# egpbos/barcode

Measured on AMD Instinct MI355X. Metric: HMC leapfrog steps/sec on 256^3 grid, higher is better.
Workload: dtype f64; 1 GPU; 256^3 grid, L=200 Mpc/h, Gaussian prior, Zel'dovich + plane-parallel RSD (reference behaviour of '2LPT+RSD', SURVEY M3), likelihood=1, mass kernel mk=3 (3 = SPH), calc_h=2, mass_type=1, fp64; one trajectory of 817 leapfrog steps per chain; grid=256, chains=1, parallelism=independent chains, 1 per GPU, rehearsal_single_device=False, steps_done=817, finite=True

## Files before the change

### barcode_amd/csrc/bchmc.hip

```cpp
#include "../../include/bchmc.h"
#include "kernels.hpp"
#include "fft_host.hpp"
#include "owned.hpp"
#include "pass_launch.hpp"
#include "launch_grid.hpp"
#include "eval_plan.hpp"
#include "interp_plan.hpp"

#include <rocfft/rocfft.h>
#include <rocprofiler-sdk-roctx/roctx.h>

#include <algorithm>
#include <chrono>
#include <cmath>
#include <cfloat>
#include <cstdarg>
#include <cstdio>
#include <cstdlib>
#include <climits>
#include <cstring>
#include <mutex>
#include <string>
#include <thread>
#include <type_traits>
#include <vector>

using namespace bchmc;
using namespace owned;

namespace {

struct ProfRec {
  int cls;
  Event a, b;
};

}

struct bchmc_handle {
  bchmc_config c{};
  Geo g{};
  bool f32 = false;
  size_t esz = 8;
  int mass_fs = 0, mass_rs = 0;
  PathSwitches sw;
  bool no_tiles_low = false;
  std::string err;
  RocfftUser fft_user;
  Stream stream;

  DevBytes work;
  FftInfo info;
  FftPlan r2c1, c2r1, r2c3, c2r3;

  DevBytes in_arr[6];
  bool have[6] = {false, false, false, false, false, false};
  DevBuf<double> wS, wM;

  DevBytes qk, pk, gk;
  DevBytes qk2, pk2;
  DevBytes Ck;
  bool ck_pair = false;
  DevBytes tC;
  DevBytes psi;
  DevBytes V;
  DevBytes rho, plike;
  DevBuf<long long> rho_fix;
  DevBuf<int> fix_sat;
  long long fix_sat_limit = 1ll << 62;
  bool fix = false;
  DevBytes ioq, iop;
  DevBytes gprior, glike;
  DevBytes conv;
  DevBuf<double> convF;
  DevBuf<double> dstage;
  DevBytes cq, cp;
  DevBuf<double> part6;
  bool have_cq = false, have_cp = false, have_prop = false;
  DevBytes cg;
  bool cg_valid = false, prop_g_valid = false;
  double c_like = 0., prop_like = 0.;
  DevBuf<double> rho_part, partA;
  DevBuf<double> guard;
  DevBuf<int> stop;
  DevBuf<unsigned long long> steps_done;
  PinnedBuf<double> h_part;
  struct MtDraw {
    long long S = 0, C = 0, G = 0;
    int B = 0;
    DevBuf<uint32_t> poly, win, words, st;
    DevBuf<unsigned long long> nz, nzoff, acc, accoff, lastend;
    DevBuf<unsigned long long> res;
    PinnedBuf<unsigned long long> h_io;
    DevBuf<double> gauss;
    double setup_ms = 0.;
  } mt;
  struct Mock {
    DevBuf<unsigned long long> cnt, off, gsum, goff, res;
  } mock;
  DevBuf<double> spec_bins;
  DevBytes cross_ak;
  struct Ens {
    struct Slot {
      uint64_t count = 0;
      DevBuf<double> mean, m2;
    } slot[BCHMC_ENS_SLOTS];
    int ncu = 0;
  } ens;
  struct Tweb {
    DevBytes t[6];
    DevBytes xk;
    DevBuf<unsigned char> type;
    DevBuf<double> lam;
    DevBuf<unsigned long long> part;
    DevBuf<unsigned int> cnt;
    bool have_t = false;
    uint64_t samples = 0;
    bool have_par = false;
// ... 258 lines not shown
  pp.L = h->g.L;
  pp.rsd = rsd;
  pp.periodic = 1;
  const double a = h->c.ascale, OM = h->c.OM, OL = h->c.OL;
  pp.cpecvel = c_pecvel1(a, OM, OL);
  const double Hub = 100. * std::sqrt(OM / a / a / a + OL + (1. - OM - OL) / a / a);
  pp.v_norm = 1. / Hub / a;
  return pp;
}

SphPar make_sph(const bchmc_handle *h) {
  SphPar sp;
  sp.h = h->c.particle_kernel_h;
  sp.h_inv = 1. / sp.h;
  sp.w_norm = 1. / M_PI / (sp.h * sp.h * sp.h);
  sp.r2_lim = 4. * sp.h * sp.h * (1. + (h->f32 ? 1e-5 : 1e-12));
  sp.min1 = h->c.min1;
  sp.min2 = h->c.min2;
  sp.min3 = h->c.min3;
  sp.reach = h->plan.reach;
  return sp;
}

LikePar make_like(const bchmc_handle *h) {
  LikePar lp;
  lp.rho_c = h->c.rho_c;
  lp.biasP = h->c.biasP;
  lp.biasE = h->c.biasE;
  lp.delta_min = h->c.delta_min;
  lp.likelihood = h->c.likelihood;
  lp.bias_is_identity = (h->c.biasE == 1.0);
  return lp;
}

HullPar make_hull(const bchmc_handle *h) {
  HullPar hp;
  const double hh = h->c.particle_kernel_h;
  hp.cols = h->hull;
  hp.ncol = h->plan.hull_n;
  hp.h_inv = 1. / hh;
  hp.d_h = h->g.d * hp.h_inv;
  hp.norm = 1. / (M_PI * (hh * hh) * (hh * hh));
  hp.normalize = h->c.rho_c * h->g.L * h->g.L * h->g.L / (double)h->g.N;
  hp.f1 = fgrow1(h->c.ascale, h->c.OM, h->c.OL);
  return hp;
}

int need_input(bchmc_handle *h, int f, const char *name) {
  if (!h->have[f]) return h->fail(BCHMC_ERR_STATE, "input array %s was never uploaded", name);
  return BCHMC_OK;
}

struct FieldSource {
  enum Made { kAsHeld, kOverdens, kPositions };
  void *base = nullptr;
  size_t offset = 0;
  Made made = kAsHeld;
};
int field_source(bchmc_handle *h, int field, FieldSource *fs) {
  const size_t N = (size_t)h->g.N;
  *fs = FieldSource{};
  switch (field) {
    case BCHMC_F_SIGNAL_PS: case BCHMC_F_MASS_F: case BCHMC_F_MASS_R:
    case BCHMC_F_NOBS: case BCHMC_F_NOISE: case BCHMC_F_WINDOW:
      fs->base = h->in_arr[field].get();
      break;
    case BCHMC_F_DELTAX: fs->base = h->ioq.get(), fs->made = FieldSource::kOverdens; break;
    case BCHMC_F_POSX: case BCHMC_F_POSY: case BCHMC_F_POSZ: fs->base = h->ioq.get(), fs->made = FieldSource::kPositions; break;
    case BCHMC_F_RHO: fs->base = h->rho.get(); break;
    case BCHMC_F_PART_LIKE: fs->base = h->plike.get(); break;
    case BCHMC_F_VX: case BCHMC_F_VY: case BCHMC_F_VZ: fs->base = h->V.get(), fs->offset = (size_t)(field - BCHMC_F_VX) * N; break;
    case BCHMC_F_PSIX: case BCHMC_F_PSIY: case BCHMC_F_PSIZ:
      fs->base = h->psi.get(), fs->offset = (size_t)(field - BCHMC_F_PSIX) * N;
      break;
    case BCHMC_F_GRAD_PRIOR: fs->base = h->gprior.get(); break;
    case BCHMC_F_GRAD_LIKE: fs->base = h->glike.get(); break;
    default: return h->fail(BCHMC_ERR_ARG, "unknown field %d", field);
  }
  if (!fs->base) return h->fail(BCHMC_ERR_STATE, "field %d has not been computed", field);
  return BCHMC_OK;
}
int fetch_ready(bchmc_handle *h, int field) {
  if (field >= BCHMC_F_DELTAX && field <= BCHMC_F_PSIZ && !h->have_eval)
    return h->fail(BCHMC_ERR_STATE, "no forward evaluation to fetch from");
  FieldSource fs;
  return field_source(h, field, &fs);
}

int check_inputs(bchmc_handle *h) {
  CHK(need_input(h, BCHMC_F_SIGNAL_PS, "signal_PS"));
  if (h->mass_fs) CHK(need_input(h, BCHMC_F_MASS_F, "mass_f"));
  if (h->mass_rs) CHK(need_input(h, BCHMC_F_MASS_R, "mass_r"));
  CHK(need_input(h, BCHMC_F_NOBS, "nobs"));
  CHK(need_input(h, BCHMC_F_WINDOW, "window"));
  if (h->c.likelihood != 0) CHK(need_input(h, BCHMC_F_NOISE, "noise"));
  return BCHMC_OK;
}

RecQuad *recs(const bchmc_handle *h) { return static_cast<RecQuad *>(h->srec.get()); }
int *slot_words(bchmc_handle *h) { return h->t_cnt + (kOct + 1) * (size_t)h->plan.tp.ntiles + 1; }

void repartition(bchmc_handle *h) {
  h->plan.tp.cap = h->plan.slots.cap;
  h->sorted_valid = false;
}

int realloc_slots(bchmc_handle *h, long long want) {
  HIPCHK(hipStreamSynchronize(h->stream));
  SlotPolicy &sl = h->plan.slots;
  const bool verbose = env_on("BCHMC_VERBOSE");
  const long long cap = sl.clamp_to_budget(want);
  if (!cap) {
    if (verbose) fprintf(stderr, "bchmc: record slots stay at %lld per tile (memory budget %lld): overflowing evaluations "
                                 "run the two-pass sort\n", sl.cap_alloc, sl.cap_budget);
    sl.after_realloc(SlotGot::kOldSize, cap);
    return BCHMC_OK;
  }
  (void)h->srec.release();
  h->sorted_valid = false;
  for (SlotGot got : {SlotGot::kWanted, SlotGot::kOldSize, SlotGot::kRecordsOnly}) {
    const size_t nrec = record_count(h->g.N, sl.rung(got, cap), h->plan.tp.ntiles);
    if (h->srec.alloc(nrec * 4 * h->esz) == hipSuccess) {
      if (got == SlotGot::kWanted) {
        if (verbose) fprintf(stderr, "bchmc: record array reallocated for %lld slots per tile\n", cap);
// ... 77 lines not shown
  bool ok2 = rocfft_plan_description_create(&f2) == rocfft_status_success &&
             rocfft_plan_description_create(&i2) == rocfft_status_success;
  ok2 = ok2 && rocfft_plan_description_set_data_layout(f2, rocfft_array_type_real, rocfft_array_type_hermitian_interleaved,
                                                       nullptr, nullptr, 2, rs2, (size_t)g.n * g.n, 2, cs2,
                                                       (size_t)g.n * g.nhp) == rocfft_status_success;
  ok2 = ok2 && rocfft_plan_description_set_data_layout(i2, rocfft_array_type_hermitian_interleaved, rocfft_array_type_real,
                                                       nullptr, nullptr, 2, cs2, (size_t)g.n * g.nhp, 2, rs2,
                                                       (size_t)g.n * g.n) == rocfft_status_success;
  ok2 = ok2 && r2c.create(rocfft_plan_create, rocfft_placement_notinplace, rocfft_transform_type_real_forward, prec, 2,
                          len2, batch, f2) == rocfft_status_success;
  ok2 = ok2 && c2r.create(rocfft_plan_create, rocfft_placement_notinplace, rocfft_transform_type_real_inverse, prec, 2,
                          len2, batch, i2) == rocfft_status_success;
  if (f2) rocfft_plan_description_destroy(f2);
  if (i2) rocfft_plan_description_destroy(i2);
  if (ok2 && h->info) {
    size_t need = 0;
    for (const FftPlan *p : {&r2c, &c2r}) {
      size_t wb = 0;
      if (rocfft_plan_get_work_buffer_size(*p, &wb) != rocfft_status_success) ok2 = false;
      need = std::max(need, wb);
    }
    if (ok2 && need > h->work.capacity()) {
      DevBytes nw;
      (void)hipStreamSynchronize(h->stream);
      if (nw.alloc(need) == hipSuccess &&
          rocfft_execution_info_set_work_buffer(h->info, nw, need) == rocfft_status_success) {
        h->work = std::move(nw);
      } else {
        (void)hipGetLastError();
        ok2 = false;
      }
    }
  }
  if (!ok2) {
    r2c.reset();
    c2r.reset();
    return BCHMC_ERR_ROCFFT;
  }
  return BCHMC_OK;
}

PathSwitches read_path_switches() {
  PathSwitches s;
  s.no_planes = env_on("BCHMC_NO_PLANES");
  s.no_planes_ends = env_on("BCHMC_NO_PLANES_ENDS");
  s.no_fuse = env_on("BCHMC_NO_FUSE");
  s.no_alpt_planes = env_on("BCHMC_NO_ALPT_PLANES");
  s.no_zbin = env_on("BCHMC_NO_ZBIN");
  s.zbin_128 = env_on("BCHMC_ZBIN_128");
  s.yfwd_f64 = env_on("BCHMC_YFWD_F64");
  s.bx_v1 = env_on("BCHMC_BX_V1");
  s.bx_v2 = env_on("BCHMC_BX_V2");
  s.no_pair = env_on("BCHMC_NO_PAIR");
  return s;
}

PathFacts path_facts(bchmc_handle *h, int rsd) {
  PathFacts f;
  f.n = h->g.n, f.esz = (int)h->esz, f.Nhp = h->g.Nhp;
  f.planes_ok = h->planes_ok && h->xtw;
  f.tiled = h->plan.tiled, f.sort_direct = h->plan.slots.sort_direct;
  f.mk = h->c.mk, f.calc_h = h->c.calc_h, f.likelihood = h->c.likelihood, f.sfmodel = h->c.sfmodel;
  f.rsd_model = h->c.rsd_model, f.mass_rs = h->mass_rs != 0;
  if (alpt_planes_wanted(f, h->sw, rsd) && !h->c2r2d_2 && !h->alpt_plans_failed &&
      make_plans_2d(h, 2 * (size_t)h->g.n, h->r2c2d_2, h->c2r2d_2) != BCHMC_OK)
    h->alpt_plans_failed = true;
  f.alpt_plans = h->c2r2d_2 != nullptr;
  return f;
}

int host_sum(bchmc_handle *h, const double *d_part, double *out) {
  HIPCHK(hipMemcpyAsync(h->h_part, d_part, kRedBlocks * sizeof(double), hipMemcpyDeviceToHost, h->stream));
  HIPCHK(hipStreamSynchronize(h->stream));
  double s = 0.;
  for (int i = 0; i < kRedBlocks; i++) s += h->h_part[i];
  *out = s;
  return BCHMC_OK;
}

void par_memcpy(void *dst, const void *src, size_t bytes, int nt) {
  if (nt <= 1 || bytes < ((size_t)4 << 20)) {
    std::memcpy(dst, src, bytes);
    return;
  }
  std::vector<std::thread> th;
  const size_t per = ((bytes / (size_t)nt) + 4095) & ~(size_t)4095;
  for (int t = 1; t < nt; t++) {
    const size_t off = per * (size_t)t;
    if (off >= bytes) break;
    const size_t len = std::min(per, bytes - off);
    th.emplace_back([=] { std::memcpy((char *)dst + off, (const char *)src + off, len); });
  }
  std::memcpy(dst, src, std::min(per, bytes));
  for (auto &t : th) t.join();
}

int stg_init(bchmc_handle *h) {
  if (h->stg[0]) return BCHMC_OK;
  size_t chunk = (size_t)16 << 20;
  if (const char *ev = std::getenv("BCHMC_STAGE_MB")) chunk = (size_t)std::max(1, atoi(ev)) << 20;
  int nt = (int)std::min(8u, std::max(1u, std::thread::hardware_concurrency() / 2));
  if (const char *ev = std::getenv("BCHMC_STAGE_THREADS")) nt = std::max(1, atoi(ev));
  for (int b = 0; b < 2; b++) {
    HIPCHK(h->stg[b].alloc(chunk));
    HIPCHK(h->stg_ev[b].create(hipEventDisableTiming));
  }
  h->stg_chunk = chunk;
  h->stg_threads = nt;
  return BCHMC_OK;
}

int h2d(bchmc_handle *h, void *dst, const void *src, size_t bytes, hipStream_t stream = nullptr) {
  if (!stream) stream = h->stream;
  if (bytes <= ((size_t)1 << 20)) {
// ... 599 lines not shown
      CHK(fft_exec(h, h->r2c2d_2, h->V, Ck, BCHMC_K_FFT_R2C));
      ProfScope ps(h, BCHMC_K_KSPACE_DRIFT_ZA);
      HIPCHK(launch_alpt_mix_x<T>(pass_ctx(h), Ck, h->c.kth, 1. / h->alpt_wtot, 1. / (double)N));
    } else {
      CHK(fft_exec(h, h->r2c1, a_out, Ck, BCHMC_K_FFT_R2C));
      CHK(fft_exec(h, h->r2c1, b_out, Ck + Nhp, BCHMC_K_FFT_R2C));
      ProfScope ps(h, BCHMC_K_KSPACE_DRIFT_ZA);
      k_alpt_mix<T><<<nblk_stride(Nhp), 256, 0, h->stream>>>(h->g, Ck, h->c.kth, 1. / h->alpt_wtot, 1. / (double)N);
      HIPCHK(hipGetLastError());
    }
    return BCHMC_OK;
  }

  static int launch_alpt(bchmc_handle *h, double dq_factor, bool planes) {
    const double scale = dq_factor / (double)h->g.N;
    if (planes) {
      {
        ProfScope ps(h, BCHMC_K_KSPACE_DRIFT_ZA);
        StepCtl nc{h->stop, h->steps_done, nullptr, 0., 0};
        BoundaryX<T> bx;
        bx.qi = C(h->qk), bx.c_za = scale, bx.ctl = nc;
        CHK((launch_boundary_x<BX_FIRST, true>(h, bx)));
      }
      return alpt_middle(h, true);
    }
    {
      ProfScope ps(h, BCHMC_K_KSPACE_DRIFT_ZA);
      k_alpt_poisson<T><<<nblk_stride(h->g.Nhp), 256, 0, h->stream>>>(h->g, C(h->qk), C(h->Ck), C(h->Ck) + h->g.Nhp, scale);
      HIPCHK(hipGetLastError());
    }
    return alpt_middle(h, false);
  }

  static int forward_rest(bchmc_handle *h, int rsd, EvalMode m) {
    if (rsd && !h->c.planepar) return h->fail(BCHMC_ERR_RSD_NOT_PLANEPAR, "non-plane-parallel RSD is not implemented");
    const bool zbin = eval_zbin(path_facts(h, rsd), h->sw, m);
    const bool pair = h->ck_pair;
    h->ck_pair = false;
    if (pair && !zbin) return h->fail(BCHMC_ERR_STATE, "two arrays between the x and y passes, and no y pass of the engine's own");
    if (zbin) {
      ProfScope ps(h, BCHMC_K_FFT_C2R);
      HIPCHK(pair ? launch_ypass_pair<T>(pass_ctx(h), C(h->Ck)) : launch_ypass<T>(pass_ctx(h), C(h->Ck)));
    } else {
      CHK(fft_exec(h, m.planes_c2r ? h->c2r2d : h->c2r3, h->Ck, h->psi, BCHMC_K_FFT_C2R));
    }
    return particle_stage(h, rsd, m, zbin);
  }

  static int particle_stage(bchmc_handle *h, int rsd, EvalMode m, bool zbin) {
    h->sorted_valid = false;
    bool rho_cleared = false;
    const PosPar pp = make_pos(h, rsd);
    const SphPar sp = make_sph(h);
    if (h->plan.tiled) {
      ProfScope ps(h, BCHMC_K_SORT);
      const int nt = h->plan.tp.ntiles, nbricks = nblk_full(h->g.N);
      int *cnt1 = h->t_cnt, *cnt2 = h->t_cnt + kOct * nt, *ovf = h->t_cnt + (kOct + 1) * nt;
      if (!h->cnt_clean) HIPCHK(hipMemsetAsync(h->t_cnt, 0, ((kOct + 1) * (size_t)nt + 1) * sizeof(int), h->stream));
      h->cnt_clean = false;
      const int fb_grid = h->plan.slots.sort_direct ? std::min(nbricks, 4096) : nbricks;
      if (zbin) {
        HIPCHK(launch_zbin<T>(pass_ctx(h), pp, sp, h->plan.tp, C(h->Ck), cnt1, ovf, recs(h), R(h->V), h->rho_part,
                              h->fix ? nullptr : R(h->rho), h->fix ? h->rho_fix : nullptr,
                              m.psi_unread ? nullptr : R(h->psi)));
        if (m.psi_unread)
          HIPCHK((launch_zbin<T, true>(pass_ctx(h), pp, sp, h->plan.tp, C(h->Ck), cnt1, ovf, nullptr, nullptr, nullptr,
                                       nullptr, nullptr, R(h->psi))));
        rho_cleared = true;
      } else if (h->plan.slots.sort_direct) {
        const int nsuper = (nbricks + kBinPer - 1) / kBinPer;
        k_bin_direct<T><<<nsuper, BCHMC_BIN_THREADS, 0, h->stream>>>(h->g, pp, sp, h->plan.tp, nsuper, R(h->psi), cnt1, ovf,
                                                       recs(h), R(h->V), h->rho_part,
                                                       h->fix ? nullptr : R(h->rho),
                                                       h->fix ? h->rho_fix : nullptr);
        rho_cleared = true;
      } else {
        HIPCHK(hipMemsetAsync(ovf, 1, 1, h->stream));
      }
      k_bin<T><<<fb_grid, 256, 0, h->stream>>>(h->g, pp, sp, h->plan.tp, nbricks, R(h->psi), cnt2, ovf, h->t_rank, R(h->V));
      k_scan_tiles<<<(nt + 1023) / 1024, 1024, 0, h->stream>>>(h->plan.tp, cnt1, cnt2, ovf, h->t_off, h->t_end, h->t_woff,
                                                               h->t_oct, h->t_seg, ovf + 2);
      k_reorder<T><<<fb_grid, 256, 0, h->stream>>>(h->g, pp, nbricks, R(h->psi), h->t_rank, h->t_off, ovf,
                                                   recs(h));
      HIPCHK(hipGetLastError());
      h->sorted_valid = true;
    }
    {
      ProfScope ps(h, BCHMC_K_SCATTER);
      const bool tile_path = (h->c.mk == 3 && h->plan.tiled), tile_low = (h->c.mk >= 0 && h->c.mk <= 2 && h->plan.tiled);
      const double fix_scale = h->c.mk == 3 ? 70368744177664. / sp.w_norm : 70368744177664.;
      if (rho_cleared) {
      } else if (h->fix) {
        HIPCHK(hipMemsetAsync(h->rho_fix, 0, h->g.N * sizeof(long long), h->stream));
      } else {
        HIPCHK(hipMemsetAsync(h->rho, 0, h->g.N * sizeof(T), h->stream));
      }
      if (tile_path) {
        if (!h->plan.slots.sort_direct && !h->fix) HIPCHK(hipMemsetAsync(h->rho_part, 0, kRedBlocks * sizeof(double), h->stream));
        const int grid = tile_grid(h);
        const int ncol = h->plan.hull_exact ? h->plan.hull_n : 0;
        const int reorder = (h->plan.tp.chunk > 2048) ? 0 : 2;
        if (reorder) {
          k_subsort<T><<<std::min(grid, 8192), 256, 0, h->stream>>>(h->g, h->plan.tp, reorder, recs(h), h->t_off, h->t_end, h->t_woff,
                                                   h->t_oct, h->t_seg);
          HIPCHK(hipGetLastError());
        }
        if (h->plan.std81) {
          if (h->fix)
            k_scatter_tile81<T, 12, 20, true><<<grid, kTile81Threads, tile_lds(h, 0, sizeof(double)), h->stream>>>(
                h->g, sp, h->plan.tp, recs(h), h->t_off, h->t_end, h->t_woff,
                h->t_oct, h->t_seg, h->rho_fix, h->rho_part, h->t_cnt,
                (kOct + 1) * h->plan.tp.ntiles + 1, fix_scale);
          else
            k_scatter_tile81<T, 12, 20, false><<<grid, kTile81Threads, tile_lds(h, 0, sizeof(double)), h->stream>>>(
                h->g, sp, h->plan.tp, recs(h), h->t_off, h->t_end, h->t_woff,
                h->t_oct, h->t_seg, R(h->rho), h->rho_part, h->t_cnt,
                (kOct + 1) * h->plan.tp.ntiles + 1, fix_scale);
          h->cnt_clean = true;
        } else if (h->fix) {
          k_scatter_tile<T, true><<<grid, 256, tile_lds(h, ncol, sizeof(double)), h->stream>>>(
              h->g, sp, h->plan.tp, h->hull, ncol, recs(h), h->t_off, h->t_end,
              h->t_woff, h->t_oct, h->t_seg, h->rho_fix, h->rho_part, fix_scale);
        } else {
          k_scatter_tile<T, false><<<grid, 256, tile_lds(h, ncol, sizeof(double)), h->stream>>>(
              h->g, sp, h->plan.tp, h->hull, ncol, recs(h), h->t_off, h->t_end,
              h->t_woff, h->t_oct, h->t_seg, R(h->rho), h->rho_part, fix_scale);
        }
      } else if (tile_low) {
        if (!h->plan.slots.sort_direct && !h->fix) HIPCHK(hipMemsetAsync(h->rho_part, 0, kRedBlocks * sizeof(double), h->stream));
        const int grid = tile_grid(h);
        const size_t lds = (size_t)(h->plan.tp.tx + 2) * (h->plan.tp.ty + 2) * (h->plan.tp.tz + 2) * sizeof(double);
        const int ncnt = (kOct + 1) * h->plan.tp.ntiles + 1;
// ... 1 lines not shown
          k_scatter_tile_low<T, true><<<grid, 256, lds, h->stream>>>(h->g, h->plan.tp, h->c.mk, recs(h), h->t_off,
                                                                     h->t_end, h->t_woff, h->t_oct, h->t_seg, h->rho_fix,
                                                                     h->rho_part, h->t_cnt, ncnt, fix_scale);
        else
          k_scatter_tile_low<T, false><<<grid, 256, lds, h->stream>>>(h->g, h->plan.tp, h->c.mk, recs(h), h->t_off,
                                                                      h->t_end, h->t_woff, h->t_oct, h->t_seg, R(h->rho),
                                                                      h->rho_part, h->t_cnt, ncnt, fix_scale);
        h->cnt_clean = true;
      } else if (h->c.mk == 3) {
        if (h->fix)
          k_scatter_sph<T, true><<<nblk_full(h->g.N), 256, 0, h->stream>>>(h->g, pp, sp, R(h->psi), h->rho_fix, fix_scale);
        else
          k_scatter_sph<T, false><<<nblk_full(h->g.N), 256, 0, h->stream>>>(h->g, pp, sp, R(h->psi), R(h->rho), fix_scale);
      } else if (h->c.mk >= 0 && h->c.mk <= 2) {
        if (h->fix)
          k_scatter_low_order<T, true><<<nblk_full(h->g.N), 256, 0, h->stream>>>(h->g, pp, sp, h->c.mk, R(h->psi),
                                                                                 h->rho_fix, fix_scale);
        else
          k_scatter_low_order<T, false><<<nblk_full(h->g.N), 256, 0, h->stream>>>(h->g, pp, sp, h->c.mk, R(h->psi),
                                                                                  R(h->rho), fix_scale);
      } else {
        return h->fail(BCHMC_ERR_ARG, "masskernel %d is not a valid value (0..3)", h->c.mk);
      }
      HIPCHK(hipGetLastError());
      if (h->fix) {
        k_fix_to_rho<T><<<kRedBlocks, 256, 0, h->stream>>>(h->g.N, h->rho_fix, 1. / fix_scale, R(h->rho), h->rho_part,
                                                           h->fix_sat, h->fix_sat_limit);
        HIPCHK(hipGetLastError());
      }
    }
    if (!h->plan.tiled && !h->fix) {
      ProfScope ps(h, BCHMC_K_MEAN_PARTIAL);
      k_sum<T><<<kRedBlocks, 256, 0, h->stream>>>(R(h->rho), h->g.N, h->rho_part);
      HIPCHK(hipGetLastError());
    }
    h->have_eval = true;
    h->last_rsd = rsd;
    return BCHMC_OK;
  }

  static int ensure_conv(bchmc_handle *h) {
    if (!h->conv) CHK(dev_alloc(h, h->conv, 3 * (size_t)h->g.N * sizeof(T)));
    return BCHMC_OK;
  }

  static int like_force(bchmc_handle *h, EvalMode m, int *like_mode, bool transform = true) {
    if (h->c.calc_h == 2 || h->c.calc_h == 3) {
      if (h->c.mk != 3)
        return h->fail(BCHMC_ERR_MK_NOT_SPH, "Must use SPH mass kernel (masskernel = 3) with calc_h = 2 or 3");
    } else if (h->c.calc_h != 1 && h->c.calc_h != 0) {
      return h->fail(BCHMC_ERR_ARG, "calc_h = %d is not a valid value (0..3)", h->c.calc_h);
    }
    const long long N = h->g.N, Nh = h->g.Nhp;
    {
      ProfScope ps(h, BCHMC_K_MEAN_PARTIAL);
      k_partial_like<T><<<nblk_stride(N), 256, 0, h->stream>>>(h->g, make_like(h), R(h->rho), h->rho_part,
                                                               R(h->in_arr[BCHMC_F_NOBS]), R(h->in_arr[BCHMC_F_NOISE]),
                                                               R(h->in_arr[BCHMC_F_WINDOW]), R(h->plike));
      HIPCHK(hipGetLastError());
    }
    if (h->c.calc_h == 1) {
      if (transform) CHK(fft_exec(h, h->r2c1, h->plike, h->Ck, BCHMC_K_FFT_R2C));
      *like_mode = 1;
      return BCHMC_OK;
    }
    if (h->c.calc_h == 0) {
      {
        ProfScope ps(h, BCHMC_K_OTHER);
        k_overdens<T><<<nblk_stride(N), 256, 0, h->stream>>>(h->g, R(h->rho), h->rho_part, R(h->ioq));
        HIPCHK(hipGetLastError());
      }
      if (h->c.likelihood == 1) {
        CHK(ensure_conv(h));
        CHK(fft_exec(h, h->r2c1, h->ioq, h->tC, BCHMC_K_FFT_R2C));
        {
          ProfScope ps(h, BCHMC_K_OTHER);
          k_gradfft_mult<T><<<nblk_stride(Nh), 256, 0, h->stream>>>(h->g, C(h->tC), C(h->Ck), 1. / (double)N);
          HIPCHK(hipGetLastError());
        }
        CHK(fft_exec(h, h->c2r3, h->Ck, h->conv, BCHMC_K_FFT_C2R));
        ProfScope ps(h, BCHMC_K_OTHER);
        k_mul3<T><<<nblk_stride(N), 256, 0, h->stream>>>(N, R(h->plike), R(h->conv), R(h->V));
        HIPCHK(hipGetLastError());
      } else {
        ProfScope ps(h, BCHMC_K_OTHER);
        k_findif_mul<T><<<nblk_stride(N), 256, 0, h->stream>>>(h->g, make_like(h), R(h->ioq), R(h->plike), R(h->V));
        HIPCHK(hipGetLastError());
      }
      if (transform) CHK(fft_exec(h, h->r2c3, h->V, h->Ck, BCHMC_K_FFT_R2C));
      *like_mode = 0;
      return BCHMC_OK;
    }
    if (h->c.calc_h == 3) {
      if (h->last_rsd && !h->c.planepar)
        return h->fail(BCHMC_ERR_RSD_NOT_PLANEPAR, "non-plane-parallel RSD is not implemented in calc_V");
      CHK(ensure_conv(h));
      if (!h->convF) CHK(build_conv_table(h));
      CHK(fft_exec(h, h->r2c1, h->plike, h->tC, BCHMC_K_FFT_R2C));
      const double hh = h->c.particle_kernel_h;
      {
        ProfScope ps(h, BCHMC_K_OTHER);
        k_conv_kernel<T><<<nblk_stride(Nh), 256, 0, h->stream>>>(h->g, C(h->tC), h->convF, C(h->Ck), hh, 1. / (double)N);
        HIPCHK(hipGetLastError());
      }
      CHK(fft_exec(h, h->c2r3, h->Ck, h->conv, BCHMC_K_FFT_C2R));
      {
        ProfScope ps(h, BCHMC_K_GATHER);
        if (h->plan.tiled && h->sorted_valid && !h->no_tiles_low) {
          const int grid = tile_grid(h);
          const size_t lds = 3 * (size_t)(h->plan.tp.tx + 2) * (h->plan.tp.ty + 2) * (h->plan.tp.tz + 2) * sizeof(T);
          k_interp_tsc_tile<T><<<grid, 256, lds, h->stream>>>(h->g, h->plan.tp, h->last_rsd, fgrow1(h->c.ascale, h->c.OM, h->c.OL),
                                                              recs(h), h->t_off, h->t_end, h->t_woff,
                                                              h->t_oct, h->t_seg, R(h->conv), R(h->V));
        } else {
          k_interp_tsc<T><<<nblk_full(N), 256, 0, h->stream>>>(h->g, make_pos(h, h->last_rsd),
                                                               fgrow1(h->c.ascale, h->c.OM, h->c.OL), R(h->psi),
                                                               R(h->conv), R(h->V));
        }
        HIPCHK(hipGetLastError());
      }
    } else {
      ProfScope ps(h, BCHMC_K_GATHER);
      HullPar hp = make_hull(h);
      if (h->plan.tiled && h->sorted_valid) {
        const int grid = tile_grid(h);
        if (h->plan.std81)
          k_gather_tile81<T, 12, 20><<<grid, kTile81Threads, tile_lds(h, 0, sizeof(T)), h->stream>>>(
              h->g, hp, h->plan.tp, h->last_rsd, recs(h), h->t_off, h->t_end, h->t_woff,
              h->t_oct, h->t_seg, R(h->plike), R(h->V));
        else
          k_gather_tile<T><<<grid, 256, tile_lds(h, hp.ncol, sizeof(T)), h->stream>>>(
              h->g, hp, h->plan.tp, h->last_rsd, recs(h), h->t_off, h->t_end, h->t_woff,
              h->t_oct, h->t_seg, R(h->plike), R(h->V));
      } else {
        k_gather_sph<T><<<nblk_full(N), 256, hp.ncol * sizeof(int4), h->stream>>>(h->g, make_pos(h, h->last_rsd), hp,
                                                                                  R(h->psi), R(h->plike), R(h->V));
      }
      HIPCHK(hipGetLastError());
    }
    if (!transform) {
    } else if (eval_yfwd(path_facts(h, h->c.rsd_model), h->sw, m)) {
      ProfScope ps(h, BCHMC_K_FFT_R2C);
      HIPCHK(launch_zr2c<T>(pass_ctx(h), R(h->V), C(h->Ck)));
      HIPCHK((launch_ypass<T, false>(pass_ctx(h), C(h->Ck))));
    } else {
      CHK(fft_exec(h, m.planes_r2c ? h->r2c2d : h->r2c3, h->V, h->Ck, BCHMC_K_FFT_R2C));
    }
    *like_mode = 0;
    return BCHMC_OK;
  }

  static int grf_force(bchmc_handle *h) {
    {
      ProfScope ps(h, BCHMC_K_OTHER);
      k_scale_c<T><<<nblk_stride(h->g.Nhp), 256, 0, h->stream>>>(h->g.Nhp, C(h->qk), C(h->tC), 1. / (double)h->g.N);
      HIPCHK(hipGetLastError());
    }
    CHK(fft_exec(h, h->c2r1, h->tC, h->plike, BCHMC_K_FFT_C2R));
    {
      ProfScope ps(h, BCHMC_K_OTHER);
      k_grf_grad<T><<<nblk_stride(h->g.N), 256, 0, h->stream>>>(h->g.N, R(h->plike), R(h->in_arr[BCHMC_F_NOBS]),
                                                                R(h->in_arr[BCHMC_F_NOISE]),
                                                                R(h->in_arr[BCHMC_F_WINDOW]), R(h->rho));
      HIPCHK(hipGetLastError());
    }
    CHK(fft_exec(h, h->r2c1, h->rho, h->Ck, BCHMC_K_FFT_R2C));
    h->have_eval = false;
    return BCHMC_OK;
  }

  static int force_sources(bchmc_handle *h, bool pre_za, EvalMode m, int *like_mode, double *b) {
    if (h->c.likelihood == 3) {
      CHK(grf_force(h));
      *like_mode = 1;
      *b = h->c.grad_psi_likeli_factor;
      return BCHMC_OK;
    }
    if (!pre_za) {
      CHK(displacement(h, h->c.deltaQ_factor, h->c.rsd_model, &m.planes_c2r));
    } else if (m.alpt_pending) {
      CHK(alpt_middle(h, true));
      m.planes_c2r = true;
    }
    CHK(forward_rest(h, h->c.rsd_model, m));
    CHK(like_force(h, m, like_mode));
    double norm = -1.;
    norm *= h->c.deltaQ_factor;
    if (h->c.correct_delta) norm *= h->c.D1;
    *b = h->c.grad_psi_likeli_factor * norm;
    return BCHMC_OK;
  }

  template <bool KICK>
  static int launch_assemble(bchmc_handle *h, double a, double b, int like_mode, double c_kick, double *guard_slot) {
    h->prop_g_valid = false;
    ProfScope ps(h, BCHMC_K_KSPACE_FORCE_KICK);
    k_assemble<T, KICK><<<nblk_stride(h->g.Nhp), 256, 0, h->stream>>>(h->g, C(h->Ck), C(h->qk), h->wS, C(h->gk), C(h->pk),
                                                                     a, b, like_mode, c_kick, guard_slot, h->stop);
    HIPCHK(hipGetLastError());
    return BCHMC_OK;
  }

  static int r2c_state(bchmc_handle *h, const double *d_real, void *staging, void *out) {
    CHK(load_real(h, d_real, R(staging)));
    return fft_exec(h, h->r2c1, staging, out, BCHMC_K_FFT_R2C);
  }

  static int c2r_scaled(bchmc_handle *h, const void *xk, void *out_T) {
    {
      ProfScope ps(h, BCHMC_K_OTHER);
      k_scale_c<T><<<nblk_stride(h->g.Nhp), 256, 0, h->stream>>>(h->g.Nhp, reinterpret_cast<const CT *>(xk), C(h->tC),
                                                                1. / (double)h->g.N);
      HIPCHK(hipGetLastError());
    }
    return fft_exec(h, h->c2r1, h->tC, out_T, BCHMC_K_FFT_C2R);
  }

  static int c2r_state(bchmc_handle *h, const void *xk, void *scratch_T, double *d_out) {
    if (kDouble) return c2r_scaled(h, xk, d_out);
    CHK(c2r_scaled(h, xk, scratch_T));
    return store_real(h, R(scratch_T), d_out);
  }

  static int mass_rs_term(bchmc_handle *h) {
    CHK(c2r_scaled(h, h->pk, h->iop));
    {
      ProfScope ps(h, BCHMC_K_OTHER);
      k_div_mass_r<T><<<nblk_stride(h->g.N), 256, 0, h->stream>>>(h->g.N, R(h->iop), R(h->in_arr[BCHMC_F_MASS_R]),
                                                                  R(h->iop));
      HIPCHK(hipGetLastError());
    }
    return fft_exec(h, h->r2c1, h->iop, h->tC, BCHMC_K_FFT_R2C);
  }

  struct Tap {
    double *like_i, *like_f;
  };

  static int tap_loglike(bchmc_handle *h, double *partials) {
    k_loglike<T><<<kRedBlocks, 256, 0, h->stream>>>(h->g, make_like(h), R(h->rho), h->rho_part,
                                                    R(h->in_arr[BCHMC_F_NOBS]), R(h->in_arr[BCHMC_F_NOISE]),
                                                    R(h->in_arr[BCHMC_F_WINDOW]), partials);
    HIPCHK(hipGetLastError());
    return BCHMC_OK;
  }

  struct Traj {
    PathFacts f;
    TrajPlan p;
    double a, c_za;
    bool pair;
  };
  static Traj traj(bchmc_handle *h) {
    Traj t;
    t.f = path_facts(h, h->c.rsd_model);
    t.p = traj_plan(t.f, h->sw);
    t.a = h->c.grad_psi_prior_factor;
    t.c_za = (t.p.c_za == CZa::kAlptInput ? 1. : -h->c.D1) * h->c.deltaQ_factor / (double)h->g.N;
    t.pair = psi_pair(t.f, h->sw, t.p);
    return t;
  }

  template <int MODE, bool ALPT = false>
  static int launch_boundary_x(bchmc_handle *h, const BoundaryX<T> &bx) {
    HIPCHK((launch_step_boundary_x<T, MODE, ALPT>(pass_ctx(h), C(h->Ck), h->wS, bx)));
    h->ck_pair = bx.pair && !ALPT && MODE != BX_LAST;
    return BCHMC_OK;
  }

  static int initial_force(bchmc_handle *h, const Traj &t, double *like_i, void *g0_out) {
    int like_mode = 2;
    double b = 0.;
    const InitialEval kind = initial_eval(t.f, h->sw, t.p);
    if (kind == InitialEval::k3d) {
      CHK(force_sources(h, false, EvalMode{}, &like_mode, &b));
      if (like_i) CHK(tap_loglike(h, like_i));
      CHK(launch_assemble<false>(h, t.a, b, like_mode, 0., nullptr));
    } else {
      StepCtl nc{h->stop, h->steps_done, nullptr, 0., 0};
      {
        ProfScope ps(h, BCHMC_K_KSPACE_DRIFT_ZA);
        BoundaryX<T> bx;
        bx.qi = C(h->qk), bx.c_za = t.c_za, bx.ctl = nc, bx.pair = t.pair;
        if (kind == InitialEval::kBxFirstAlpt) CHK((launch_boundary_x<BX_FIRST, true>(h, bx)));
        else CHK(launch_boundary_x<BX_FIRST>(h, bx));
      }
      EvalMode m;
      m.planes_c2r = m.planes_r2c = true;
      m.alpt_pending = t.p.alpt_x;
      CHK(force_sources(h, true, m, &like_mode, &b));
      if (like_mode != 0) return h->fail(BCHMC_ERR_STATE, "planes mode without the three V components");
      if (like_i) CHK(tap_loglike(h, like_i));
      h->prop_g_valid = false;
      ProfScope ps(h, BCHMC_K_KSPACE_FORCE_KICK);
      BoundaryX<T> bx;
      bx.qi = C(h->qk), bx.a = t.a, bx.b = b, bx.ctl = nc, bx.g_out = C(h->gk);
      CHK(launch_boundary_x<BX_LAST>(h, bx));
    }
    if (g0_out)
      HIPCHK(hipMemcpyAsync(g0_out, h->gk, 2 * (size_t)h->g.Nhp * sizeof(T), hipMemcpyDeviceToDevice, h->stream));
    return BCHMC_OK;
  }

  static int trajectory(bchmc_handle *h, double eps, uint64_t neps, const Tap *tap, const void *g0_in = nullptr,
                        void *g0_out = nullptr) {
    h->prop_g_valid = false;
    if (neps + 1 > h->guard.capacity())
      CHK(dev_reserve(h, h->guard, std::max<size_t>(4096, 2 * (neps + 1))));
    HIPCHK(hipMemsetAsync(h->guard, 0, (neps + 1) * sizeof(double), h->stream));
    k_init_ctl<<<1, 1, 0, h->stream>>>(h->stop, h->steps_done, (unsigned long long)neps);
    HIPCHK(hipGetLastError());

    const Traj t = traj(h);
    int like_mode = 2;
    double b = 0.;
    if (!g0_in) CHK(initial_force(h, t, tap ? tap->like_i : nullptr, g0_out));
    const void *g_first = g0_in ? g0_in : h->gk;
// ... 33 lines not shown

  static int trajectory_fused(bchmc_handle *h, double eps, uint64_t neps, const Tap *tap, const Traj &t,
                              const void *g_first) {
    const double *wM = h->mass_fs ? h->wM : nullptr;
    const double guard_limit = 1e50 * (double)h->g.N, a = t.a, c_za = t.c_za;
    if (!h->qk2) {
      CHK(dev_alloc(h, h->qk2, 2 * (size_t)h->g.Nhp * sizeof(T)));
      CHK(dev_alloc(h, h->pk2, 2 * (size_t)h->g.Nhp * sizeof(T)));
    }
    void *const q0 = h->qk, *const p0 = h->pk, *const q1 = h->qk2, *const p1 = h->pk2;
    int like_mode = 2;
    double b = 0.;
    int cur = 0;
    {
      StepCtl ctl{h->stop, h->steps_done, nullptr, guard_limit, 0};
      ProfScope ps(h, BCHMC_K_KSPACE_DRIFT_ZA);
      BoundaryX<T> bx;
      bx.qi = bx.qo = C(q0), bx.pi = bx.po = C(p0), bx.wM = wM, bx.half_eps = 0.5 * eps, bx.eps = eps, bx.c_za = c_za;
      bx.ctl = ctl, bx.g_in = C(g_first), bx.pair = t.pair;
      switch (opening(t.f, h->sw, t.p)) {
        case Opening::kBxFirstAlpt: CHK((launch_boundary_x<BX_FIRST, true>(h, bx))); break;
        case Opening::kBxFirst: CHK(launch_boundary_x<BX_FIRST>(h, bx)); break;
        case Opening::kKickDriftZa:
          h->ck_pair = false;
          k_kick_drift_za<T, true><<<nblk_stride(h->g.Nhp), 256, 0, h->stream>>>(h->g, C(q0), C(p0), C(g_first), wM,
                                                                               nullptr, C(h->Ck), 0.5 * eps, eps, c_za, ctl);
          break;
      }
      HIPCHK(hipGetLastError());
    }
    for (uint64_t s = 0; s < neps; s++) {
      const bool last = (s + 1 == neps);
      if (last && h->early_q_dev && h->ev_q) {
        CHK(c2r_state(h, cur ? q1 : q0, h->ioq, h->early_q_dev));
        HIPCHK(hipEventRecord(h->ev_q, h->stream));
        h->early_q_done = true;
      }
      if (h->plan.slots.slot_watch && h->plan.tiled && h->plan.slots.sort_direct && s > 0 && s % kSlotPoll == 0)
        CHK(poll_slots(h, s / kSlotPoll));
      CHK(force_sources(h, true, step_mode(t.f, h->sw, t.p, s, neps), &like_mode, &b));
      if (tap && tap->like_f && last) CHK(tap_loglike(h, tap->like_f));
      StepCtl ctl{h->stop, h->steps_done, s > 0 ? h->guard + (s - 1) : nullptr, guard_limit, s};
      void *qi = cur ? q1 : q0, *pi = cur ? p1 : p0, *qo = cur ? q0 : q1, *po = cur ? p0 : p1;
      ProfScope ps(h, BCHMC_K_KSPACE_FORCE_KICK);
      BoundaryX<T> bx;
      bx.qi = C(qi), bx.pi = C(pi), bx.qo = C(qo), bx.po = C(po), bx.wM = wM, bx.a = a, bx.b = b, bx.half_eps = 0.5 * eps;
      bx.eps = eps, bx.c_za = c_za, bx.guard_slot = h->guard + s, bx.ctl = ctl, bx.pair = t.pair;
      switch (closing(t.f, h->sw, t.p, s, neps, like_mode)) {
        case Closing::kBxLast:
          bx.qo = nullptr, bx.po = C(pi), bx.g_out = C(h->gk);
          CHK(launch_boundary_x<BX_LAST>(h, bx));
          break;
        case Closing::kStepBoundaryLast:
          k_step_boundary<T, true><<<nblk_stride(h->g.Nhp), 256, 0, h->stream>>>(
              h->g, C(h->Ck), C(qi), C(pi), C(qi), C(pi), C(h->gk), h->wS, wM, a, b, like_mode, 0.5 * eps, eps, c_za,
              h->guard + s, ctl);
          break;
        case Closing::kBxInteriorAlpt: CHK((launch_boundary_x<BX_INTERIOR, true>(h, bx))); break;
        case Closing::kBxInterior: CHK(launch_boundary_x<BX_INTERIOR>(h, bx)); break;
        case Closing::kBxInteriorTwoTile:
          HIPCHK(launch_step_boundary_x2<T>(pass_ctx(h), C(h->Ck), h->wS, bx));
          h->ck_pair = bx.pair;
          break;
        case Closing::kStepBoundary:
          k_step_boundary<T, false><<<nblk_stride(h->g.Nhp), 256, 0, h->stream>>>(
              h->g, C(h->Ck), C(qi), C(pi), C(qo), C(po), C(h->gk), h->wS, wM, a, b, like_mode, 0.5 * eps, eps, c_za,
              h->guard + s, ctl);
          break;
      }
      if (buffers_flip(s, neps)) cur ^= 1;
      HIPCHK(hipGetLastError());
    }
    {
      ProfScope ps(h, BCHMC_K_OTHER);
      k_rollback<T><<<nblk_stride(h->g.Nhp), 256, 0, h->stream>>>(h->g.Nhp, h->stop, h->steps_done, C(q0), C(p0), C(q1),
                                                                 C(p1), C(cur ? q1 : q0), C(cur ? p1 : p0));
      HIPCHK(hipGetLastError());
    }
    if (cur) {
      std::swap(h->qk, h->qk2);
      std::swap(h->pk, h->pk2);
    }
    return BCHMC_OK;
  }

  static int leapfrog_core(bchmc_handle *h, const double *d_q0, const double *d_p0, double *d_q1, double *d_p1,
                           double eps, uint64_t neps, bool prologue_done = false) {
    CHK(check_inputs(h));
    if (eps > 2.) eps = 2.;
    if (!prologue_done) CHK(r2c_state(h, d_q0, h->ioq, h->qk));
    CHK(r2c_state(h, d_p0, h->iop, h->pk));
    CHK(trajectory(h, eps, neps, nullptr, prologue_done ? h->gk : nullptr));
    if (!h->early_q_done) CHK(c2r_state(h, h->qk, h->ioq, d_q1));
    CHK(c2r_state(h, h->pk, h->iop, d_p1));
    return BCHMC_OK;
  }
  static int requeue_q(bchmc_handle *h, double *d_q1) { return c2r_state(h, h->qk, h->ioq, d_q1); }

  static int chain_alloc(bchmc_handle *h) {
    if (!h->cq) {
      CHK(dev_alloc(h, h->cq, 2 * (size_t)h->g.Nhp * sizeof(T)));
      CHK(dev_alloc(h, h->cp, 2 * (size_t)h->g.Nhp * sizeof(T)));
      CHK(dev_alloc(h, h->part6, (size_t)6 * kRedBlocks));
    }
    return BCHMC_OK;
  }

  static int chain_draw(bchmc_handle *h, uint64_t seed, uint64_t attempt) {
    const long long N = h->g.N, Nh = h->g.Nhp;
    const uint2 key = make_uint2((unsigned)seed, (unsigned)(seed >> 32));
    ProfScope ps(h, BCHMC_K_OTHER);
    if (h->mass_fs) {
      k_white_noise<T><<<nblk_stride((N + 1) / 2), 256, 0, h->stream>>>(N, key, (unsigned)attempt, 0u, nullptr, R(h->iop));
      HIPCHK(hipGetLastError());
      CHK(fft_exec(h, h->r2c1, h->iop, h->tC, BCHMC_K_FFT_R2C));
      k_color_momenta<T><<<nblk_stride(Nh), 256, 0, h->stream>>>(Nh, C(h->tC), h->wM, C(h->cp), 0);
      HIPCHK(hipGetLastError());
// ... 196 lines not shown
                                                          h->partA);
      HIPCHK(hipGetLastError());
      CHK(host_sum(h, h->partA, &like));
    } else {
      const bool gauss = (h->c.likelihood == 1);
      EvalMode m;
      CHK(displacement(h, gauss ? h->c.deltaQ_factor : 1., gauss ? h->c.rsd_model : 0, &m.planes_c2r));
      CHK(forward_rest(h, gauss ? h->c.rsd_model : 0, m));
      k_loglike<T><<<kRedBlocks, 256, 0, h->stream>>>(h->g, make_like(h), R(h->rho), h->rho_part,
                                                      R(h->in_arr[BCHMC_F_NOBS]), R(h->in_arr[BCHMC_F_NOISE]),
                                                      R(h->in_arr[BCHMC_F_WINDOW]), h->partA);
      HIPCHK(hipGetLastError());
      CHK(host_sum(h, h->partA, &like));
    }
    out[0] = prior;
    out[1] = like;
    return BCHMC_OK;
  }

  static int energies_core(bchmc_handle *h, const double *d_q, const double *d_p, double out[3]) {
    CHK(check_inputs(h));
    CHK(kinetic_core(h, d_p, &out[0]));
    return psi_core(h, d_q, &out[1]);
  }

  static int forward(bchmc_handle *h, const double *d_q, int rsd) {
    CHK(r2c_state(h, d_q, h->ioq, h->qk));
    EvalMode m;
    CHK(displacement(h, 1., rsd, &m.planes_c2r));
    return forward_rest(h, rsd, m);
  }

  static int chain_forward(bchmc_handle *h, int rsd) {
    HIPCHK(hipMemcpyAsync(h->qk, h->cq, 2 * (size_t)h->g.Nhp * sizeof(T), hipMemcpyDeviceToDevice, h->stream));
    EvalMode m;
    CHK(displacement(h, 1., rsd, &m.planes_c2r));
    return forward_rest(h, rsd, m);
  }

  static int probe_load(bchmc_handle *h, int c) { return load_real(h, h->dstage, R(h->psi) + (size_t)c * h->g.N); }
  static int probe(bchmc_handle *h, int rsd, bool with_force) {
    EvalMode m;
    CHK(particle_stage(h, rsd, m, false));
    int like_mode = 0;
    if (with_force) CHK(like_force(h, m, &like_mode, false));
    return BCHMC_OK;
  }
  static int probe_z(bchmc_handle *h, int rsd, bool with_force, bool store_psi) {
    const int n = h->g.n;
    k_scale_r<T><<<nblk_stride(3 * h->g.N), 256, 0, h->stream>>>(3 * h->g.N, R(h->psi), T(1) / T(n));
    HIPCHK(hipGetLastError());
    HIPCHK(launch_zr2c<T>(pass_ctx(h), R(h->psi), C(h->Ck)));
    EvalMode m;
    m.planes_c2r = true;
    m.psi_unread = !store_psi;
    CHK(particle_stage(h, rsd, m, true));
    int like_mode = 0;
    if (with_force) CHK(like_force(h, m, &like_mode, false));
    return BCHMC_OK;
  }

  static int corr_field(bchmc_handle *h, int src) {
    const void *xk = h->tC;
    if (src == BCHMC_CORR_HOST) {
      CHK(r2c_state(h, h->dstage, h->ioq, h->tC));
    } else if (src == BCHMC_CORR_CHAIN_STATE) {
      xk = h->cq;
    } else {
      k_overdens<T><<<nblk_stride(h->g.N), 256, 0, h->stream>>>(h->g, R(h->rho), h->rho_part, R(h->ioq));
      HIPCHK(hipGetLastError());
      CHK(fft_exec(h, h->r2c1, h->ioq, h->tC, BCHMC_K_FFT_R2C));
    }
    {
      ProfScope ps(h, BCHMC_K_OTHER);
      k_corr_abs2<T><<<nblk_stride(h->g.Nhp), 256, 0, h->stream>>>(h->g.Nhp, C(xk), C(h->tC), 1. / (double)h->g.N);
      HIPCHK(hipGetLastError());
    }
    return fft_exec(h, h->c2r1, h->tC, h->ioq, BCHMC_K_FFT_C2R);
  }

  static int corr1d_bins(bchmc_handle *h, uint64_t n_bin, double *rmode, uint64_t *nmode, double *corr) {
    auto &c = h->corr1;
    const Geo &g = h->g;
    const size_t nb = (size_t)n_bin, words = 5 * nb + 1;
    if (c.acc.capacity() < words) {
      c.n_bin = 0;
      CHK(dev_reserve(h, c.acc, words));
    }
    const bool geom = c.n_bin != n_bin;
    const double dr = corr_dr(g, n_bin);
    const int grid = std::min(nblk_full(g.N), 1024);
    unsigned long long *d_geo = c.acc + 2 * nb + 1;
    std::vector<unsigned long long> hb(words);
    {
      ProfScope ps(h, BCHMC_K_OTHER);
      HIPCHK(hipMemsetAsync(c.acc, 0, (geom ? words : 2 * nb + 1) * sizeof(unsigned long long), h->stream));
      if (geom) {
        const double rscale = std::ldexp(1., 62 - std::ilogb(g.L / 2 * std::sqrt(3.)));
        k_corr1d<T, true><<<grid, 256, 3 * nb * sizeof(unsigned long long), h->stream>>>(g, nullptr, (int)n_bin, dr,
                                                                                      rscale, d_geo);
      }
      k_corr1d<T, false><<<grid, 256, 2 * nb * sizeof(unsigned long long), h->stream>>>(g, R(h->ioq), (int)n_bin, dr, 0.,
                                                                                     c.acc);
      HIPCHK(hipGetLastError());
      HIPCHK(hipMemcpyAsync(hb.data(), c.acc, (geom ? words : 2 * nb + 1) * sizeof(unsigned long long),
                            hipMemcpyDeviceToHost, h->stream));
    }
// ... 332 lines not shown
    const dim3 g1((unsigned)((w.ncls + kMpWaves - 1) / kMpWaves), (unsigned)((g.nh + kSpecChunk - 1) / kSpecChunk));
    const dim3 g2((unsigned)n_bin + 1, (unsigned)nseg);
    {
      ProfScope ps(h, BCHMC_K_OTHER);
      k_mp_classes<T, NS, REAL><<<g1, kSpecChunk * kMpWaves, 0, h->stream>>>(g, a, b, w.rows, w.ncls, w.part, stride);
      if (hg) {
        k_mp_shells<1, true><<<g2, kMpBlock, 0, h->stream>>>(g.n, g.nh, u, dt, (int)n_bin, w.ncls, w.cls, w.part, stride, REAL ? 0 : 1, w.out);
        HIPCHK(hipMemcpyAsync(hg, w.out, cells * kMpGeom * sizeof(double), hipMemcpyDeviceToHost, h->stream));
      }
      k_mp_shells<NS, false><<<g2, kMpBlock, 0, h->stream>>>(g.n, g.nh, u, dt, (int)n_bin, w.ncls, w.cls, w.part, stride, REAL ? 0 : 1, w.out);
      HIPCHK(hipGetLastError());
      HIPCHK(hipMemcpyAsync(hs, w.out, cells * 3 * NS * sizeof(double), hipMemcpyDeviceToHost, h->stream));
    }
    HIPCHK(hipStreamSynchronize(h->stream));
    return BCHMC_OK;
  }
  static int mp_auto(bchmc_handle *h, const void *xk, uint64_t n_bin, double *hg, double *hs) {
    return mp_sums<1, false>(h, xk, nullptr, n_bin, hg, hs);
  }
  static int mp_cross(bchmc_handle *h, const void *ak, const void *bk, uint64_t n_bin, double *hg, double *hs) {
    return mp_sums<3, false>(h, ak, bk, n_bin, hg, hs);
  }
  static int mp_corr(bchmc_handle *h, uint64_t n_bin, double *hg, double *hs) {
    return mp_sums<1, true>(h, h->ioq, nullptr, n_bin, hg, hs);
  }

  static int gradient(bchmc_handle *h, const double *d_q, double *d_g) {
    const size_t N = (size_t)h->g.N;
    if (!h->gprior) {
      CHK(dev_alloc(h, h->gprior, N * sizeof(T)));
      CHK(dev_alloc(h, h->glike, N * sizeof(T)));
    }
    CHK(r2c_state(h, d_q, h->ioq, h->qk));
    int like_mode = 2;
    double b = 0.;
    CHK(force_sources(h, false, EvalMode{}, &like_mode, &b));
    CHK(launch_assemble<false>(h, h->c.grad_psi_prior_factor, 0., 2, 0., nullptr));
    CHK(c2r_scaled(h, h->gk, h->gprior));
    CHK(launch_assemble<false>(h, 0., b, like_mode, 0., nullptr));
    CHK(c2r_scaled(h, h->gk, h->glike));
    k_add_r<T><<<nblk_stride(h->g.N), 256, 0, h->stream>>>(h->g.N, R(h->gprior), R(h->glike), R(h->iop));
    HIPCHK(hipGetLastError());
    return store_real(h, R(h->iop), d_g);
  }

  static int fetch(bchmc_handle *h, bchmc_field field, double *d_out) {
    FieldSource fs;
    CHK(field_source(h, (int)field, &fs));
    if (fs.made == FieldSource::kOverdens)
      k_overdens<T><<<nblk_stride(h->g.N), 256, 0, h->stream>>>(h->g, R(h->rho), h->rho_part, R(h->ioq));
    if (fs.made == FieldSource::kPositions)
      k_positions<T><<<nblk_stride(h->g.N), 256, 0, h->stream>>>(h->g, make_pos(h, h->last_rsd), R(h->psi), R(h->ioq),
                                                                 (int)field - (int)BCHMC_F_POSX);
    if (fs.made != FieldSource::kAsHeld) HIPCHK(hipGetLastError());
    return store_real(h, R(fs.base) + fs.offset, d_out);
  }

  static int mt_place(bchmc_handle *h) {
    const long long N = h->g.N, Nh = h->g.Nhp;
    const int n = h->g.n;
    ProfScope ps(h, BCHMC_K_OTHER);
    HIPCHK(hipMemsetAsync(h->cp, 0, 2 * (size_t)Nh * sizeof(T), h->stream));
    if (h->mass_fs) {
      const long long cells = (long long)(n / 2 + 1) * (n / 2 + 1) * (n / 2 + 1);
      const double amp = (double)N * (double)N / (h->g.L * h->g.L * h->g.L);
      k_mt_place<T><<<nblk_stride(cells), 256, 0, h->stream>>>(n, h->g.nhp, h->mt.gauss, R(h->in_arr[BCHMC_F_MASS_F]),
                                                               amp, C(h->cp));
      HIPCHK(hipGetLastError());
    }
    if (h->mass_rs) {
      k_mt_real_space<T><<<nblk_stride(N), 256, 0, h->stream>>>(N, h->mt.gauss + (h->mass_fs ? 2 * N : 0),
                                                                R(h->in_arr[BCHMC_F_MASS_R]), R(h->iop));
      HIPCHK(hipGetLastError());
      CHK(fft_exec(h, h->r2c1, h->iop, h->tC, BCHMC_K_FFT_R2C));
      k_color_momenta<T><<<nblk_stride(Nh), 256, 0, h->stream>>>(Nh, C(h->tC), nullptr, C(h->cp), 1);
      HIPCHK(hipGetLastError());
    }
    return BCHMC_OK;
  }

  static int mock_place(bchmc_handle *h, void *dst) {
    const long long N = h->g.N;
    const int n = h->g.n;
    ProfScope ps(h, BCHMC_K_OTHER);
    HIPCHK(hipMemsetAsync(dst, 0, 2 * (size_t)h->g.Nhp * sizeof(T), h->stream));
    const long long cells = (long long)(n / 2 + 1) * (n / 2 + 1) * (n / 2 + 1);
    const double amp = (double)N * (double)N / (h->g.L * h->g.L * h->g.L);
    k_mt_place<T><<<nblk_stride(cells), 256, 0, h->stream>>>(n, h->g.nhp, h->mt.gauss, R(h->in_arr[BCHMC_F_SIGNAL_PS]),
                                                             amp, C(dst));
    HIPCHK(hipGetLastError());
    return BCHMC_OK;
  }

  static long long mock_tiles(const bchmc_handle *h) { return (h->g.N + kMockTile - 1) / kMockTile; }
  static long long mock_groups(const bchmc_handle *h) { return (mock_tiles(h) + kMtThreads - 1) / kMtThreads; }

  static int mock_alloc(bchmc_handle *h) {
    auto &k = h->mock;
    if (k.cnt) return BCHMC_OK;
    CHK(dev_alloc(h, k.cnt, (size_t)mock_tiles(h)));
    CHK(dev_alloc(h, k.off, (size_t)mock_tiles(h)));
    CHK(dev_alloc(h, k.gsum, (size_t)mock_groups(h)));
    CHK(dev_alloc(h, k.goff, (size_t)mock_groups(h)));
    CHK(dev_alloc(h, k.res, (size_t)2));
    return BCHMC_OK;
  }
// ... 2535 lines not shown
```

### barcode_amd/csrc/eval_plan.hpp

```cpp
#pragma once

#include "pass_launch.hpp"

namespace bchmc {

struct PathSwitches {
  bool no_planes = false;
  bool no_planes_ends = false;
  bool no_fuse = false;
  bool no_alpt_planes = false;
  bool no_zbin = false;
  bool zbin_128 = false;
  bool yfwd_f64 = false;
  bool bx_v1 = false;
  bool bx_v2 = false;
  bool no_pair = false;
};

struct PathFacts {
  int n = 0, esz = 8;
  long long Nhp = 0;
  bool planes_ok = false;
  bool tiled = false;
  bool sort_direct = false;
  int mk = 3, calc_h = 2, likelihood = 1, sfmodel = 1, rsd_model = 0;
  bool mass_rs = false;
  bool alpt_plans = false;
};

struct EvalMode {
  bool planes_c2r = false;
  bool planes_r2c = false;
  bool alpt_pending = false;
  bool psi_unread = false;
};

constexpr bool planes_on(const PathFacts &f, const PathSwitches &s) {
  return f.planes_ok && x_shape(f.esz, f.n).nt && f.calc_h == 2 && f.mk == 3 && !s.no_planes;
}
constexpr bool planes_at_ends(const PathFacts &f, const PathSwitches &s) { return planes_on(f, s) && !s.no_planes_ends; }

constexpr bool uses_alpt(const PathFacts &f, int rsd) { return !rsd && f.sfmodel != 1; }
constexpr bool alpt_planes_wanted(const PathFacts &f, const PathSwitches &s, int rsd) {
  return uses_alpt(f, rsd) && planes_at_ends(f, s) && !s.no_alpt_planes;
}
constexpr bool alpt_on_planes(const PathFacts &f, const PathSwitches &s, int rsd) {
  return alpt_planes_wanted(f, s, rsd) && f.alpt_plans;
}

enum class ZbinWhyNot { kNone, kSwitchedOff, kNeeds128Switch, kGridSize, kNotSphAdjoint, kNoOnePassBinning, kNoPlanes };

constexpr ZbinWhyNot zbin_why_not(const PathFacts &f, const PathSwitches &s) {
  if (s.no_zbin) return ZbinWhyNot::kSwitchedOff;
  if (f.n == 128 && !s.zbin_128) return ZbinWhyNot::kNeeds128Switch;
  if (!z_shape(f.esz, f.n).nt) return ZbinWhyNot::kGridSize;
  if (f.mk != 3 || f.calc_h != 2) return ZbinWhyNot::kNotSphAdjoint;
  if (!f.tiled || !f.sort_direct) return ZbinWhyNot::kNoOnePassBinning;
  if (!f.planes_ok) return ZbinWhyNot::kNoPlanes;
  return ZbinWhyNot::kNone;
}
constexpr const char *zbin_why_not_text(ZbinWhyNot w) {
  switch (w) {
    case ZbinWhyNot::kNone: return nullptr;
    case ZbinWhyNot::kSwitchedOff: return "BCHMC_NO_ZBIN is set";
    case ZbinWhyNot::kNeeds128Switch: return "Nx = 128 takes it with BCHMC_ZBIN_128=1 only";
    case ZbinWhyNot::kGridSize: return "it exists for Nx = 128, 256 and 512";
    case ZbinWhyNot::kNotSphAdjoint: return "it needs masskernel 3 with calc_h 2";
    case ZbinWhyNot::kNoOnePassBinning: return "the one-pass tile binning is not in use";
    case ZbinWhyNot::kNoPlanes: break;
  }
  return "the planes-mode transforms are not available";
}
constexpr bool zbin_ok(const PathFacts &f, const PathSwitches &s) { return zbin_why_not(f, s) == ZbinWhyNot::kNone; }
constexpr bool eval_zbin(const PathFacts &f, const PathSwitches &s, const EvalMode &m) { return m.planes_c2r && zbin_ok(f, s); }

constexpr bool yfwd_ok(const PathFacts &f, const PathSwitches &s) {
  return f.n == 512 && (f.esz == 4 || s.yfwd_f64) && f.planes_ok;
}
constexpr bool eval_yfwd(const PathFacts &f, const PathSwitches &s, const EvalMode &m) { return m.planes_r2c && yfwd_ok(f, s); }

constexpr bool interior_two_tile(const PathFacts &f, const PathSwitches &s) {
  const bool want = (f.esz == 4 && !s.bx_v1) || (f.esz == 8 && f.n <= 256 && s.bx_v2);
  return x2_shape(f.esz, f.n).nt && want && (unsigned long long)f.Nhp * 2 * f.esz < (1ull << 32);
}

enum class CZa {
  kZeldovich,
  kAlptInput
};
struct TrajPlan {
  bool alpt_x = false, fused_za = false, fused = false;
  CZa c_za = CZa::kZeldovich;
};

constexpr bool psi_pair(const PathFacts &f, const PathSwitches &s, const TrajPlan &tp) {
  return !s.no_pair && !tp.alpt_x && planes_on(f, s) && zbin_ok(f, s) && ypair_shape(f.esz, f.n).nt;
}
constexpr TrajPlan traj_plan(const PathFacts &f, const PathSwitches &s) {
  TrajPlan tp;
  const bool alpt = uses_alpt(f, f.rsd_model) && f.likelihood != 3;
  tp.alpt_x = alpt && !f.mass_rs && !s.no_fuse && alpt_on_planes(f, s, f.rsd_model);
  tp.fused_za = f.likelihood != 3 && !alpt;
  tp.c_za = tp.alpt_x ? CZa::kAlptInput : CZa::kZeldovich;
  tp.fused = (tp.fused_za || tp.alpt_x) && !f.mass_rs && !s.no_fuse;
  return tp;
}

enum class InitialEval { k3d, kBxFirst, kBxFirstAlpt };
constexpr InitialEval initial_eval(const PathFacts &f, const PathSwitches &s, const TrajPlan &tp) {
  if (!(tp.fused && planes_at_ends(f, s))) return InitialEval::k3d;
  return tp.alpt_x ? InitialEval::kBxFirstAlpt : InitialEval::kBxFirst;
}

enum class Opening { kKickDriftZa, kBxFirst, kBxFirstAlpt };
constexpr Opening opening(const PathFacts &f, const PathSwitches &s, const TrajPlan &tp) {
  if (!planes_at_ends(f, s)) return Opening::kKickDriftZa;
  return tp.alpt_x ? Opening::kBxFirstAlpt : Opening::kBxFirst;
}
constexpr EvalMode step_mode(const PathFacts &f, const PathSwitches &s, const TrajPlan &tp, unsigned long long step,
                             unsigned long long neps) {
  const bool planes = planes_on(f, s), ends = planes_at_ends(f, s), last = step + 1 == neps;
  EvalMode m;
  m.planes_c2r = planes && (step > 0 || ends);
  m.planes_r2c = planes && (!last || ends);
  m.alpt_pending = tp.alpt_x;
  m.psi_unread = !last;
  return m;
}
enum class Closing { kBxLast, kStepBoundaryLast, kBxInterior, kBxInteriorTwoTile, kBxInteriorAlpt, kStepBoundary };
constexpr Closing closing(const PathFacts &f, const PathSwitches &s, const TrajPlan &tp, unsigned long long step,
                          unsigned long long neps, int like_mode) {
  const bool last = step + 1 == neps, xmode = step_mode(f, s, tp, step, neps).planes_r2c && like_mode == 0;
  if (last) return xmode ? Closing::kBxLast : Closing::kStepBoundaryLast;
  if (!xmode) return Closing::kStepBoundary;
  if (tp.alpt_x) return Closing::kBxInteriorAlpt;
  return interior_two_tile(f, s) ? Closing::kBxInteriorTwoTile : Closing::kBxInterior;
}
constexpr bool buffers_flip(unsigned long long step, unsigned long long neps) { return step + 1 != neps; }

}
```

### barcode_amd/csrc/fft_probe.hip

```cpp
#include "kernels.hpp"
#include "fft_host.hpp"
#include "pass_launch.hpp"
#include "launch_grid.hpp"

#include <cmath>
#include <cstring>
#include <vector>

using namespace bchmc;

namespace {

constexpr size_t kCanary = 64 * 1024;
constexpr unsigned char kCanaryByte = 0x5b;

template <typename T, int NT>
__global__ void __launch_bounds__(NT)
k_probe_xfft(int n, int log2n, int kb, int inverse, const C2<T> *__restrict__ twiddle, C2<T> *data) {
  extern __shared__ __attribute__((aligned(16))) unsigned char s_raw_p[];
  C2<T> *s = reinterpret_cast<C2<T> *>(s_raw_p);
  C2<T> *tw = s + (size_t)n * kb;
  for (int t = threadIdx.x; t < n / 2; t += NT) tw[t] = twiddle[t];
  C2<T> *col = data + (long long)blockIdx.x * n * kb;
  const int shift = 32 - log2n;
// ... 44 lines not shown
      for (unsigned char b : c)
        if (b != kCanaryByte) return (int)i + 1;
    }
    return 0;
  }
  template <typename T> const C2<T> *twiddles(int n) {
    const std::vector<T> tw = fft_twiddles<T>(n);
    return static_cast<const C2<T> *>(alloc(tw.size() * sizeof(T), tw.data()));
  }
  template <typename T> PassCtx<T> ctx(const Geo &g) { return {nullptr, g, ilog2(g.n), twiddles<T>(g.n)}; }
};

Geo probe_geo(int n, int esz, double L = 0.) {
  Geo g;
  g.n = n;
  g.nh = n / 2 + 1;
  g.nhp = fft_row_stride(n, esz);
  g.N = (long long)n * n * n;
  g.Nh = (long long)n * n * g.nh;
  g.Nhp = (long long)n * n * g.nhp;
  g.L = L > 0. ? L : (double)n;
  g.d = g.L / n;
  g.kfac = 2. * M_PI / g.L;
  return g;
}

template <typename T, int NT>
void launch_xfft(Probe &pr, int groups, int n, int kb, int inverse, const C2<T> *tw, C2<T> *d) {
  const size_t lds = ((size_t)n * kb + n / 2) * sizeof(C2<T>);
  pr.ok(launch_dyn_lds(nullptr, k_probe_xfft<T, NT>, groups, NT, lds, n, ilog2(n), kb, inverse, tw, d));
}

template <typename T> int xfft(int n, int kb, int inverse, int groups, void *data) {
  if (ilog2(n) < 5 || n > 512 || groups < 1 || (kb != pass_kb(sizeof(T)) && kb != 6)) return -1;
  const int nt = kb == 6 ? n : x_shape(sizeof(T), n).nt;
  Probe pr;
  const size_t bytes = (size_t)groups * n * kb * sizeof(C2<T>);
  const C2<T> *tw = pr.twiddles<T>(n);
  C2<T> *d = static_cast<C2<T> *>(pr.alloc(bytes, data));
  if (pr.err) return pr.err;
  switch (nt) {
    case 32: launch_xfft<T, 32>(pr, groups, n, kb, inverse, tw, d); break;
    case 64: launch_xfft<T, 64>(pr, groups, n, kb, inverse, tw, d); break;
    case 128: launch_xfft<T, 128>(pr, groups, n, kb, inverse, tw, d); break;
    case 256: launch_xfft<T, 256>(pr, groups, n, kb, inverse, tw, d); break;
    case 512: launch_xfft<T, 512>(pr, groups, n, kb, inverse, tw, d); break;
    case 1024: launch_xfft<T, 1024>(pr, groups, n, kb, inverse, tw, d); break;
    default: return -1;
  }
  return pr.finish({{1, data}});
}

template <typename T> int ypass(int n, int inverse, void *ck) {
  if (!y_shape(sizeof(T), n).nt || (!inverse && n != 512)) return -1;
  const Geo g = probe_geo(n, (int)sizeof(T));
  if (g.nhp % pass_kb(sizeof(T))) return -1;
  Probe pr;
  const PassCtx<T> x = pr.ctx<T>(g);
  C2<T> *d = static_cast<C2<T> *>(pr.alloc((size_t)3 * g.Nhp * sizeof(C2<T>), ck));
  if (pr.err) return pr.err;
  pr.ok(inverse ? launch_ypass<T>(x, d) : launch_ypass<T, false>(x, d));
  return pr.finish({{1, ck}});
}

template <typename T> int ypass_pair(int n, double box_len, void *ck) {
  if (!ypair_shape(sizeof(T), n).nt) return -1;
  const Geo g = probe_geo(n, (int)sizeof(T), box_len);
  if (g.nhp % pass_kb(sizeof(T))) return -1;
  Probe pr;
  const PassCtx<T> x = pr.ctx<T>(g);
  C2<T> *d = static_cast<C2<T> *>(pr.alloc((size_t)3 * g.Nhp * sizeof(C2<T>), ck));
  if (pr.err) return pr.err;
  pr.ok(launch_ypass_pair<T>(x, d));
  return pr.finish({{1, ck}});
}

template <typename T> int zr2c(int n, const void *V, void *ck) {
  if (!z_shape(sizeof(T), n).nt) return -1;
  const Geo g = probe_geo(n, (int)sizeof(T));
  Probe pr;
  const PassCtx<T> x = pr.ctx<T>(g);
  const T *dv = static_cast<const T *>(pr.alloc((size_t)3 * g.N * sizeof(T), V));
  C2<T> *dc = static_cast<C2<T> *>(pr.alloc((size_t)3 * g.Nhp * sizeof(C2<T>), ck));
  if (pr.err) return pr.err;
  pr.ok(launch_zr2c<T>(x, dv, dc));
  return pr.finish({{2, ck}});
}

template <typename T> int zc2r(int n, const void *ck, void *psi) {
  if (!z_shape(sizeof(T), n).nt) return -1;
  const Geo g = probe_geo(n, (int)sizeof(T));
  Probe pr;
  const PassCtx<T> x = pr.ctx<T>(g);
  const C2<T> *dc = static_cast<const C2<T> *>(pr.alloc((size_t)3 * g.Nhp * sizeof(C2<T>), ck));
  const int ovf_h[3] = {1, 0, 0};
  int *ovf = static_cast<int *>(pr.alloc(sizeof(ovf_h), ovf_h));
  T *dp = static_cast<T *>(pr.alloc((size_t)3 * g.N * sizeof(T), nullptr));
  if (pr.err) return pr.err;
  pr.ok((launch_zbin<T, true>(x, PosPar{}, SphPar{}, TilePar{}, dc, nullptr, ovf, nullptr, nullptr, nullptr, nullptr, nullptr,
                              dp)));
  return pr.finish({{3, psi}});
}


struct CtlArgs {
  int *stop;
  unsigned long long *steps_done;
  const double *guard_prev;
  double guard_limit;
  unsigned long long step_index;
};
struct CtlDev {
  StepCtl ctl{};
  int i_stop = -1, i_done = -1;
};
CtlDev ctl_alloc(Probe &pr, const CtlArgs &c) {
  CtlDev d;
  d.ctl.stop = static_cast<int *>(pr.alloc(sizeof(int), c.stop));
  d.i_stop = (int)pr.bufs.size() - 1;
  d.ctl.steps_done = static_cast<unsigned long long *>(pr.alloc(sizeof(unsigned long long), c.steps_done));
  d.i_done = (int)pr.bufs.size() - 1;
  d.ctl.guard_prev = c.guard_prev ? static_cast<const double *>(pr.alloc(sizeof(double), c.guard_prev)) : nullptr;
  d.ctl.guard_limit = c.guard_limit;
  d.ctl.step_index = c.step_index;
  return d;
}

template <typename U> U *opt(Probe &pr, size_t bytes, const void *host, int *idx = nullptr) {
  if (!host) return nullptr;
  U *d = static_cast<U *>(pr.alloc(bytes, host));
  if (idx) *idx = (int)pr.bufs.size() - 1;
  return d;
}

using Outs = std::vector<std::pair<int, void *>>;
void out(Outs &o, int idx, void *host) {
  if (host && idx >= 0) o.push_back({idx, host});
}

template <typename T>
int step_boundary_x(int n, double L, int mode, int alpt, int two_tile, void *Ck, const void *q_in, const void *p_in,
                    const void *g_in, void *q_out, void *p_out, void *g_out, const double *wS, const double *wM,
                    const double *scal, double *guard_slot, const CtlArgs &ca) {
  if (mode < BX_INTERIOR || mode > BX_LAST || (alpt && mode == BX_LAST)) return -1;
  if (two_tile ? (!x2_shape(sizeof(T), n).nt || mode != BX_INTERIOR || alpt) : !x_shape(sizeof(T), n).nt) return -1;
  const Geo g = probe_geo(n, (int)sizeof(T), L);
  if (g.nhp % pass_kb(sizeof(T)) || !Ck || !q_in || !scal) return -1;
  const bool first_kick = mode == BX_FIRST && g_in, last_kick = mode == BX_LAST && p_out;
  if (mode == BX_INTERIOR && !(p_in && q_out && p_out && guard_slot)) return -1;
  if (first_kick && !(p_in && q_out && p_out)) return -1;
  if (mode == BX_LAST && (!g_out || (last_kick && !(p_in && guard_slot)))) return -1;
  if (mode != BX_FIRST && scal[0] != 0. && !wS) return -1;
  Probe pr;
  const PassCtx<T> x = pr.ctx<T>(g);
  const size_t cb = (size_t)g.Nhp * sizeof(C2<T>), db = (size_t)g.Nhp * sizeof(double);
  int i_ck, i_qo = -1, i_po = -1, i_go = -1, i_gs = -1;
  C2<T> *d_ck = opt<C2<T>>(pr, 3 * cb, Ck, &i_ck);
  BoundaryX<T> a;
  a.qi = opt<const C2<T>>(pr, cb, q_in);
  a.pi = opt<const C2<T>>(pr, cb, p_in);
  a.g_in = opt<const C2<T>>(pr, cb, g_in);
  a.qo = opt<C2<T>>(pr, cb, q_out, &i_qo);
  a.po = opt<C2<T>>(pr, cb, p_out, &i_po);
  a.g_out = opt<C2<T>>(pr, cb, g_out, &i_go);
  const double *d_ws = opt<const double>(pr, db, wS);
  a.wM = opt<const double>(pr, db, wM);
  a.a = scal[0], a.b = scal[1], a.half_eps = scal[2], a.eps = scal[3], a.c_za = scal[4];
  a.guard_slot = opt<double>(pr, sizeof(double), guard_slot, &i_gs);
  const CtlDev cd = ctl_alloc(pr, ca);
  a.ctl = cd.ctl;
  if (pr.err) return pr.err;
  hipError_t e = hipErrorInvalidConfiguration;
  if (two_tile) e = launch_step_boundary_x2<T>(x, d_ck, d_ws, a);
  else if (mode == BX_INTERIOR) e = alpt ? launch_step_boundary_x<T, BX_INTERIOR, true>(x, d_ck, d_ws, a)
                                         : launch_step_boundary_x<T, BX_INTERIOR, false>(x, d_ck, d_ws, a);
  else if (mode == BX_FIRST) e = alpt ? launch_step_boundary_x<T, BX_FIRST, true>(x, d_ck, d_ws, a)
                                      : launch_step_boundary_x<T, BX_FIRST, false>(x, d_ck, d_ws, a);
  else e = launch_step_boundary_x<T, BX_LAST, false>(x, d_ck, d_ws, a);
  pr.ok(e);
  Outs o;
  out(o, i_ck, Ck), out(o, i_qo, q_out), out(o, i_po, p_out), out(o, i_go, g_out), out(o, i_gs, guard_slot);
  out(o, cd.i_stop, ca.stop), out(o, cd.i_done, ca.steps_done);
  return pr.finish(o);
}

template <typename T> int alpt_mix_x(int n, double L, void *Ck, double smol, double inv_wtot, double inv_n) {
  if (!x_shape(sizeof(T), n).nt) return -1;
  const Geo g = probe_geo(n, (int)sizeof(T), L);
  if (g.nhp % pass_kb(sizeof(T))) return -1;
  Probe pr;
  const PassCtx<T> x = pr.ctx<T>(g);
  C2<T> *d = static_cast<C2<T> *>(pr.alloc((size_t)3 * g.Nhp * sizeof(C2<T>), Ck));
  if (pr.err) return pr.err;
  pr.ok(launch_alpt_mix_x<T>(x, d, smol, inv_wtot, inv_n));
  return pr.finish({{1, Ck}});
}

bool ok3d(int n) { return n >= 2 && n <= 512; }

template <typename T>
int kick_drift_za(int n, double L, int drift, void *qk, void *pk, const void *gk, const double *wM, const void *extra,
                  void *Ck, const double *scal, const CtlArgs &ca) {
  if (!ok3d(n) || !qk || !Ck || !scal || (drift && !(pk && gk))) return -1;
  const Geo g = probe_geo(n, (int)sizeof(T), L);
  Probe pr;
  const size_t cb = (size_t)g.Nhp * sizeof(C2<T>);
  int i_q, i_p = -1, i_ck;
  C2<T> *dq = opt<C2<T>>(pr, cb, qk, &i_q), *dp = opt<C2<T>>(pr, cb, pk, &i_p);
  const C2<T> *dg = opt<const C2<T>>(pr, cb, gk);
  const double *dw = opt<const double>(pr, (size_t)g.Nhp * sizeof(double), wM);
  const C2<T> *dx = opt<const C2<T>>(pr, cb, extra);
  C2<T> *dc = opt<C2<T>>(pr, 3 * cb, Ck, &i_ck);
  const CtlDev cd = ctl_alloc(pr, ca);
  if (pr.err) return pr.err;
  if (drift)
    k_kick_drift_za<T, true><<<nblk_stride(g.Nhp), 256>>>(g, dq, dp, dg, dw, dx, dc, scal[0], scal[1], scal[2], cd.ctl);
  else
    k_kick_drift_za<T, false><<<nblk_stride(g.Nhp), 256>>>(g, dq, dp, dg, dw, dx, dc, scal[0], scal[1], scal[2], cd.ctl);
  Outs o;
  out(o, i_q, qk), out(o, i_p, pk), out(o, i_ck, Ck), out(o, cd.i_stop, ca.stop), out(o, cd.i_done, ca.steps_done);
  return pr.finish(o);
}

// ... 236 lines not shown
  if (rc) return rc;
  if (!pr.ok(hipMemcpy(res, dp + (size_t)nblk * kTwebWords, kTwebWords * sizeof(unsigned long long), hipMemcpyDeviceToHost)))
    return pr.err;
  return 0;
}

template <typename T>
int bispec_triple(int n_shell, long long count, const void *arrays, const unsigned char *s3_end, double *sums, float *ms) {
  if (n_shell < 1 || n_shell > kBispecMaxShell || count < 1 || count > (1ll << 27) || !arrays || !sums) return -1;
  Probe pr;
  const T *da = static_cast<const T *>(pr.alloc((size_t)n_shell * count * sizeof(T), arrays));
  const int grid = bispec_grid(count), W = bispec_triplets(n_shell);
  double *dp = static_cast<double *>(pr.alloc(((size_t)grid + 1) * W * sizeof(double), nullptr));
  if (pr.err) return pr.err;
  const BispecPlan plan = bispec_plan(n_shell, reinterpret_cast<const unsigned char(*)[kBispecMaxShell]>(s3_end));
  BispecArrays arr{};
  for (int s = 0; s < n_shell; s++) arr.a[s] = da + (size_t)s * count;
  hipEvent_t e0 = nullptr, e1 = nullptr;
  if (ms && (!pr.ok(hipEventCreate(&e0)) || !pr.ok(hipEventCreate(&e1)))) return pr.err;
  if (ms) pr.ok(hipEventRecord(e0, nullptr));
  pr.ok(launch_bispec_triple<T>(nullptr, count, n_shell, arr, plan, dp, dp + (size_t)grid * W));
  if (ms) pr.ok(hipEventRecord(e1, nullptr));
  int rc = pr.finish({});
  if (!rc && ms && !pr.ok(hipEventElapsedTime(ms, e0, e1))) rc = pr.err;
  if (e0) (void)hipEventDestroy(e0);
  if (e1) (void)hipEventDestroy(e1);
  if (rc) return rc;
  if (!pr.ok(hipMemcpy(sums, dp + (size_t)grid * W, (size_t)W * sizeof(double), hipMemcpyDeviceToHost))) return pr.err;
  return 0;
}

}

extern "C" {

int fftp_row_stride(int n, int prec) { return fft_row_stride(n, prec ? 4 : 8); }

int fftp_xfft(int prec, int n, int kb, int inverse, int groups, void *data) {
  return prec ? xfft<float>(n, kb, inverse, groups, data) : xfft<double>(n, kb, inverse, groups, data);
}

int fftp_ypass(int prec, int n, int inverse, void *ck) {
  return prec ? ypass<float>(n, inverse, ck) : ypass<double>(n, inverse, ck);
}

int fftp_ypass_pair(int prec, int n, double box_len, void *ck) {
  return prec ? ypass_pair<float>(n, box_len, ck) : ypass_pair<double>(n, box_len, ck);
}

int fftp_zr2c(int prec, int n, const void *V, void *ck) {
  return prec ? zr2c<float>(n, V, ck) : zr2c<double>(n, V, ck);
}

int fftp_zc2r(int prec, int n, const void *ck, void *psi) {
  return prec ? zc2r<float>(n, ck, psi) : zc2r<double>(n, ck, psi);
}


int fftp_step_boundary_x(int prec, int n, double box_len, int mode, int alpt, int two_tile, void *Ck, const void *q_in,
                         const void *p_in, const void *g_in, void *q_out, void *p_out, void *g_out, const double *wS,
                         const double *wM, const double *scal, double *guard_slot, int *stop,
                         unsigned long long *steps_done, const double *guard_prev, double guard_limit,
                         unsigned long long step_index) {
  const CtlArgs ca{stop, steps_done, guard_prev, guard_limit, step_index};
  if (!stop || !steps_done) return -1;
  return prec ? step_boundary_x<float>(n, box_len, mode, alpt, two_tile, Ck, q_in, p_in, g_in, q_out, p_out, g_out, wS, wM,
                                       scal, guard_slot, ca)
              : step_boundary_x<double>(n, box_len, mode, alpt, two_tile, Ck, q_in, p_in, g_in, q_out, p_out, g_out, wS, wM,
                                        scal, guard_slot, ca);
}

int fftp_alpt_mix_x(int prec, int n, double box_len, void *Ck, double smol, double inv_wtot, double inv_n) {
  return prec ? alpt_mix_x<float>(n, box_len, Ck, smol, inv_wtot, inv_n)
              : alpt_mix_x<double>(n, box_len, Ck, smol, inv_wtot, inv_n);
}

int fftp_kick_drift_za(int prec, int n, double box_len, int drift, void *qk, void *pk, const void *gk, const double *wM,
                       const void *extra, void *Ck, const double *scal, int *stop, unsigned long long *steps_done,
                       const double *guard_prev, double guard_limit, unsigned long long step_index) {
  const CtlArgs ca{stop, steps_done, guard_prev, guard_limit, step_index};
  if (!stop || !steps_done) return -1;
  return prec ? kick_drift_za<float>(n, box_len, drift, qk, pk, gk, wM, extra, Ck, scal, ca)
              : kick_drift_za<double>(n, box_len, drift, qk, pk, gk, wM, extra, Ck, scal, ca);
}

int fftp_assemble(int prec, int n, double box_len, int kick, const void *Ck, const void *qk, const double *wS, void *gk,
                  void *pk, const double *scal, int like_mode, double *guard_slot, int *stop) {
  return prec ? assemble<float>(n, box_len, kick, Ck, qk, wS, gk, pk, scal, like_mode, guard_slot, stop)
              : assemble<double>(n, box_len, kick, Ck, qk, wS, gk, pk, scal, like_mode, guard_slot, stop);
}

int fftp_step_boundary(int prec, int n, double box_len, int last, void *Ck, const void *q_in, const void *p_in, void *q_out,
                       void *p_out, void *gk, const double *wS, const double *wM, const double *scal, int like_mode,
                       double *guard_slot, int *stop, unsigned long long *steps_done, const double *guard_prev,
                       double guard_limit, unsigned long long step_index) {
  const CtlArgs ca{stop, steps_done, guard_prev, guard_limit, step_index};
  if (!stop || !steps_done) return -1;
  return prec ? step_boundary<float>(n, box_len, last, Ck, q_in, p_in, q_out, p_out, gk, wS, wM, scal, like_mode, guard_slot, ca)
              : step_boundary<double>(n, box_len, last, Ck, q_in, p_in, q_out, p_out, gk, wS, wM, scal, like_mode, guard_slot,
                                      ca);
}

int fftp_alpt_poisson(int prec, int n, double box_len, const void *qk, void *d1k, void *phik, double scale) {
  return prec ? alpt_poisson<float>(n, box_len, qk, d1k, phik, scale) : alpt_poisson<double>(n, box_len, qk, d1k, phik, scale);
}

int fftp_alpt_mix(int prec, int n, double box_len, void *Ck, double smol, double inv_wtot, double inv_n) {
  return prec ? alpt_mix<float>(n, box_len, Ck, smol, inv_wtot, inv_n) : alpt_mix<double>(n, box_len, Ck, smol, inv_wtot, inv_n);
}

int fftp_prepare_mult(int prec, int n, const double *corr, double *mult, double normFS) {
  return prepare_mult(n, prec ? 4 : 8, corr, mult, normFS);
}

int fftp_parseval_blocks(void) { return kRedBlocks; }
int fftp_parseval(int prec, int n, const void *xk, const double *w, double *partials) {
  return prec ? parseval<float>(n, xk, w, partials) : parseval<double>(n, xk, w, partials);
}

int fftp_rollback(int prec, long long count, const int *stop, const unsigned long long *steps_done, const void *q0,
                  const void *p0, const void *q1, const void *p1, void *q_dst, void *p_dst) {
  return prec ? rollback<float>(count, stop, steps_done, q0, p0, q1, p1, q_dst, p_dst)
              : rollback<double>(count, stop, steps_done, q0, p0, q1, p1, q_dst, p_dst);
}
// ... 55 lines not shown
```

### barcode_amd/csrc/pass_launch.hpp

```cpp
#pragma once

#include <cstddef>

namespace bchmc {

constexpr int pass_kb(int esz) { return 128 / (2 * esz); }
constexpr int pass_nt_big(int esz) { return esz == 8 ? 256 : 512; }
constexpr int pass_nt_small(int esz) { return pass_nt_big(esz) / 4; }

struct PassShape {
  int nt = 0;
  int per = 0;
};

constexpr PassShape x_shape(int esz, int n) {
  const int big = pass_nt_big(esz), small = pass_nt_small(esz);
  switch (n) {
    case 32: return {small, 4};
    case 64: return {small, 8};
    case 128: return {big, 4};
    case 256: return {2 * big, 4};
    case 512: return {2 * big, 8};
    default: return {};
  }
}
constexpr PassShape x2_shape(int esz, int n) { return n == 128 || n == 256 ? x_shape(esz, n) : PassShape{}; }
constexpr PassShape y_shape(int esz, int n) {
  const int nt = n == 128 ? 256 : 512;
  return n == 128 || n == 256 || n == 512 ? PassShape{nt, n * pass_kb(esz) / nt} : PassShape{};
}
constexpr PassShape ypair_shape(int esz, int n) { return y_shape(esz, n); }
constexpr int ypair_comps = 2;
constexpr PassShape z_shape(int , int n) { return n == 128 || n == 256 || n == 512 ? PassShape{n, 6} : PassShape{}; }

constexpr size_t col_lds(int esz, int n, int tiles = 1) { return ((size_t)tiles * n * pass_kb(esz) + n / 2) * 2 * esz; }
constexpr size_t zrow_lds(int esz, int n) { return ((size_t)n * 6 + n / 2) * 2 * esz; }

constexpr int col_grid(int esz, int n, int nhp, int comps = 1) { return comps * n * (nhp / pass_kb(esz)); }
constexpr int row_grid(int n) { return (n / 2) * (n / 2); }
constexpr int ypair_grid(int esz, int n, int nhp) { return col_grid(esz, n, nhp, ypair_comps); }

}

#ifdef __HIPCC__
#include "kernels.hpp"

#include <type_traits>

namespace bchmc {

template <typename... P, typename... A>
hipError_t launch_dyn_lds(hipStream_t stream, void (*kern)(P...), int grid, int threads, size_t lds, const A &...args) {
  if (lds > 48 * 1024) {
    const hipError_t e =
        hipFuncSetAttribute(reinterpret_cast<const void *>(kern), hipFuncAttributeMaxDynamicSharedMemorySize, (int)lds);
    if (e != hipSuccess) return e;
  }
  kern<<<grid, threads, lds, stream>>>(args...);
  return hipGetLastError();
}

template <PassShape (*TABLE)(int, int), typename T, int N, typename F>
hipError_t pass_row(int n, F &f) {
  constexpr PassShape s = TABLE((int)sizeof(T), N);
  if constexpr (s.nt != 0) {
    if (n == N) return f(std::integral_constant<int, s.nt>{}, std::integral_constant<int, s.per>{});
  }
  return hipErrorInvalidConfiguration;
}
template <PassShape (*TABLE)(int, int), typename T, typename F>
hipError_t pass_dispatch(int n, F f) {
  switch (n) {
    case 32: return pass_row<TABLE, T, 32>(n, f);
    case 64: return pass_row<TABLE, T, 64>(n, f);
    case 128: return pass_row<TABLE, T, 128>(n, f);
    case 256: return pass_row<TABLE, T, 256>(n, f);
    case 512: return pass_row<TABLE, T, 512>(n, f);
    default: return hipErrorInvalidConfiguration;
  }
}

template <typename T>
struct PassCtx {
  hipStream_t stream;
  Geo g;
  int log2n;
  const C2<T> *tw;
  int col_grid(int comps = 1) const { return bchmc::col_grid(sizeof(T), g.n, g.nhp, comps); }
  size_t col_lds(int tiles = 1) const { return bchmc::col_lds(sizeof(T), g.n, tiles); }
};

template <typename T, bool INV = true>
hipError_t launch_ypass(const PassCtx<T> &x, C2<T> *ck) {
  auto go = [&](auto nt, auto per) {
    return launch_dyn_lds(x.stream, k_ypass<T, nt, per, BCHMC_YPASS_NT, INV>, x.col_grid(3), nt, x.col_lds(), x.g, x.log2n,
                          x.tw, ck);
  };
  if constexpr (INV) return pass_dispatch<y_shape, T>(x.g.n, go);
  else return pass_row<y_shape, T, 512>(x.g.n, go);
}

template <typename T>
hipError_t launch_ypass_pair(const PassCtx<T> &x, C2<T> *ck) {
  return pass_dispatch<ypair_shape, T>(x.g.n, [&](auto nt, auto per) {
    return launch_dyn_lds(x.stream, k_ypass_pair<T, nt, per, BCHMC_YPASS_NT>, ypair_grid(sizeof(T), x.g.n, x.g.nhp), nt,
                          x.col_lds(), x.g, x.log2n, x.tw, ck);
  });
}

template <typename T>
hipError_t launch_zr2c(const PassCtx<T> &x, const T *V, C2<T> *ck) {
  return pass_dispatch<z_shape, T>(x.g.n, [&](auto nz, auto) {
    return launch_dyn_lds(x.stream, k_zr2c<T, nz>, row_grid(x.g.n), nz, zrow_lds(sizeof(T), x.g.n), x.g, x.log2n, x.tw, V, ck);
  });
}

template <typename T, bool PSI_ONLY = false, typename... A>
hipError_t launch_zbin(const PassCtx<T> &x, const PosPar &pp, const SphPar &sp, const TilePar &tp, const C2<T> *ck,
                       const A &...out) {
  return pass_dispatch<z_shape, T>(x.g.n, [&](auto nz, auto) {
    return launch_dyn_lds(x.stream, k_zbin_direct<T, nz, PSI_ONLY>, row_grid(x.g.n), nz, zbin_lds<T>(x.g.n), x.g, pp, sp, tp,
                          x.log2n, x.tw, ck, out...);
  });
}

template <typename T>
hipError_t launch_alpt_mix_x(const PassCtx<T> &x, C2<T> *Ck, double smol, double inv_wtot, double inv_n) {
  return pass_dispatch<x_shape, T>(x.g.n, [&](auto nt, auto per) {
    return launch_dyn_lds(x.stream, k_alpt_mix_x<T, nt, per>, x.col_grid(), nt, x.col_lds(), x.g, x.log2n, x.tw, Ck, smol,
                          inv_wtot, inv_n);
  });
}

template <typename T>
struct BoundaryX {
  const C2<T> *qi = nullptr, *pi = nullptr;
  C2<T> *qo = nullptr, *po = nullptr;
  const double *wM = nullptr;
  double a = 0., b = 0., half_eps = 0., eps = 0., c_za = 0.;
  double *guard_slot = nullptr;
  StepCtl ctl{};
  const C2<T> *g_in = nullptr;
  C2<T> *g_out = nullptr;
  bool pair = false;
};

template <typename T, int MODE, bool ALPT>
hipError_t launch_step_boundary_x(const PassCtx<T> &x, C2<T> *Ck, const double *wS, const BoundaryX<T> &a) {
  return pass_dispatch<x_shape, T>(x.g.n, [&](auto nt, auto per) {
    return launch_dyn_lds(x.stream, k_step_boundary_x<T, nt, per, MODE, ALPT>, x.col_grid(), nt, x.col_lds(), x.g, x.log2n,
                          x.tw, Ck, a.qi, a.pi, a.qo, a.po, wS, a.wM, a.a, a.b, a.half_eps, a.eps, a.c_za, a.guard_slot,
                          a.ctl, a.g_in, a.g_out, a.pair && !ALPT && MODE != BX_LAST);
  });
}

template <typename T>
hipError_t launch_step_boundary_x2(const PassCtx<T> &x, C2<T> *Ck, const double *wS, const BoundaryX<T> &a) {
  return pass_dispatch<x2_shape, T>(x.g.n, [&](auto nt, auto per) {
    return launch_dyn_lds(x.stream, k_step_boundary_x2<T, nt, per>, x.col_grid(), nt, x.col_lds(2), x.g, x.log2n, x.tw, Ck,
                          a.qi, a.pi, a.qo, a.po, wS, a.wM, a.a, a.b, a.half_eps, a.eps, a.c_za, a.guard_slot, a.ctl, a.pair);
  });
}

}
#endif
```

### barcode_amd/csrc/step_boundary_x.hpp

```cpp
#pragma once
#include "common.hpp"

#ifndef BCHMC_BX_WAVES
#define BCHMC_BX_WAVES 4
#endif

namespace bchmc {

#ifndef BCHMC_BX_NT
#define BCHMC_BX_NT 2
#endif
typedef double bx_dv2 __attribute__((ext_vector_type(2)));
typedef float bx_fv2 __attribute__((ext_vector_type(2)));
__device__ __forceinline__ void bx_store(double2 *p, const double2 v) {
  if (BCHMC_BX_NT) {
    bx_dv2 t = {v.x, v.y};
    __builtin_nontemporal_store(t, reinterpret_cast<bx_dv2 *>(p));
  } else {
    *p = v;
  }
}
__device__ __forceinline__ void bx_store(float2 *p, const float2 v) {
  if (BCHMC_BX_NT) {
    bx_fv2 t = {v.x, v.y};
    __builtin_nontemporal_store(t, reinterpret_cast<bx_fv2 *>(p));
  } else {
    *p = v;
  }
}

__device__ __forceinline__ double2 bx_load(const double2 *p) {
  if (BCHMC_BX_NT >= 2) {
    const bx_dv2 t = __builtin_nontemporal_load(reinterpret_cast<const bx_dv2 *>(p));
    return make_double2(t.x, t.y);
  }
  return *p;
}
__device__ __forceinline__ float2 bx_load(const float2 *p) {
  if (BCHMC_BX_NT >= 2) {
    const bx_fv2 t = __builtin_nontemporal_load(reinterpret_cast<const bx_fv2 *>(p));
    return make_float2(t.x, t.y);
  }
  return *p;
}
__device__ __forceinline__ double bx_load(const double *p) {
  return BCHMC_BX_NT >= 2 ? __builtin_nontemporal_load(p) : *p;
}

template <typename T>
__device__ __forceinline__ C2<T> cmul(const C2<T> a, const C2<T> b) {
  C2<T> r;
  r.x = a.x * b.x - a.y * b.y;
  r.y = a.x * b.y + a.y * b.x;
  return r;
}

template <typename T>
__device__ __forceinline__ void xfft_inplace(C2<T> *__restrict__ s, const C2<T> *__restrict__ tw, int n, int log2n,
                                             int KB, bool inverse) {
  int st = 1;
  if (log2n & 1) {
    const int nb = (n >> 1) * KB;
    for (int b = threadIdx.x; b < nb; b += blockDim.x) {
      const int c = b % KB, i0 = (b / KB) << 1;
      const C2<T> a = s[i0 * KB + c], x = s[(i0 + 1) * KB + c];
      C2<T> o0, o1;
      o0.x = a.x + x.x; o0.y = a.y + x.y;
      o1.x = a.x - x.x; o1.y = a.y - x.y;
      s[i0 * KB + c] = o0;
      s[(i0 + 1) * KB + c] = o1;
    }
    __syncthreads();
    st = 2;
  }
  const int nq = (n >> 2) * KB;
  for (; st < log2n; st += 2) {
    const int half = 1 << (st - 1);
    const int t1 = n >> st, t2 = n >> (st + 1);
    for (int b = threadIdx.x; b < nq; b += blockDim.x) {
      const int c = b % KB, bf = b / KB;
      const int r = bf & (half - 1), grp = bf >> (st - 1);
      const int j = (grp << (st + 1)) + r;
      C2<T> w1 = tw[r * t1], w2 = tw[r * t2];
      if (inverse) {
        w1.y = -w1.y;
        w2.y = -w2.y;
      }
      const C2<T> e0 = s[j * KB + c], e1 = s[(j + half) * KB + c], e2 = s[(j + 2 * half) * KB + c],
                  e3 = s[(j + 3 * half) * KB + c];
      const C2<T> m1 = cmul<T>(w1, e1), m3 = cmul<T>(w1, e3);
      C2<T> a0, a1, a2, a3;
      a0.x = e0.x + m1.x; a0.y = e0.y + m1.y;
      a1.x = e0.x - m1.x; a1.y = e0.y - m1.y;
      a2.x = e2.x + m3.x; a2.y = e2.y + m3.y;
      a3.x = e2.x - m3.x; a3.y = e2.y - m3.y;
      const C2<T> n2 = cmul<T>(w2, a2), n3 = cmul<T>(w2, a3);
      C2<T> r3;
      if (inverse) {
        r3.x = -n3.y; r3.y = n3.x;
      } else {
        r3.x = n3.y; r3.y = -n3.x;
      }
      C2<T> o0, o1, o2, o3;
      o0.x = a0.x + n2.x; o0.y = a0.y + n2.y;
      o2.x = a0.x - n2.x; o2.y = a0.y - n2.y;
      o1.x = a1.x + r3.x; o1.y = a1.y + r3.y;
      o3.x = a1.x - r3.x; o3.y = a1.y - r3.y;
      s[j * KB + c] = o0;
      s[(j + half) * KB + c] = o1;
      s[(j + 2 * half) * KB + c] = o2;
      s[(j + 3 * half) * KB + c] = o3;
    }
    __syncthreads();
  }
}

enum { BX_INTERIOR = 0, BX_FIRST = 1, BX_LAST = 2 };

template <typename T, int NT, int PER, int MODE = BX_INTERIOR, bool ALPT = false>
__global__ void __launch_bounds__(NT, BCHMC_BX_WAVES)
k_step_boundary_x(Geo g, int log2n, const C2<T> *__restrict__ twiddle, C2<T> *Ck, const C2<T> *q_in, const C2<T> *p_in,
                  C2<T> *q_out, C2<T> *p_out, const double *__restrict__ wS, const double *__restrict__ wM, double a,
                  double b, double half_eps, double eps, double c_za, double *guard_slot, StepCtl ctl,
                  const C2<T> *g_in = nullptr, C2<T> *g_out = nullptr, bool pair = false) {
  constexpr int KB = 128 / (int)sizeof(C2<T>);
  constexpr int kMaxPer = PER;
  extern __shared__ __attribute__((aligned(16))) unsigned char s_raw_x[];
  __shared__ double red[NT / 64];
  const bool controlled = MODE == BX_INTERIOR || (MODE == BX_FIRST && g_in) || (MODE == BX_LAST && p_out);
  if (controlled) {
    if (*ctl.stop) return;
    if (ctl.guard_prev && fabs(*ctl.guard_prev) > ctl.guard_limit) {
      if (blockIdx.x == 0 && threadIdx.x == 0) {
        *ctl.steps_done = ctl.step_index;
        __threadfence();
        *ctl.stop = 1;
      }
      return;
    }
  }
  const int n = g.n;
  C2<T> *s = reinterpret_cast<C2<T> *>(s_raw_x);
  C2<T> *tw = s + (size_t)n * KB;
  for (int t = threadIdx.x; t < n / 2; t += blockDim.x) tw[t] = twiddle[t];
  const int ntk = g.nhp / KB;
  int bid = (int)blockIdx.x;
  if ((gridDim.x & 7) == 0) bid = (bid & 7) * (int)(gridDim.x >> 3) + (bid >> 3);
  const int j = bid / ntk, k0 = (bid % ntk) * KB;
  const int c = threadIdx.x % KB, irow = threadIdx.x / KB;
  constexpr int rows = NT / KB, per = PER;
  const int k = k0 + c;
  const long long plane = (long long)g.n * g.nhp;
  const long long col = k + (long long)g.nhp * j;
  const double ky = kval(j, g.n, g.kfac), kz = kval(k, g.n, g.kfac);
  const int shift = 32 - log2n;
  double2 hk[kMaxPer];
  for (int pass = 0; pass < (MODE == BX_FIRST ? 0 : 2); pass++) {
    __syncthreads();
#pragma unroll
    for (int m = 0; m < kMaxPer; m++) {
      const int i = irow + rows * m;
      const long long e = col + plane * i;
      C2<T> v;
      if (pass == 0) {
        v = bx_load(Ck + e);
      } else {
        const C2<T> vy = bx_load(Ck + e + g.Nhp), vz = bx_load(Ck + e + 2 * g.Nhp);
        v.x = (T)(ky * (double)vy.x + kz * (double)vz.x);
        v.y = (T)(ky * (double)vy.y + kz * (double)vz.y);
      }
      s[(int)(__brev((unsigned)i) >> shift) * KB + c] = v;
    }
    __syncthreads();
    xfft_inplace<T>(s, tw, n, log2n, KB, false);
#pragma unroll
    for (int m = 0; m < kMaxPer; m++) {
      const int i = irow + rows * m;
      const C2<T> v = s[i * KB + c];
      if (pass == 0) {
        const double kx = kval(i, g.n, g.kfac);
        hk[m] = make_double2(kx * (double)v.y, -(kx * (double)v.x));
      } else {
        hk[m].x += (double)v.y;
        hk[m].y -= (double)v.x;
      }
    }
  }
  double gsum = 0.;
  C2<T> qkeep[kMaxPer];
  __syncthreads();
#pragma unroll
  for (int m = 0; m < kMaxPer; m++) {
    const int i = irow + rows * m;
    const long long idx = col + plane * i;
    const double kx = kval(i, g.n, g.kfac);
    const double ksq = kx * kx + ky * ky + kz * kz;
    const bool nyq = (i == g.n / 2) || (j == g.n / 2) || (k == g.n / 2);
    double2 q;
    if (MODE == BX_INTERIOR) {
      const C2<T> t = bx_load(q_in + idx);
      q = make_double2((double)t.x, (double)t.y);
    } else q = ld2<T>(q_in, idx);
    if (MODE == BX_FIRST) {
      if (g_in) {
        double2 p = ld2<T>(p_in, idx);
        const double2 g0 = ld2<T>(g_in, idx);
        p.x -= half_eps * g0.x;
        p.y -= half_eps * g0.y;
        st2<T>(p_out, idx, p.x, p.y);
        if (wM) {
          const double w = wM[idx];
          q.x += eps * (w * p.x);
          q.y += eps * (w * p.y);
        }
        st2<T>(q_out, idx, q.x, q.y);
      }
    } else {
      double2 gg = make_double2(0., 0.);
      if (ksq > 0 && !nyq) {
        const double f = b * (1 / ksq);
        gg = make_double2(f * hk[m].x, f * hk[m].y);
      }
// ... 147 lines not shown
  o3.x = a1.x - r3.x; o3.y = a1.y - r3.y;
  s[j * KB + c] = o0;
  s[(j + half) * KB + c] = o1;
  s[(j + 2 * half) * KB + c] = o2;
  s[(j + 3 * half) * KB + c] = o3;
}

template <typename T, bool INV>
__device__ __forceinline__ void xfft_inplace2(C2<T> *__restrict__ sa, C2<T> *__restrict__ sb,
                                              const C2<T> *__restrict__ tw, int n, int log2n, int KB) {
  int st = 1;
  if (log2n & 1) {
    const int nb = (n >> 1) * KB;
    for (int b = threadIdx.x; b < nb; b += blockDim.x) {
      const int c = b % KB, i0 = (b / KB) << 1;
#pragma unroll
      for (int u = 0; u < 2; u++) {
        C2<T> *s = u ? sb : sa;
        const C2<T> a = s[i0 * KB + c], x = s[(i0 + 1) * KB + c];
        C2<T> o0, o1;
        o0.x = a.x + x.x; o0.y = a.y + x.y;
        o1.x = a.x - x.x; o1.y = a.y - x.y;
        s[i0 * KB + c] = o0;
        s[(i0 + 1) * KB + c] = o1;
      }
    }
    __syncthreads();
    st = 2;
  }
  const int nq = (n >> 2) * KB;
  for (; st < log2n; st += 2) {
    const int half = 1 << (st - 1);
    const int t1 = n >> st, t2 = n >> (st + 1);
    for (int b = threadIdx.x; b < nq; b += blockDim.x) {
      const int c = b % KB, bf = b / KB;
      const int r = bf & (half - 1), grp = bf >> (st - 1);
      const int j = (grp << (st + 1)) + r;
      C2<T> w1 = tw[r * t1], w2 = tw[r * t2];
      if (INV) {
        w1.y = -w1.y;
        w2.y = -w2.y;
      }
      xfft_r4<T, INV>(sa, j, half, KB, c, w1, w2);
      xfft_r4<T, INV>(sb, j, half, KB, c, w1, w2);
    }
    __syncthreads();
  }
}

template <typename T, int NT, int PER>
__global__ void __launch_bounds__(NT, BCHMC_BX_WAVES)
k_step_boundary_x2(Geo g, int log2n, const C2<T> *__restrict__ twiddle, C2<T> *Ck, const C2<T> *q_in, const C2<T> *p_in,
                   C2<T> *q_out, C2<T> *p_out, const double *__restrict__ wS, const double *__restrict__ wM, double a,
                   double b, double half_eps, double eps, double c_za, double *guard_slot, StepCtl ctl, bool pair = false) {
  constexpr int KB = 128 / (int)sizeof(C2<T>);
  extern __shared__ __attribute__((aligned(16))) unsigned char s_raw_x2[];
  __shared__ double red[NT / 64];
  if (*ctl.stop) return;
  if (ctl.guard_prev && fabs(*ctl.guard_prev) > ctl.guard_limit) {
    if (blockIdx.x == 0 && threadIdx.x == 0) {
      *ctl.steps_done = ctl.step_index;
      __threadfence();
      *ctl.stop = 1;
    }
    return;
  }
  const int n = g.n;
  C2<T> *sa = reinterpret_cast<C2<T> *>(s_raw_x2);
  C2<T> *sb = sa + (size_t)n * KB;
  C2<T> *tw = sb + (size_t)n * KB;
  for (int t = threadIdx.x; t < n / 2; t += blockDim.x) tw[t] = twiddle[t];
  const int ntk = g.nhp / KB;
  int bid = (int)blockIdx.x;
  if ((gridDim.x & 7) == 0) bid = (bid & 7) * (int)(gridDim.x >> 3) + (bid >> 3);
  const int j = bid / ntk, k0 = (bid % ntk) * KB;
  const int c = threadIdx.x % KB, irow = threadIdx.x / KB;
  constexpr int rows = NT / KB;
  const int k = k0 + c;
  const long long plane = (long long)g.n * g.nhp;
  const long long col = k + (long long)g.nhp * j;
  const double ky = kval(j, g.n, g.kfac), kz = kval(k, g.n, g.kfac);
  const int shift = 32 - log2n;
  unsigned boff[PER];
#pragma unroll
  for (int m = 0; m < PER; m++) boff[m] = (unsigned)((col + plane * (irow + rows * m)) * (long long)sizeof(C2<T>));
  auto at_c = [](const C2<T> *base, unsigned off) {
    return reinterpret_cast<const C2<T> *>(reinterpret_cast<const char *>(base) + off);
  };
  auto at_cw = [](C2<T> *base, unsigned off) {
    return reinterpret_cast<C2<T> *>(reinterpret_cast<char *>(base) + off);
  };
  auto at_d = [](const double *base, unsigned off) {
    return reinterpret_cast<const double *>(reinterpret_cast<const char *>(base) + off);
  };
  C2<T> *const Ck1 = Ck + g.Nhp, *const Ck2 = Ck + 2 * g.Nhp;
  {
    C2<T> vx[PER], vy[PER], vz[PER];
#pragma unroll
    for (int m = 0; m < PER; m++) {
      vx[m] = bx_load(at_c(Ck, boff[m]));
      vy[m] = bx_load(at_c(Ck1, boff[m]));
      vz[m] = bx_load(at_c(Ck2, boff[m]));
    }
#pragma unroll
    for (int m = 0; m < PER; m++) {
      const int i = irow + rows * m;
      const int r = (int)(__brev((unsigned)i) >> shift) * KB + c;
      sa[r] = vx[m];
      C2<T> w;
      w.x = (T)(ky * (double)vy[m].x + kz * (double)vz[m].x);
      w.y = (T)(ky * (double)vy[m].y + kz * (double)vz[m].y);
      sb[r] = w;
    }
  }
  C2<T> qv[PER], pv[PER];
  double ws[PER], wm[PER];
#pragma unroll
  for (int m = 0; m < PER; m++) {
    const unsigned woff = sizeof(C2<T>) == 16 ? boff[m] / 2 : boff[m];
    qv[m] = bx_load(at_c(q_in, boff[m]));
    pv[m] = bx_load(at_c(p_in, boff[m]));
    ws[m] = (a != 0.) ? bx_load(at_d(wS, woff)) : 0.;
    wm[m] = wM ? bx_load(at_d(wM, woff)) : 0.;
  }
  __syncthreads();
  xfft_inplace2<T, false>(sa, sb, tw, n, log2n, KB);
  double2 hk[PER];
#pragma unroll
  for (int m = 0; m < PER; m++) {
    const int i = irow + rows * m;
    const C2<T> v = sa[i * KB + c], w = sb[i * KB + c];
    const double kx = kval(i, g.n, g.kfac);
    hk[m] = make_double2(kx * (double)v.y, -(kx * (double)v.x));
    hk[m].x += (double)w.y;
    hk[m].y -= (double)w.x;
  }
  __syncthreads();
  double gsum = 0.;
#pragma unroll
  for (int m = 0; m < PER; m++) {
    const int i = irow + rows * m;
    const double kx = kval(i, g.n, g.kfac);
    const double ksq = kx * kx + ky * ky + kz * kz;
    const bool nyq = (i == g.n / 2) || (j == g.n / 2) || (k == g.n / 2);
    double2 q = make_double2((double)qv[m].x, (double)qv[m].y);
    double2 gg = make_double2(0., 0.);
    if (ksq > 0 && !nyq) {
      const double f = b * (1 / ksq);
      gg = make_double2(f * hk[m].x, f * hk[m].y);
    }
    if (a != 0.) {
      const double w = a * ws[m];
      gg.x += w * q.x;
      gg.y += w * q.y;
    }
    C2<T> gs;
    gs.x = (T)gg.x;
    gs.y = (T)gg.y;
    double2 p = make_double2((double)pv[m].x, (double)pv[m].y);
    C2<T> pe;
    pe.x = (T)(p.x - half_eps * gg.x);
    pe.y = (T)(p.y - half_eps * gg.y);
    const double hw = (k == 0 || ((g.n & 1) == 0 && k == g.n / 2)) ? 1. : 2.;
    if (k < g.nh) gsum += hw * (double)pe.x;
    p.x = (double)pe.x - half_eps * (double)gs.x;
// ... 54 lines not shown
```

### barcode_amd/csrc/tiles.hpp

```cpp
#pragma once
#include "common.hpp"
#include "tile_plan.hpp"
#include "tile_walk.hpp"

namespace bchmc {


template <typename T>
__device__ __forceinline__ int subcell_octant(T x, T y, T z, T inv_d) {
  const T fx = x * inv_d, fy = y * inv_d, fz = z * inv_d;
  const int b = ((fx - r_floor(fx) >= T(0.5)) ? 4 : 0) | ((fy - r_floor(fy) >= T(0.5)) ? 2 : 0) |
                ((fz - r_floor(fz) >= T(0.5)) ? 1 : 0);
  return b ^ (b >> 1) ^ (b >> 2);
}

constexpr int kSortFlagNoScatter = 1 << 30;

using RecQuad = uint4;
template <typename T> __device__ __forceinline__ void rec_store(RecQuad *base, long long slot, T x, T y, T z, int idx);
template <> __device__ __forceinline__ void rec_store<double>(RecQuad *base, long long slot, double x, double y, double z,
                                                              int idx) {
  double2 *b = reinterpret_cast<double2 *>(base) + 2 * slot;
  b[0] = make_double2(x, y);
  b[1] = make_double2(z, __longlong_as_double((long long)(unsigned)idx));
}
template <> __device__ __forceinline__ void rec_store<float>(RecQuad *base, long long slot, float x, float y, float z,
                                                             int idx) {
  reinterpret_cast<float4 *>(base)[slot] = make_float4(x, y, z, __int_as_float(idx));
}
template <typename T> __device__ __forceinline__ void rec_load(const RecQuad *base, long long slot, T &x, T &y, T &z, int &idx);
template <> __device__ __forceinline__ void rec_load<double>(const RecQuad *base, long long slot, double &x, double &y,
                                                             double &z, int &idx) {
  const double2 *b = reinterpret_cast<const double2 *>(base) + 2 * slot;
  const double2 a = b[0], c = b[1];
  x = a.x;
  y = a.y;
  z = c.x;
  idx = (int)__double_as_longlong(c.y);
}
template <> __device__ __forceinline__ void rec_load<float>(const RecQuad *base, long long slot, float &x, float &y, float &z,
                                                            int &idx) {
  const float4 v = reinterpret_cast<const float4 *>(base)[slot];
  x = v.x;
  y = v.y;
  z = v.z;
  idx = __float_as_int(v.w);
}
template <typename T> constexpr int rec_quads() { return sizeof(T) == 8 ? 2 : 1; }

__device__ __forceinline__ int tile_of(const TilePar &tp, int n, long long ix, long long iy, long long iz) {
  const int cx = (int)(ix % n), cy = (int)(iy % n), cz = (int)(iz % n);
  return (cz / tp.tz) + tp.ntz * ((cy / tp.ty) + tp.nty * (cx / tp.tx));
}

template <typename T>
__device__ __forceinline__ long long home_cell(T x, T d) {
  return (long long)(x / d);
}

template <typename T> struct HomeCell {
  T d, inv_d, thr;
  int n;
};
template <typename T>
__device__ __forceinline__ HomeCell<T> make_home(const Geo &g) {
  HomeCell<T> hc;
  hc.d = (T)g.d;
  hc.inv_d = T(1) / hc.d;
  hc.thr = (T)g.n * (sizeof(T) == 8 ? T(1e-15) : T(5e-7));
  hc.n = g.n;
  return hc;
}
template <typename T>
__device__ __forceinline__ int home_cell_i(const HomeCell<T> &hc, T x) {
  const T f = x * hc.inv_d;
  if (__builtin_expect(fabs(f - rint(f)) < hc.thr, 0)) return (int)(x / hc.d);
  return (int)f;
}
__device__ __forceinline__ int wrap_cell(int c, int n) { return c >= n ? c - n : c; }
__device__ __forceinline__ int tile_of_wrapped(const TilePar &tp, int cx, int cy, int cz) {
  const int sx = __builtin_ctz(tp.tx), sy = __builtin_ctz(tp.ty), sz = __builtin_ctz(tp.tz);
  return (cz >> sz) + tp.ntz * ((cy >> sy) + tp.nty * (cx >> sx));
}

__device__ __forceinline__ long long brick_particle(const Geo &g, int b, int tid, int &i, int &j, int &k) {
  const int n = g.n;
  if ((n & 15) == 0) {
    const int nbz = n >> 4, nby = n >> 2;
    const int bk = b % nbz, bj = (b / nbz) % nby, bi = b / (nbz * nby);
    i = bi * 4 + (tid >> 6);
    j = bj * 4 + ((tid >> 4) & 3);
    k = bk * 16 + (tid & 15);
    return k + (long long)n * (j + (long long)n * i);
  }
  const long long p = b * 256ll + tid;
  k = (int)(p % n);
  const long long ij = p / n;
  j = (int)(ij % n);
  i = (int)(ij / n);
  return p;
}
__device__ __forceinline__ long long brick_particle(const Geo &g, int b, int &i, int &j, int &k) {
  return brick_particle(g, b, (int)threadIdx.x, i, j, k);
}

#ifndef BCHMC_BIN_PER
#define BCHMC_BIN_PER 4
#endif
#ifndef BCHMC_BIN_THREADS
#define BCHMC_BIN_THREADS 256
#endif
constexpr int kBinPer = BCHMC_BIN_PER;
constexpr int kBinGroups = BCHMC_BIN_THREADS / 256;
constexpr int kBinLoop = kBinPer / kBinGroups;

__device__ __forceinline__ int super_brick(const Geo &g, int sb, int m) {
  static_assert(kBinPer == 1 || kBinPer == 2 || kBinPer == 4, "kBinPer");
  constexpr int PJ = kBinPer >= 2 ? 2 : 1, PI = kBinPer >= 4 ? 2 : 1;
  const int n = g.n;
  if ((n & 15) == 0) {
    const int nbz = n >> 4, nby = n >> 2, nbys = nby / PJ;
    const int sbk = sb % nbz, sbj = (sb / nbz) % nbys, sbi = sb / (nbz * nbys);
    return sbk + nbz * ((PJ * sbj + (m % PJ)) + nby * (PI * sbi + (m / PJ)));
  }
  return sb * kBinPer + m;
}

#ifndef BCHMC_BIN_WAVES
#define BCHMC_BIN_WAVES (sizeof(T) == 8 ? 3 : 4)
#endif
template <typename T>
__global__ void __launch_bounds__(BCHMC_BIN_THREADS) __attribute__((amdgpu_waves_per_eu(BCHMC_BIN_WAVES, BCHMC_BIN_WAVES)))
k_bin_direct(Geo g, PosPar pp, SphPar sp, TilePar tp, int nsuper, const T *__restrict__ psi, int *__restrict__ cnt,
             int *__restrict__ ovf, RecQuad *__restrict__ srec, T *__restrict__ V, double *__restrict__ zero_part,
             T *__restrict__ rho_zero, long long *__restrict__ fix_zero) {
  constexpr int kSlots = 2048;
  __shared__ int hkey[kSlots], hcnt[kSlots], hbase[kSlots];
  if (zero_part && blockIdx.x == 0)
    for (int i = threadIdx.x; i < kRedBlocks; i += blockDim.x) zero_part[i] = 0.;
  const HomeCell<T> hc = make_home<T>(g);
  for (int sb = blockIdx.x; sb < nsuper; sb += gridDim.x) {
    for (int s = threadIdx.x; s < kSlots; s += blockDim.x) {
      hkey[s] = 0;
      hcnt[s] = 0;
    }
    __syncthreads();
    long long p[kBinLoop];
    int key[kBinLoop], slot[kBinLoop], local[kBinLoop], flag[kBinLoop];
    int li[kBinLoop], lj[kBinLoop], lk[kBinLoop];
    T x[kBinLoop], y[kBinLoop], z[kBinLoop];
    const int tid = (int)threadIdx.x & 255, grp = (int)threadIdx.x >> 8;
    constexpr int PJ = kBinPer >= 2 ? 2 : 1, PI = kBinPer >= 4 ? 2 : 1;
    const bool lattice = (g.n & 15) == 0;
    int sbi = 0, sbj = 0, sbk = 0;
    if (lattice) {
      const int nbz = g.n >> 4, nbys = (g.n >> 2) / PJ;
      sbk = sb % nbz;
      sbj = (sb / nbz) % nbys;
      sbi = sb / (nbz * nbys);
    }
#pragma unroll
    for (int m = 0; m < kBinLoop; m++) {
      const int mm = m * kBinGroups + grp;
      if (lattice) {
        li[m] = (PI * sbi + mm / PJ) * 4 + (tid >> 6);
        lj[m] = (PJ * sbj + mm % PJ) * 4 + ((tid >> 4) & 3);
        lk[m] = sbk * 16 + (tid & 15);
        p[m] = lk[m] + (long long)g.n * (lj[m] + (long long)g.n * li[m]);
      } else {
        p[m] = brick_particle(g, super_brick(g, sb, mm), tid, li[m], lj[m], lk[m]);
      }
      x[m] = y[m] = z[m] = T(0);
      if (p[m] >= g.N) continue;
      x[m] = psi[p[m]];
      y[m] = psi[p[m] + g.N];
      z[m] = psi[p[m] + 2 * g.N];
      if (rho_zero) rho_zero[p[m]] = T(0);
      if (fix_zero) fix_zero[p[m]] = 0;
    }
#pragma unroll
    for (int m = 0; m < kBinLoop; m++) {
      key[m] = -1;
      slot[m] = local[m] = flag[m] = 0;
      if (p[m] >= g.N) continue;
      particle_pos<T>(pp, li[m], lj[m], lk[m], x[m], y[m], z[m], x[m], y[m], z[m]);
      if (pos_ok(g, x[m], y[m], z[m])) {
        const int t = tile_of_wrapped(tp, wrap_cell(home_cell_i(hc, x[m]), g.n), wrap_cell(home_cell_i(hc, y[m]), g.n),
                                      wrap_cell(home_cell_i(hc, z[m]), g.n));
        flag[m] = in_domain(g, sp, x[m], y[m], z[m]) ? 0 : kSortFlagNoScatter;
        key[m] = t * kOct + subcell_octant<T>(x[m], y[m], z[m], hc.inv_d);
        int sl = (int)(((unsigned)key[m] * 2654435761u) >> 21) & (kSlots - 1);
        for (;;) {
          const int old = atomicCAS(&hkey[sl], 0, key[m] + 1);
          if (old == 0 || old == key[m] + 1) break;
          sl = (sl + 1) & (kSlots - 1);
        }
        slot[m] = sl;
        local[m] = atomicAdd(&hcnt[sl], 1);
      } else {
        V[p[m]] = T(0);
        V[p[m] + g.N] = T(0);
        V[p[m] + 2 * g.N] = T(0);
      }
    }
    __syncthreads();
    {
      constexpr int kPer = kSlots / BCHMC_BIN_THREADS;
      int hk[kPer], hb[kPer];
#pragma unroll
      for (int u = 0; u < kPer; u++) {
        const int s = (int)threadIdx.x + u * BCHMC_BIN_THREADS;
        hk[u] = hkey[s];
        hb[u] = 0;
        if (hk[u]) hb[u] = atomicAdd(&cnt[hk[u] - 1], hcnt[s]);
      }
#pragma unroll
      for (int u = 0; u < kPer; u++)
        if (hk[u]) hbase[(int)threadIdx.x + u * BCHMC_BIN_THREADS] = hb[u];
    }
    __syncthreads();
    const int seg = tp.cap / kOct;
#pragma unroll
    for (int m = 0; m < kBinLoop; m++) {
      if (key[m] < 0) continue;
      const int rank = hbase[slot[m]] + local[m];
      if (rank >= seg) {
        ovf[0] = 1;
        ovf[1] = seg;
      } else {
        const int t = key[m] / kOct;
        const long long dst = (long long)t * tp.cap + (long long)(key[m] - t * kOct) * seg + rank;
        rec_store<T>(srec, dst, x[m], y[m], z[m], (int)p[m] | flag[m]);
      }
    }
    __syncthreads();
  }
}

template <typename T>
__global__ void __launch_bounds__(256)
k_bin(Geo g, PosPar pp, SphPar sp, TilePar tp, int nbricks, const T *__restrict__ psi, int *__restrict__ cnt,
      const int *__restrict__ ovf, int2 *__restrict__ tile_rank, T *__restrict__ V) {
  constexpr int kSlots = 512;
  __shared__ int hkey[kSlots], hcnt[kSlots], hbase[kSlots];
  if (!*ovf) return;
  for (int brick = blockIdx.x; brick < nbricks; brick += gridDim.x) {
    for (int s = threadIdx.x; s < kSlots; s += blockDim.x) {
      hkey[s] = 0;
      hcnt[s] = 0;
    }
    __syncthreads();
    int i, j, k;
    const long long p = brick_particle(g, brick, i, j, k);
    const bool live = p < g.N;
    int t = -1, slot = 0, local = 0, flag = 0;
    if (live) {
      T x, y, z;
      particle_pos<T>(pp, i, j, k, psi[p], psi[p + g.N], psi[p + 2 * g.N], x, y, z);
      if (pos_ok(g, x, y, z)) {
        const HomeCell<T> hc = make_home<T>(g);
        t = tile_of_wrapped(tp, wrap_cell(home_cell_i(hc, x), g.n), wrap_cell(home_cell_i(hc, y), g.n),
                            wrap_cell(home_cell_i(hc, z), g.n));
        flag = in_domain(g, sp, x, y, z) ? 0 : kSortFlagNoScatter;
        slot = (int)(((unsigned)t * 2654435761u) >> 23) & (kSlots - 1);
        for (;;) {
          const int old = atomicCAS(&hkey[slot], 0, t + 1);
          if (old == 0 || old == t + 1) break;
          slot = (slot + 1) & (kSlots - 1);
        }
        local = atomicAdd(&hcnt[slot], 1);
      } else {
        V[p] = T(0);
        V[p + g.N] = T(0);
        V[p + 2 * g.N] = T(0);
      }
    }
    __syncthreads();
    for (int s = threadIdx.x; s < kSlots; s += blockDim.x)
      if (hkey[s]) hbase[s] = atomicAdd(&cnt[hkey[s] - 1], hcnt[s]);
    __syncthreads();
    if (live) tile_rank[p] = (t < 0) ? make_int2(-1, 0) : make_int2(t, (hbase[slot] + local) | flag);
    __syncthreads();
  }
}

__device__ __forceinline__ int2 block_exclusive_scan2_1024(int a, int b, int2 *wtot) {
  const int lane = threadIdx.x & (kWave - 1), w = threadIdx.x / kWave;
  int ia = a, ib = b;
#pragma unroll
  for (int off = 1; off < kWave; off <<= 1) {
    const int ta = __shfl_up(ia, off, kWave), tb = __shfl_up(ib, off, kWave);
    if (lane >= off) {
      ia += ta;
      ib += tb;
    }
  }
  if (lane == kWave - 1) wtot[w] = make_int2(ia, ib);
  __syncthreads();
  if (w == 0) {
    int2 v = lane < 16 ? wtot[lane] : make_int2(0, 0);
    const int2 own = v;
#pragma unroll
    for (int off = 1; off < 16; off <<= 1) {
      const int ta = __shfl_up(v.x, off, kWave), tb = __shfl_up(v.y, off, kWave);
      if (lane >= off) {
        v.x += ta;
        v.y += tb;
      }
    }
    if (lane < 16) wtot[lane] = make_int2(v.x - own.x, v.y - own.y);
  }
  __syncthreads();
  const int2 base = wtot[w];
  return make_int2(base.x + ia - a, base.y + ib - b);
}

__global__ void __launch_bounds__(1024)
k_scan_tiles(TilePar tp, const int *__restrict__ cnt_direct, const int *__restrict__ cnt_fallback,
             const int *__restrict__ ovf, long long *__restrict__ off, long long *__restrict__ tend,
             int *__restrict__ woff, int4 *__restrict__ oct, int *__restrict__ seg_out, int *__restrict__ max_out) {
  __shared__ int2 wtot[16];
  __shared__ int2 s_base;
  __shared__ int s_pop_max;
  const bool direct = !*ovf;
  const int T = tp.ntiles, tid = threadIdx.x;
  if (tid == 0) s_pop_max = 0;
  int pop_max = 0;
// ... 407 lines not shown
#pragma unroll
    for (int a = 0; a < 5; a++) {
      const T dx = ux - (T)(a - 2) * d_h, dy = uy - (T)(a - 2) * d_h, dz = uz - (T)(a - 2) * d_h;
      X[a] = r_fma(dx, dx, tiny_pos<T>());
      Y[a] = dy * dy;
      Z[a] = dz * dz;
    }
    Acc *corner = s_tile_acc + LZ * ((hy - 2) + LY * (hx - 2)) + (hz - 2);
#pragma unroll
    for (int a = 0; a < 5; a++) {
#pragma unroll
      for (int b = 0; b < 5; b++) {
        const int zw = hull81_zw(a, b);
        if (zw < 0) continue;
        const T q2ab = X[a] + Y[b];
        if (q2ab > q2_lim) continue;
        Acc *row = corner + LZ * (b + LY * a);
#pragma unroll
        for (int c = 0; c < 5; c++) {
          if (c < 2 - zw || c > 2 + zw) continue;
          const T q2 = q2ab + Z[c];
          if (q2 <= q2_lim) {
            T rq;
            const T q = sqrt_rsq(q2, rq);
            const bool far = (a == 0 || a == 4 || b == 0 || b == 4 || c == 0 || c == 4);
            const bool home = (a == 2 && b == 2 && c == 2);
            T val;
            if (home) {
              val = r_fma(q2, r_fma(c34w, q, c32w), w_norm);
            } else {
              const T t = r_max(T(2) - q, T(0));
              const T outer = (c14w * t) * (t * t);
              val = far ? outer : ((q2 <= T(1)) ? r_fma(q2, r_fma(c34w, q, c32w), w_norm) : outer);
            }
            cell_add(row + c, (double)val, fix_scale);
          }
        }
      }
    }
  }
  __syncthreads();
  double flushed = 0.;
  tile_walk<LY, LZ, kTile81Threads>(tp.lx, LY, LZ, ox, oy, oz, n, (int)threadIdx.x, kTile81Threads, [&](int c, int cell) {
    const Acc v = s_tile_acc[c];
    if (v != Acc(0)) flushed += flush_cell(rho + cell, v);
  });
  if (!FIX) {
    __shared__ double s_red_flush[4];
    flushed = block_sum(flushed, s_red_flush);
    if (threadIdx.x == 0 && flushed != 0.) atomic_add_r(rho_part + (blockIdx.x & (kRedBlocks - 1)), flushed);
  }
}

template <typename T, int LY, int LZ>
__global__ void __launch_bounds__(kTile81Threads, BCHMC_GATHER_WAVES)
k_gather_tile81(Geo g, HullPar hp, TilePar tp, int rsd, const RecQuad *__restrict__ srec,
                const long long *__restrict__ off,
                const long long *__restrict__ tend, const int *__restrict__ woff, const int4 *__restrict__ oct,
                const int *__restrict__ seg_in, const T *__restrict__ plike, T *__restrict__ V) {
  extern __shared__ __attribute__((aligned(16))) unsigned char s_raw_gather81[];
  T *s_tile_pl = reinterpret_cast<T *>(s_raw_gather81);
  int tile, pb, pe;
  long long rec0;
  OctMap om;
  if (!tile_work((int)blockIdx.x, tp, off, tend, woff, oct, seg_in, tile, rec0, pb, pe, om)) return;
  srec += rec0 * rec_quads<T>();
  const int n = g.n;
  const int tzi = tile % tp.ntz, tyi = (tile / tp.ntz) % tp.nty, txi = tile / (tp.ntz * tp.nty);
  const int ox = txi * tp.tx - 2, oy = tyi * tp.ty - 2, oz = tzi * tp.tz - 2;
  tile_walk<LY, LZ, kTile81Threads>(tp.lx, LY, LZ, ox, oy, oz, n, (int)threadIdx.x, kTile81Threads,
                                    [&](int c, int cell) { s_tile_pl[c] = plike[cell]; });
  __syncthreads();
  const T d_h = (T)hp.d_h, h_inv = (T)hp.h_inv, norm = (T)hp.norm;
  const HomeCell<T> hc = make_home<T>(g);
  for (int s = pb + threadIdx.x; s < pe; s += blockDim.x) {
    T px, py, pz;
    int rid;
    rec_load<T>(srec, om.slot(s), px, py, pz, rid);
    const int ix = home_cell_i(hc, px), iy = home_cell_i(hc, py), iz = home_cell_i(hc, pz);
    const T dpcx = px * h_inv - ((T)ix + T(0.5)) * d_h;
    const T dpcy = py * h_inv - ((T)iy + T(0.5)) * d_h;
    const T dpcz = pz * h_inv - ((T)iz + T(0.5)) * d_h;
    const int hx = wrap_cell(ix, n) - ox, hy = wrap_cell(iy, n) - oy, hz = wrap_cell(iz, n) - oz;
    T vx = T(0), vy = T(0), vz = T(0);
    const bool home_ok = (unsigned)(hx - 2) < (unsigned)tp.tx && (unsigned)(hy - 2) < (unsigned)tp.ty &&
                         (unsigned)(hz - 2) < (unsigned)tp.tz;
    if (home_ok) {
      T yh[5], zh[5];
#pragma unroll
      for (int a = 0; a < 5; a++) {
        yh[a] = dpcy - (T)(a - 2) * d_h;
        zh[a] = dpcz - (T)(a - 2) * d_h;
      }
      const T c225n = T(2.25) * norm, c3n = T(-3) * norm, c34n = T(-0.75) * norm;
      const T c3p = T(3) * norm;
      const T *corner = s_tile_pl + LZ * ((hy - 2) + LY * (hx - 2)) + (hz - 2);
#pragma unroll
      for (int a = 0; a < 5; a++) {
        const T xh_a = dpcx - (T)(a - 2) * d_h;
        const T X_a = r_fma(xh_a, xh_a, tiny_pos<T>());
#pragma unroll
        for (int b = 0; b < 5; b++) {
          const int zw = hull81_zw(a, b);
          if (zw < 0) continue;
          const T r2ab = r_fma(yh[b], yh[b], X_a);
          if (r2ab > T(4)) continue;
          const T *row = corner + LZ * (b + LY * a);
          T pl[5];
#pragma unroll
          for (int c = 0; c < 5; c++)
            if (c >= 2 - zw && c <= 2 + zw) pl[c] = row[c];
#pragma unroll
          for (int c = 0; c < 5; c++) {
            if (c < 2 - zw || c > 2 + zw) continue;
            const T q_sq = r_fma(zh[c], zh[c], r2ab);
            if (q_sq <= T(4)) {
              T rq;
              const T q = sqrt_rsq(q_sq, rq);
              const bool far = (a == 0 || a == 4 || b == 0 || b == 4 || c == 0 || c == 4);
              const bool home = (a == 2 && b == 2 && c == 2);
              T gr;
              if (home) {
                gr = r_fma(c225n, q, c3n);
              } else {
                const T outer = r_fma(c3n, rq, r_fma(c34n, q, c3p));
                gr = far ? outer : ((q_sq > T(1)) ? outer : r_fma(c225n, q, c3n));
              }
              const T common = pl[c] * gr;
              vx += common * xh_a;
              vy += common * yh[b];
              vz += common * zh[c];
            }
          }
        }
      }
    }
    const T normalize = (T)hp.normalize;
    vx *= normalize;
    vy *= normalize;
    vz *= normalize;
    if (rsd) vz += (T)hp.f1 * vz;
    const long long p = rid & ~kSortFlagNoScatter;
    V[p] = vx;
    V[p + g.N] = vy;
    V[p + 2 * g.N] = vz;
  }
}

}
```

### barcode_amd/csrc/zpass.hpp

```cpp
#pragma once
#include "common.hpp"

#ifndef BCHMC_YPASS_NT
#define BCHMC_YPASS_NT 0
#endif

namespace bchmc {

template <typename T, int NT, int PER, int HINT = 0, bool INV = true>
__global__ void __launch_bounds__(NT)
k_ypass(Geo g, int log2n, const C2<T> *__restrict__ twiddle, C2<T> *c) {
  constexpr int KB = 128 / (int)sizeof(C2<T>);
  extern __shared__ __attribute__((aligned(16))) unsigned char s_raw_y[];
  const int n = g.n;
  C2<T> *s = reinterpret_cast<C2<T> *>(s_raw_y);
  C2<T> *tw = s + (size_t)n * KB;
  for (int t = threadIdx.x; t < n / 2; t += blockDim.x) tw[t] = twiddle[t];
  const int ntk = g.nhp / KB;
  const int per_comp = n * ntk;
  const int comp = (int)blockIdx.x / per_comp, b = (int)blockIdx.x % per_comp;
  const int i = b / ntk, k0 = (b % ntk) * KB;
  const int col = threadIdx.x % KB, jrow = threadIdx.x / KB;
  constexpr int rows = NT / KB;
  C2<T> *base = c + (long long)comp * g.Nhp + (long long)g.nhp * g.n * i + k0 + col;
// ... 14 lines not shown
    else base[(long long)g.nhp * j] = s[j * KB + col];
  }
}

template <typename T, int NT, int PER, int HINT = 0>
__global__ void __launch_bounds__(NT)
k_ypass_pair(Geo g, int log2n, const C2<T> *__restrict__ twiddle, C2<T> *c) {
  constexpr int KB = 128 / (int)sizeof(C2<T>);
  extern __shared__ __attribute__((aligned(16))) unsigned char s_raw_yp[];
  const int n = g.n;
  C2<T> *s = reinterpret_cast<C2<T> *>(s_raw_yp);
  C2<T> *tw = s + (size_t)n * KB;
  for (int t = threadIdx.x; t < n / 2; t += blockDim.x) tw[t] = twiddle[t];
  const int ntk = g.nhp / KB;
  const int per_comp = n * ntk;
  const bool from_b = (int)blockIdx.x < per_comp;
  const int b = (int)blockIdx.x % per_comp;
  const int i = b / ntk, k0 = (b % ntk) * KB;
  const int col = threadIdx.x % KB, jrow = threadIdx.x / KB;
  constexpr int rows = NT / KB;
  C2<T> *base = c + (from_b ? g.Nhp : 0ll) + (long long)g.nhp * g.n * i + k0 + col;
  const int shift = 32 - log2n;
  C2<T> v[PER];
#pragma unroll
  for (int m = 0; m < PER; m++)
    v[m] = (HINT == 1 || HINT == 2) ? bx_load(base + (long long)g.nhp * (jrow + rows * m))
                                    : base[(long long)g.nhp * (jrow + rows * m)];
  const double kz = kval(k0 + col, g.n, g.kfac);
  for (int pass = 0; pass < (from_b ? 2 : 1); pass++) {
    if (pass) __syncthreads();
#pragma unroll
    for (int m = 0; m < PER; m++) {
      const int j = jrow + rows * m;
      C2<T> o = v[m];
      if (from_b) {
        const double f = pass ? kz : kval(j, g.n, g.kfac);
        o.x = (T)(f * (double)v[m].x);
        o.y = (T)(f * (double)v[m].y);
      }
      s[(int)(__brev((unsigned)j) >> shift) * KB + col] = o;
    }
    __syncthreads();
    xfft_inplace<T>(s, tw, n, log2n, KB, true);
    C2<T> *out = base + (pass ? g.Nhp : 0ll);
#pragma unroll
    for (int m = 0; m < PER; m++) {
      const int j = jrow + rows * m;
      if (HINT == 1 || HINT == 3) bx_store(out + (long long)g.nhp * j, s[j * KB + col]);
      else out[(long long)g.nhp * j] = s[j * KB + col];
    }
  }
}


#ifndef BCHMC_ZBIN_WAVES
#define BCHMC_ZBIN_WAVES ((sizeof(T) == 8 && NZ < 512) ? 3 : 4)
#endif
template <typename T, int NZ, bool PSI_ONLY = false>
__global__ void __launch_bounds__(NZ) __attribute__((amdgpu_waves_per_eu(BCHMC_ZBIN_WAVES, BCHMC_ZBIN_WAVES)))
k_zbin_direct(Geo g, PosPar pp, SphPar sp, TilePar tp, int log2n, const C2<T> *__restrict__ twiddle,
              const C2<T> *__restrict__ ck, int *__restrict__ cnt, int *__restrict__ ovf, RecQuad *__restrict__ srec,
              T *__restrict__ V, double *__restrict__ zero_part, T *__restrict__ rho_zero,
              long long *__restrict__ fix_zero, T *__restrict__ psi_out) {
  constexpr int kSlots = 4 * NZ;
  constexpr int kHashShift = 32 - (NZ == 128 ? 9 : (NZ == 256 ? 10 : 11));
  static_assert(NZ == 128 || NZ == 256 || NZ == 512, "k_zbin_direct: one thread per lattice site along z");
  constexpr int KF = 6;
  extern __shared__ __attribute__((aligned(16))) unsigned char s_raw_z[];
  unsigned long long *hcnt = reinterpret_cast<unsigned long long *>(s_raw_z);
  unsigned long long *hbase = hcnt + kSlots;
  int *hkey = reinterpret_cast<int *>(hbase + kSlots);
  if (PSI_ONLY && !*ovf) return;
  const int n = g.n, tid = (int)threadIdx.x;
  C2<T> *s = reinterpret_cast<C2<T> *>(s_raw_z);
  C2<T> *tw = s + (size_t)n * KF;
  if (!PSI_ONLY && zero_part && blockIdx.x == 0)
    for (int i = tid; i < kRedBlocks; i += NZ) zero_part[i] = 0.;
  for (int t = tid; t < n / 2; t += NZ) tw[t] = twiddle[t];
  const int nb = n >> 1;
  const int j0 = 2 * ((int)blockIdx.x % nb), i0 = 2 * ((int)blockIdx.x / nb);
  const int shift = 32 - log2n;
  {
    const int w = tid >> 6, f = w & 1;
    const long long row = (long long)g.nhp * (j0 + (long long)n * (i0 + f));
    {
      const int kk = ((w >> 1) << 6) + (tid & 63);
      C2<T> a[3], b[3], an[3], bn[3];
#pragma unroll
      for (int c = 0; c < 3; c++) {
        a[c] = ck[(long long)c * g.Nhp + row + kk];
        b[c] = ck[(long long)c * g.Nhp + row + g.nhp + kk];
        if (kk == 0) {
          an[c] = ck[(long long)c * g.Nhp + row + n / 2];
          bn[c] = ck[(long long)c * g.Nhp + row + g.nhp + n / 2];
        }
      }
#pragma unroll
      for (int c = 0; c < 3; c++) {
        const int colf = 2 * c + f;
        C2<T> lo, hi;
        if (kk == 0) {
          lo.x = a[c].x; lo.y = b[c].x;
          hi.x = an[c].x; hi.y = bn[c].x;
          s[(int)(__brev(0u) >> shift) * KF + colf] = lo;
          s[(int)(__brev((unsigned)(n / 2)) >> shift) * KF + colf] = hi;
        } else {
          lo.x = a[c].x - b[c].y; lo.y = a[c].y + b[c].x;
          hi.x = a[c].x + b[c].y; hi.y = b[c].x - a[c].y;
          s[(int)(__brev((unsigned)kk) >> shift) * KF + colf] = lo;
          s[(int)(__brev((unsigned)(n - kk)) >> shift) * KF + colf] = hi;
        }
      }
    }
  }
  __syncthreads();
  xfft_inplace<T>(s, tw, n, log2n, KF, true);
  const HomeCell<T> hc = make_home<T>(g);
  long long p[4];
  int key[4], slot[4], local[4], flag[4];
  T x[4], y[4], z[4];
#pragma unroll
  for (int f = 0; f < 2; f++) {
    const C2<T> vx = s[tid * KF + f], vy = s[tid * KF + 2 + f], vz = s[tid * KF + 4 + f];
    x[2 * f] = vx.x; x[2 * f + 1] = vx.y;
    y[2 * f] = vy.x; y[2 * f + 1] = vy.y;
    z[2 * f] = vz.x; z[2 * f + 1] = vz.y;
  }
  if (!PSI_ONLY) {
    __syncthreads();
    for (int t = tid; t < kSlots; t += NZ) {
      hkey[t] = 0;
      hcnt[t] = 0ull;
    }
    __syncthreads();
  }
#pragma unroll
  for (int m = 0; m < 4; m++) {
    const int li = i0 + (m >> 1), lj = j0 + (m & 1);
    p[m] = tid + (long long)n * (lj + (long long)n * li);
    if (PSI_ONLY || psi_out) {
      psi_out[p[m]] = x[m];
      psi_out[p[m] + g.N] = y[m];
      psi_out[p[m] + 2 * g.N] = z[m];
    }
    if (PSI_ONLY) continue;
    if (rho_zero) rho_zero[p[m]] = T(0);
    if (fix_zero) fix_zero[p[m]] = 0;
    key[m] = -1;
    slot[m] = local[m] = flag[m] = 0;
    particle_pos<T>(pp, li, lj, tid, x[m], y[m], z[m], x[m], y[m], z[m]);
    if (pos_ok(g, x[m], y[m], z[m])) {
      const int t = tile_of_wrapped(tp, wrap_cell(home_cell_i(hc, x[m]), g.n), wrap_cell(home_cell_i(hc, y[m]), g.n),
                                    wrap_cell(home_cell_i(hc, z[m]), g.n));
      flag[m] = in_domain(g, sp, x[m], y[m], z[m]) ? 0 : kSortFlagNoScatter;
      key[m] = t * kOct + subcell_octant<T>(x[m], y[m], z[m], hc.inv_d);
      const int pk = key[m] >> 1;
      int sl = (int)(((unsigned)pk * 2654435761u) >> kHashShift) & (kSlots - 1);
      for (;;) {
        const int old = atomicCAS(&hkey[sl], 0, pk + 1);
        if (old == 0 || old == pk + 1) break;
        sl = (sl + 1) & (kSlots - 1);
      }
      slot[m] = sl;
      const int sh = (key[m] & 1) << 5;
      local[m] = (int)((atomicAdd(&hcnt[sl], 1ull << sh) >> sh) & 0xffffffffull);
    } else {
      V[p[m]] = T(0);
      V[p[m] + g.N] = T(0);
      V[p[m] + 2 * g.N] = T(0);
    }
  }
  if (PSI_ONLY) return;
  __syncthreads();
  {
    constexpr int kPer = kSlots / NZ;
    int hk[kPer];
    unsigned long long hb[kPer];
#pragma unroll
    for (int u = 0; u < kPer; u++) {
      const int sl = tid + u * NZ;
      hk[u] = hkey[sl];
      hb[u] = 0ull;
      if (hk[u])
        hb[u] = atomicAdd(reinterpret_cast<unsigned long long *>(cnt) + (hk[u] - 1), hcnt[sl]);
    }
#pragma unroll
    for (int u = 0; u < kPer; u++)
      if (hk[u]) hbase[tid + u * NZ] = hb[u];
  }
  __syncthreads();
  const int seg = tp.cap / kOct;
#pragma unroll
  for (int m = 0; m < 4; m++) {
    if (key[m] < 0) continue;
    const int sh = (key[m] & 1) << 5;
    const int rank = (int)((hbase[slot[m]] >> sh) & 0xffffffffull) + local[m];
    if (rank >= seg) {
      ovf[0] = 1;
      ovf[1] = seg;
    } else {
      const int t = key[m] / kOct;
      const long long dst = (long long)t * tp.cap + (long long)(key[m] - t * kOct) * seg + rank;
      rec_store<T>(srec, dst, x[m], y[m], z[m], (int)p[m] | flag[m]);
    }
  }
}

template <typename T, int NZ>
__global__ void __launch_bounds__(NZ)
k_zr2c(Geo g, int log2n, const C2<T> *__restrict__ twiddle, const T *__restrict__ V, C2<T> *__restrict__ ck) {
  constexpr int KF = 6;
  extern __shared__ __attribute__((aligned(16))) unsigned char s_raw_zr[];
  const int n = g.n, tid = (int)threadIdx.x;
  C2<T> *s = reinterpret_cast<C2<T> *>(s_raw_zr);
  C2<T> *tw = s + (size_t)n * KF;
  for (int t = tid; t < n / 2; t += NZ) tw[t] = twiddle[t];
  const int nb = n >> 1;
  const int j0 = 2 * ((int)blockIdx.x % nb), i0 = 2 * ((int)blockIdx.x / nb);
  const int shift = 32 - log2n;
  {
    const int r = (int)(__brev((unsigned)tid) >> shift) * KF;
#pragma unroll
    for (int c = 0; c < 3; c++)
#pragma unroll
      for (int f = 0; f < 2; f++) {
        const long long p = tid + (long long)n * (j0 + (long long)n * (i0 + f));
        C2<T> v;
        v.x = V[(long long)c * g.N + p];
        v.y = V[(long long)c * g.N + p + n];
        s[r + 2 * c + f] = v;
      }
  }
  __syncthreads();
  xfft_inplace<T>(s, tw, n, log2n, KF, false);
  const int w = tid >> 6, f = w & 1, kk = ((w >> 1) << 6) + (tid & 63);
  const long long row = (long long)g.nhp * (j0 + (long long)n * (i0 + f));
#pragma unroll
  for (int c = 0; c < 3; c++) {
    const int colf = 2 * c + f;
    const C2<T> zk = s[kk * KF + colf], zm = s[((n - kk) & (n - 1)) * KF + colf];
    C2<T> a, b;
    a.x = T(0.5) * (zk.x + zm.x);
    a.y = T(0.5) * (zk.y - zm.y);
    b.x = T(0.5) * (zk.y + zm.y);
    b.y = T(-0.5) * (zk.x - zm.x);
    ck[(long long)c * g.Nhp + row + kk] = a;
    ck[(long long)c * g.Nhp + row + g.nhp + kk] = b;
    if (kk == 0) {
      const C2<T> zh = s[(n / 2) * KF + colf];
      C2<T> ah, bh;
      ah.x = zh.x; ah.y = T(0);
      bh.x = zh.y; bh.y = T(0);
      ck[(long long)c * g.Nhp + row + n / 2] = ah;
      ck[(long long)c * g.Nhp + row + g.nhp + n / 2] = bh;
    }
  }
}

template <typename T>
__global__ void k_scale_r(long long n, T *x, T s) {
  for (long long i = blockIdx.x * (long long)blockDim.x + threadIdx.x; i < n; i += (long long)gridDim.x * blockDim.x)
    x[i] *= s;
}

template <typename T> inline size_t zbin_lds(int n) {
  const size_t tile = ((size_t)n * 6 + n / 2) * sizeof(C2<T>), hash = (size_t)4 * n * 20;
  return tile > hash ? tile : hash;
}

}
```

Measured before the change: 375.7 steps/s.

## Gather velocities as packed records and pair-fuse the forward y-pass into divergence

The tile gather now writes the three velocity components as one interleaved 4-wide record per particle, so the z-direction r2c pass reads them with vector loads instead of three strided arrays. A new forward y-pass kernel transforms the y and z components together and combines them into a single paired field, which cuts the number of complex arrays the step-boundary kernels must read. This adds a second V buffer, state flags for the paired layout with guard checks, and an unpack kernel for fetching velocities. The risk is extra memory and more complex state tracking between evaluation and boundary stages.

```diff
diff --git a/barcode_amd/csrc/bchmc.hip b/barcode_amd/csrc/bchmc.hip
--- a/barcode_amd/csrc/bchmc.hip
+++ b/barcode_amd/csrc/bchmc.hip
@@ -64,6 +64,10 @@
   DevBytes tC;
   DevBytes psi;
   DevBytes V;
+  DevBytes vrec;
+  bool ck_vpair = false;
+  bool vrec_eval = false;
+  bool v_in_vrec = false;
   DevBytes rho, plike;
   DevBuf<long long> rho_fix;
   DevBuf<int> fix_sat;
@@ -428,7 +432,7 @@
 }
 
 struct FieldSource {
-  enum Made { kAsHeld, kOverdens, kPositions };
+  enum Made { kAsHeld, kOverdens, kPositions, kVrec };
   void *base = nullptr;
   size_t offset = 0;
   Made made = kAsHeld;
@@ -445,7 +449,10 @@
     case BCHMC_F_POSX: case BCHMC_F_POSY: case BCHMC_F_POSZ: fs->base = h->ioq.get(), fs->made = FieldSource::kPositions; break;
     case BCHMC_F_RHO: fs->base = h->rho.get(); break;
     case BCHMC_F_PART_LIKE: fs->base = h->plike.get(); break;
-    case BCHMC_F_VX: case BCHMC_F_VY: case BCHMC_F_VZ: fs->base = h->V.get(), fs->offset = (size_t)(field - BCHMC_F_VX) * N; break;
+    case BCHMC_F_VX: case BCHMC_F_VY: case BCHMC_F_VZ:
+      if (h->v_in_vrec) fs->base = h->ioq.get(), fs->made = FieldSource::kVrec;
+      else fs->base = h->V.get(), fs->offset = (size_t)(field - BCHMC_F_VX) * N;
+      break;
     case BCHMC_F_PSIX: case BCHMC_F_PSIY: case BCHMC_F_PSIZ:
       fs->base = h->psi.get(), fs->offset = (size_t)(field - BCHMC_F_PSIX) * N;
       break;
@@ -629,6 +636,8 @@
   s.bx_v1 = env_on("BCHMC_BX_V1");
   s.bx_v2 = env_on("BCHMC_BX_V2");
   s.no_pair = env_on("BCHMC_NO_PAIR");
+  s.no_vpair = env_on("BCHMC_NO_VPAIR");
+  s.no_vrec = env_on("BCHMC_NO_VREC");
   return s;
 }
 
@@ -636,7 +645,7 @@
   PathFacts f;
   f.n = h->g.n, f.esz = (int)h->esz, f.Nhp = h->g.Nhp;
   f.planes_ok = h->planes_ok && h->xtw;
-  f.tiled = h->plan.tiled, f.sort_direct = h->plan.slots.sort_direct;
+  f.tiled = h->plan.tiled, f.sort_direct = h->plan.slots.sort_direct, f.std81 = h->plan.std81;
   f.mk = h->c.mk, f.calc_h = h->c.calc_h, f.likelihood = h->c.likelihood, f.sfmodel = h->c.sfmodel;
   f.rsd_model = h->c.rsd_model, f.mass_rs = h->mass_rs != 0;
   if (alpt_planes_wanted(f, h->sw, rsd) && !h->c2r2d_2 && !h->alpt_plans_failed &&
@@ -1342,6 +1351,9 @@
     bool rho_cleared = false;
     const PosPar pp = make_pos(h, rsd);
     const SphPar sp = make_sph(h);
+    h->vrec_eval = eval_vrec(path_facts(h, h->c.rsd_model), h->sw, m);
+    if (h->vrec_eval && !h->vrec) CHK(dev_alloc(h, h->vrec, 4 * (size_t)h->g.N * sizeof(T)));
+    T *const vrec = h->vrec_eval ? R(h->vrec) : nullptr;
     if (h->plan.tiled) {
       ProfScope ps(h, BCHMC_K_SORT);
       const int nt = h->plan.tp.ntiles, nbricks = nblk_full(h->g.N);
@@ -1352,22 +1364,23 @@
       if (zbin) {
         HIPCHK(launch_zbin<T>(pass_ctx(h), pp, sp, h->plan.tp, C(h->Ck), cnt1, ovf, recs(h), R(h->V), h->rho_part,
                               h->fix ? nullptr : R(h->rho), h->fix ? h->rho_fix : nullptr,
-                              m.psi_unread ? nullptr : R(h->psi)));
+                              m.psi_unread ? nullptr : R(h->psi), vrec));
         if (m.psi_unread)
           HIPCHK((launch_zbin<T, true>(pass_ctx(h), pp, sp, h->plan.tp, C(h->Ck), cnt1, ovf, nullptr, nullptr, nullptr,
-                                       nullptr, nullptr, R(h->psi))));
+                                       nullptr, nullptr, R(h->psi), nullptr)));
         rho_cleared = true;
       } else if (h->plan.slots.sort_direct) {
         const int nsuper = (nbricks + kBinPer - 1) / kBinPer;
         k_bin_direct<T><<<nsuper, BCHMC_BIN_THREADS, 0, h->stream>>>(h->g, pp, sp, h->plan.tp, nsuper, R(h->psi), cnt1, ovf,
                                                        recs(h), R(h->V), h->rho_part,
                                                        h->fix ? nullptr : R(h->rho),
-                                                       h->fix ? h->rho_fix : nullptr);
+                                                       h->fix ? h->rho_fix : nullptr, vrec);
         rho_cleared = true;
       } else {
         HIPCHK(hipMemsetAsync(ovf, 1, 1, h->stream));
       }
-      k_bin<T><<<fb_grid, 256, 0, h->stream>>>(h->g, pp, sp, h->plan.tp, nbricks, R(h->psi), cnt2, ovf, h->t_rank, R(h->V));
+      k_bin<T><<<fb_grid, 256, 0, h->stream>>>(h->g, pp, sp, h->plan.tp, nbricks, R(h->psi), cnt2, ovf, h->t_rank, R(h->V),
+                                             vrec);
       k_scan_tiles<<<(nt + 1023) / 1024, 1024, 0, h->stream>>>(h->plan.tp, cnt1, cnt2, ovf, h->t_off, h->t_end, h->t_woff,
                                                                h->t_oct, h->t_seg, ovf + 2);
       k_reorder<T><<<fb_grid, 256, 0, h->stream>>>(h->g, pp, nbricks, R(h->psi), h->t_rank, h->t_off, ovf,
@@ -1475,6 +1488,8 @@
       return h->fail(BCHMC_ERR_ARG, "calc_h = %d is not a valid value (0..3)", h->c.calc_h);
     }
     const long long N = h->g.N, Nh = h->g.Nhp;
+    const bool vrec = h->vrec_eval;
+    h->vrec_eval = h->v_in_vrec = h->ck_vpair = false;
     {
       ProfScope ps(h, BCHMC_K_MEAN_PARTIAL);
       k_partial_like<T><<<nblk_stride(N), 256, 0, h->stream>>>(h->g, make_like(h), R(h->rho), h->rho_part,
@@ -1547,7 +1562,12 @@
       HullPar hp = make_hull(h);
       if (h->plan.tiled && h->sorted_valid) {
         const int grid = tile_grid(h);
-        if (h->plan.std81)
+        if (h->plan.std81 && vrec) {
+          k_gather_tile81<T, 12, 20, true><<<grid, kTile81Threads, tile_lds(h, 0, sizeof(T)), h->stream>>>(
+              h->g, hp, h->plan.tp, h->last_rsd, recs(h), h->t_off, h->t_end, h->t_woff,
+              h->t_oct, h->t_seg, R(h->plike), R(h->vrec));
+          h->v_in_vrec = true;
+        } else if (h->plan.std81)
           k_gather_tile81<T, 12, 20><<<grid, kTile81Threads, tile_lds(h, 0, sizeof(T)), h->stream>>>(
               h->g, hp, h->plan.tp, h->last_rsd, recs(h), h->t_off, h->t_end, h->t_woff,
               h->t_oct, h->t_seg, R(h->plike), R(h->V));
@@ -1560,8 +1580,18 @@
                                                                                   R(h->psi), R(h->plike), R(h->V));
       }
       HIPCHK(hipGetLastError());
-    }
+      if (vrec && !h->v_in_vrec) return h->fail(BCHMC_ERR_STATE, "V records were zeroed and no gather writes records");
+    }
+    const bool vpair = eval_vpair(path_facts(h, h->c.rsd_model), h->sw, m);
+    if (transform && h->v_in_vrec && !vpair)
+      return h->fail(BCHMC_ERR_STATE, "V was gathered as records, and a transform that reads three arrays");
     if (!transform) {
+    } else if (vpair) {
+      ProfScope ps(h, BCHMC_K_FFT_R2C);
+      if (h->v_in_vrec) HIPCHK((launch_zr2c<T, true>(pass_ctx(h), R(h->vrec), C(h->Ck))));
+      else HIPCHK(launch_zr2c<T>(pass_ctx(h), R(h->V), C(h->Ck)));
+      HIPCHK(launch_ypass_fwd_pair<T>(pass_ctx(h), C(h->Ck)));
+      h->ck_vpair = true;
     } else if (eval_yfwd(path_facts(h, h->c.rsd_model), h->sw, m)) {
       ProfScope ps(h, BCHMC_K_FFT_R2C);
       HIPCHK(launch_zr2c<T>(pass_ctx(h), R(h->V), C(h->Ck)));
@@ -1617,6 +1647,7 @@
   template <bool KICK>
   static int launch_assemble(bchmc_handle *h, double a, double b, int like_mode, double c_kick, double *guard_slot) {
     h->prop_g_valid = false;
+    if (h->ck_vpair) return h->fail(BCHMC_ERR_STATE, "two arrays of V^ in Ck, and a kernel that reads three");
     ProfScope ps(h, BCHMC_K_KSPACE_FORCE_KICK);
     k_assemble<T, KICK><<<nblk_stride(h->g.Nhp), 256, 0, h->stream>>>(h->g, C(h->Ck), C(h->qk), h->wS, C(h->gk), C(h->pk),
                                                                      a, b, like_mode, c_kick, guard_slot, h->stop);
@@ -1685,7 +1716,12 @@
   }
 
   template <int MODE, bool ALPT = false>
-  static int launch_boundary_x(bchmc_handle *h, const BoundaryX<T> &bx) {
+  static int launch_boundary_x(bchmc_handle *h, BoundaryX<T> bx) {
+    if (MODE != BX_FIRST) {
+      if (ALPT && h->ck_vpair) return h->fail(BCHMC_ERR_STATE, "two arrays of V^ in Ck, and a boundary that reads three");
+      bx.vpair = h->ck_vpair;
+      h->ck_vpair = false;
+    }
     HIPCHK((launch_step_boundary_x<T, MODE, ALPT>(pass_ctx(h), C(h->Ck), h->wS, bx)));
     h->ck_pair = bx.pair && !ALPT && MODE != BX_LAST;
     return BCHMC_OK;
@@ -1825,6 +1861,7 @@
           CHK(launch_boundary_x<BX_LAST>(h, bx));
           break;
         case Closing::kStepBoundaryLast:
+          if (h->ck_vpair) return h->fail(BCHMC_ERR_STATE, "two arrays of V^ in Ck, and a boundary that reads three");
           k_step_boundary<T, true><<<nblk_stride(h->g.Nhp), 256, 0, h->stream>>>(
               h->g, C(h->Ck), C(qi), C(pi), C(qi), C(pi), C(h->gk), h->wS, wM, a, b, like_mode, 0.5 * eps, eps, c_za,
               h->guard + s, ctl);
@@ -1832,10 +1869,13 @@
         case Closing::kBxInteriorAlpt: CHK((launch_boundary_x<BX_INTERIOR, true>(h, bx))); break;
         case Closing::kBxInterior: CHK(launch_boundary_x<BX_INTERIOR>(h, bx)); break;
         case Closing::kBxInteriorTwoTile:
+          bx.vpair = h->ck_vpair;
+          h->ck_vpair = false;
           HIPCHK(launch_step_boundary_x2<T>(pass_ctx(h), C(h->Ck), h->wS, bx));
           h->ck_pair = bx.pair;
           break;
         case Closing::kStepBoundary:
+          if (h->ck_vpair) return h->fail(BCHMC_ERR_STATE, "two arrays of V^ in Ck, and a boundary that reads three");
           k_step_boundary<T, false><<<nblk_stride(h->g.Nhp), 256, 0, h->stream>>>(
               h->g, C(h->Ck), C(qi), C(pi), C(qo), C(po), C(h->gk), h->wS, wM, a, b, like_mode, 0.5 * eps, eps, c_za,
               h->guard + s, ctl);
@@ -2138,7 +2178,7 @@
     HIPCHK(hipGetLastError());
     HIPCHK(launch_zr2c<T>(pass_ctx(h), R(h->psi), C(h->Ck)));
     EvalMode m;
-    m.planes_c2r = true;
+    m.planes_c2r = m.planes_r2c = true;
     m.psi_unread = !store_psi;
     CHK(particle_stage(h, rsd, m, true));
     int like_mode = 0;
@@ -2577,6 +2617,8 @@
     if (fs.made == FieldSource::kPositions)
       k_positions<T><<<nblk_stride(h->g.N), 256, 0, h->stream>>>(h->g, make_pos(h, h->last_rsd), R(h->psi), R(h->ioq),
                                                                  (int)field - (int)BCHMC_F_POSX);
+    if (fs.made == FieldSource::kVrec)
+      k_vrec_unpack<T><<<nblk_stride(h->g.N), 256, 0, h->stream>>>(h->g.N, R(h->vrec), (int)field - (int)BCHMC_F_VX, R(h->ioq));
     if (fs.made != FieldSource::kAsHeld) HIPCHK(hipGetLastError());
     return store_real(h, R(fs.base) + fs.offset, d_out);
   }
diff --git a/barcode_amd/csrc/eval_plan.hpp b/barcode_amd/csrc/eval_plan.hpp
--- a/barcode_amd/csrc/eval_plan.hpp
+++ b/barcode_amd/csrc/eval_plan.hpp
@@ -15,6 +15,8 @@
   bool bx_v1 = false;
   bool bx_v2 = false;
   bool no_pair = false;
+  bool no_vpair = false;
+  bool no_vrec = false;
 };
 
 struct PathFacts {
@@ -26,6 +28,7 @@
   int mk = 3, calc_h = 2, likelihood = 1, sfmodel = 1, rsd_model = 0;
   bool mass_rs = false;
   bool alpt_plans = false;
+  bool std81 = false;
 };
 
 struct EvalMode {
@@ -106,6 +109,18 @@
   return tp;
 }
 
+constexpr bool v_pair(const PathFacts &f, const PathSwitches &s, const TrajPlan &tp) {
+  return !s.no_vpair && !tp.alpt_x && f.n != 512 && planes_on(f, s) && zbin_ok(f, s) && f.std81 &&
+         y_shape(f.esz, f.n).nt && z_shape(f.esz, f.n).nt && yfwd_pair_shape(f.esz, f.n).nt;
+}
+constexpr bool eval_vpair(const PathFacts &f, const PathSwitches &s, const EvalMode &m) {
+  return m.planes_r2c && v_pair(f, s, traj_plan(f, s));
+}
+constexpr bool v_rec(const PathFacts &f, const PathSwitches &s) { return v_pair(f, s, traj_plan(f, s)) && !s.no_vrec; }
+constexpr bool eval_vrec(const PathFacts &f, const PathSwitches &s, const EvalMode &m) {
+  return eval_vpair(f, s, m) && !s.no_vrec;
+}
+
 enum class InitialEval { k3d, kBxFirst, kBxFirstAlpt };
 constexpr InitialEval initial_eval(const PathFacts &f, const PathSwitches &s, const TrajPlan &tp) {
   if (!(tp.fused && planes_at_ends(f, s))) return InitialEval::k3d;
diff --git a/barcode_amd/csrc/fft_probe.hip b/barcode_amd/csrc/fft_probe.hip
--- a/barcode_amd/csrc/fft_probe.hip
+++ b/barcode_amd/csrc/fft_probe.hip
@@ -120,7 +120,7 @@
 }
 
 template <typename T> int ypass(int n, int inverse, void *ck) {
-  if (!y_shape(sizeof(T), n).nt || (!inverse && n != 512)) return -1;
+  if (!y_shape(sizeof(T), n).nt) return -1;
   const Geo g = probe_geo(n, (int)sizeof(T));
   if (g.nhp % pass_kb(sizeof(T))) return -1;
   Probe pr;
@@ -143,15 +143,27 @@
   return pr.finish({{1, ck}});
 }
 
-template <typename T> int zr2c(int n, const void *V, void *ck) {
+template <typename T> int ypass_fwd_pair(int n, double box_len, void *ck) {
+  if (!yfwd_pair_shape(sizeof(T), n).nt) return -1;
+  const Geo g = probe_geo(n, (int)sizeof(T), box_len);
+  if (g.nhp % pass_kb(sizeof(T))) return -1;
+  Probe pr;
+  const PassCtx<T> x = pr.ctx<T>(g);
+  C2<T> *d = static_cast<C2<T> *>(pr.alloc((size_t)3 * g.Nhp * sizeof(C2<T>), ck));
+  if (pr.err) return pr.err;
+  pr.ok(launch_ypass_fwd_pair<T>(x, d));
+  return pr.finish({{1, ck}});
+}
+
+template <typename T, bool REC = false> int zr2c(int n, const void *V, void *ck) {
   if (!z_shape(sizeof(T), n).nt) return -1;
   const Geo g = probe_geo(n, (int)sizeof(T));
   Probe pr;
   const PassCtx<T> x = pr.ctx<T>(g);
-  const T *dv = static_cast<const T *>(pr.alloc((size_t)3 * g.N * sizeof(T), V));
+  const T *dv = static_cast<const T *>(pr.alloc((size_t)(REC ? 4 : 3) * g.N * sizeof(T), V));
   C2<T> *dc = static_cast<C2<T> *>(pr.alloc((size_t)3 * g.Nhp * sizeof(C2<T>), ck));
   if (pr.err) return pr.err;
-  pr.ok(launch_zr2c<T>(x, dv, dc));
+  pr.ok((launch_zr2c<T, REC>(x, dv, dc)));
   return pr.finish({{2, ck}});
 }
 
@@ -166,7 +178,7 @@
   T *dp = static_cast<T *>(pr.alloc((size_t)3 * g.N * sizeof(T), nullptr));
   if (pr.err) return pr.err;
   pr.ok((launch_zbin<T, true>(x, PosPar{}, SphPar{}, TilePar{}, dc, nullptr, ovf, nullptr, nullptr, nullptr, nullptr, nullptr,
-                              dp)));
+                              dp, nullptr)));
   return pr.finish({{3, psi}});
 }
 
@@ -209,8 +221,9 @@
 template <typename T>
 int step_boundary_x(int n, double L, int mode, int alpt, int two_tile, void *Ck, const void *q_in, const void *p_in,
                     const void *g_in, void *q_out, void *p_out, void *g_out, const double *wS, const double *wM,
-                    const double *scal, double *guard_slot, const CtlArgs &ca) {
+                    const double *scal, double *guard_slot, const CtlArgs &ca, int vpair = 0) {
   if (mode < BX_INTERIOR || mode > BX_LAST || (alpt && mode == BX_LAST)) return -1;
+  if (vpair && (alpt || mode == BX_FIRST)) return -1;
   if (two_tile ? (!x2_shape(sizeof(T), n).nt || mode != BX_INTERIOR || alpt) : !x_shape(sizeof(T), n).nt) return -1;
   const Geo g = probe_geo(n, (int)sizeof(T), L);
   if (g.nhp % pass_kb(sizeof(T)) || !Ck || !q_in || !scal) return -1;
@@ -237,6 +250,7 @@
   a.guard_slot = opt<double>(pr, sizeof(double), guard_slot, &i_gs);
   const CtlDev cd = ctl_alloc(pr, ca);
   a.ctl = cd.ctl;
+  a.vpair = vpair != 0;
   if (pr.err) return pr.err;
   hipError_t e = hipErrorInvalidConfiguration;
   if (two_tile) e = launch_step_boundary_x2<T>(x, d_ck, d_ws, a);
@@ -579,6 +593,14 @@
   return prec ? zr2c<float>(n, V, ck) : zr2c<double>(n, V, ck);
 }
 
+int fftp_zr2c_rec(int prec, int n, const void *V, void *ck) {
+  return prec ? zr2c<float, true>(n, V, ck) : zr2c<double, true>(n, V, ck);
+}
+
+int fftp_ypass_fwd_pair(int prec, int n, double box_len, void *ck) {
+  return prec ? ypass_fwd_pair<float>(n, box_len, ck) : ypass_fwd_pair<double>(n, box_len, ck);
+}
+
 int fftp_zc2r(int prec, int n, const void *ck, void *psi) {
   return prec ? zc2r<float>(n, ck, psi) : zc2r<double>(n, ck, psi);
 }
@@ -597,6 +619,19 @@
                                         scal, guard_slot, ca);
 }
 
+int fftp_step_boundary_x_vpair(int prec, int n, double box_len, int mode, int alpt, int two_tile, void *Ck, const void *q_in,
+                               const void *p_in, const void *g_in, void *q_out, void *p_out, void *g_out, const double *wS,
+                               const double *wM, const double *scal, double *guard_slot, int *stop,
+                               unsigned long long *steps_done, const double *guard_prev, double guard_limit,
+                               unsigned long long step_index, int vpair) {
+  const CtlArgs ca{stop, steps_done, guard_prev, guard_limit, step_index};
+  if (!stop || !steps_done) return -1;
+  return prec ? step_boundary_x<float>(n, box_len, mode, alpt, two_tile, Ck, q_in, p_in, g_in, q_out, p_out, g_out, wS, wM,
+                                       scal, guard_slot, ca, vpair)
+              : step_boundary_x<double>(n, box_len, mode, alpt, two_tile, Ck, q_in, p_in, g_in, q_out, p_out, g_out, wS, wM,
+                                        scal, guard_slot, ca, vpair);
+}
+
 int fftp_alpt_mix_x(int prec, int n, double box_len, void *Ck, double smol, double inv_wtot, double inv_n) {
   return prec ? alpt_mix_x<float>(n, box_len, Ck, smol, inv_wtot, inv_n)
               : alpt_mix_x<double>(n, box_len, Ck, smol, inv_wtot, inv_n);
diff --git a/barcode_amd/csrc/pass_launch.hpp b/barcode_amd/csrc/pass_launch.hpp
--- a/barcode_amd/csrc/pass_launch.hpp
+++ b/barcode_amd/csrc/pass_launch.hpp
@@ -31,6 +31,7 @@
 }
 constexpr PassShape ypair_shape(int esz, int n) { return y_shape(esz, n); }
 constexpr int ypair_comps = 2;
+constexpr PassShape yfwd_pair_shape(int esz, int n) { return ypair_shape(esz, n); }
 constexpr PassShape z_shape(int , int n) { return n == 128 || n == 256 || n == 512 ? PassShape{n, 6} : PassShape{}; }
 
 constexpr size_t col_lds(int esz, int n, int tiles = 1) { return ((size_t)tiles * n * pass_kb(esz) + n / 2) * 2 * esz; }
@@ -92,12 +93,18 @@
 
 template <typename T, bool INV = true>
 hipError_t launch_ypass(const PassCtx<T> &x, C2<T> *ck) {
-  auto go = [&](auto nt, auto per) {
+  return pass_dispatch<y_shape, T>(x.g.n, [&](auto nt, auto per) {
     return launch_dyn_lds(x.stream, k_ypass<T, nt, per, BCHMC_YPASS_NT, INV>, x.col_grid(3), nt, x.col_lds(), x.g, x.log2n,
                           x.tw, ck);
-  };
-  if constexpr (INV) return pass_dispatch<y_shape, T>(x.g.n, go);
-  else return pass_row<y_shape, T, 512>(x.g.n, go);
+  });
+}
+
+template <typename T>
+hipError_t launch_ypass_fwd_pair(const PassCtx<T> &x, C2<T> *ck) {
+  return pass_dispatch<yfwd_pair_shape, T>(x.g.n, [&](auto nt, auto per) {
+    return launch_dyn_lds(x.stream, k_ypass_fwd_pair<T, nt, per>, ypair_grid(sizeof(T), x.g.n, x.g.nhp),
+                          nt, x.col_lds(), x.g, x.log2n, x.tw, ck);
+  });
 }
 
 template <typename T>
@@ -108,10 +115,11 @@
   });
 }
 
-template <typename T>
+template <typename T, bool REC = false>
 hipError_t launch_zr2c(const PassCtx<T> &x, const T *V, C2<T> *ck) {
   return pass_dispatch<z_shape, T>(x.g.n, [&](auto nz, auto) {
-    return launch_dyn_lds(x.stream, k_zr2c<T, nz>, row_grid(x.g.n), nz, zrow_lds(sizeof(T), x.g.n), x.g, x.log2n, x.tw, V, ck);
+    return launch_dyn_lds(x.stream, k_zr2c<T, nz, REC>, row_grid(x.g.n), nz, zrow_lds(sizeof(T), x.g.n), x.g, x.log2n, x.tw, V,
+                          ck);
   });
 }
 
@@ -143,6 +151,7 @@
   const C2<T> *g_in = nullptr;
   C2<T> *g_out = nullptr;
   bool pair = false;
+  bool vpair = false;
 };
 
 template <typename T, int MODE, bool ALPT>
@@ -150,7 +159,8 @@
   return pass_dispatch<x_shape, T>(x.g.n, [&](auto nt, auto per) {
     return launch_dyn_lds(x.stream, k_step_boundary_x<T, nt, per, MODE, ALPT>, x.col_grid(), nt, x.col_lds(), x.g, x.log2n,
                           x.tw, Ck, a.qi, a.pi, a.qo, a.po, wS, a.wM, a.a, a.b, a.half_eps, a.eps, a.c_za, a.guard_slot,
-                          a.ctl, a.g_in, a.g_out, a.pair && !ALPT && MODE != BX_LAST);
+                          a.ctl, a.g_in, a.g_out, a.pair && !ALPT && MODE != BX_LAST,
+                          a.vpair && !ALPT && MODE != BX_FIRST);
   });
 }
 
@@ -158,7 +168,8 @@
 hipError_t launch_step_boundary_x2(const PassCtx<T> &x, C2<T> *Ck, const double *wS, const BoundaryX<T> &a) {
   return pass_dispatch<x2_shape, T>(x.g.n, [&](auto nt, auto per) {
     return launch_dyn_lds(x.stream, k_step_boundary_x2<T, nt, per>, x.col_grid(), nt, x.col_lds(2), x.g, x.log2n, x.tw, Ck,
-                          a.qi, a.pi, a.qo, a.po, wS, a.wM, a.a, a.b, a.half_eps, a.eps, a.c_za, a.guard_slot, a.ctl, a.pair);
+                          a.qi, a.pi, a.qo, a.po, wS, a.wM, a.a, a.b, a.half_eps, a.eps, a.c_za, a.guard_slot, a.ctl, a.pair,
+                          a.vpair);
   });
 }
 
diff --git a/barcode_amd/csrc/step_boundary_x.hpp b/barcode_amd/csrc/step_boundary_x.hpp
--- a/barcode_amd/csrc/step_boundary_x.hpp
+++ b/barcode_amd/csrc/step_boundary_x.hpp
@@ -53,6 +53,14 @@
   r.x = a.x * b.x - a.y * b.y;
   r.y = a.x * b.y + a.y * b.x;
   return r;
+}
+
+template <typename T>
+__device__ __forceinline__ C2<T> bx_w_of(double ky, double kz, const C2<T> vy, const C2<T> vz) {
+  C2<T> w;
+  w.x = (T)(ky * (double)vy.x + kz * (double)vz.x);
+  w.y = (T)(ky * (double)vy.y + kz * (double)vz.y);
+  return w;
 }
 
 template <typename T>
@@ -122,7 +130,7 @@
 k_step_boundary_x(Geo g, int log2n, const C2<T> *__restrict__ twiddle, C2<T> *Ck, const C2<T> *q_in, const C2<T> *p_in,
                   C2<T> *q_out, C2<T> *p_out, const double *__restrict__ wS, const double *__restrict__ wM, double a,
                   double b, double half_eps, double eps, double c_za, double *guard_slot, StepCtl ctl,
-                  const C2<T> *g_in = nullptr, C2<T> *g_out = nullptr, bool pair = false) {
+                  const C2<T> *g_in = nullptr, C2<T> *g_out = nullptr, bool pair = false, bool vpair = false) {
   constexpr int KB = 128 / (int)sizeof(C2<T>);
   constexpr int kMaxPer = PER;
   extern __shared__ __attribute__((aligned(16))) unsigned char s_raw_x[];
@@ -164,10 +172,11 @@
       C2<T> v;
       if (pass == 0) {
         v = bx_load(Ck + e);
+      } else if (vpair) {
+        v = bx_load(Ck + e + g.Nhp);
       } else {
         const C2<T> vy = bx_load(Ck + e + g.Nhp), vz = bx_load(Ck + e + 2 * g.Nhp);
-        v.x = (T)(ky * (double)vy.x + kz * (double)vz.x);
-        v.y = (T)(ky * (double)vy.y + kz * (double)vz.y);
+        v = bx_w_of<T>(ky, kz, vy, vz);
       }
       s[(int)(__brev((unsigned)i) >> shift) * KB + c] = v;
     }
@@ -421,7 +430,8 @@
 __global__ void __launch_bounds__(NT, BCHMC_BX_WAVES)
 k_step_boundary_x2(Geo g, int log2n, const C2<T> *__restrict__ twiddle, C2<T> *Ck, const C2<T> *q_in, const C2<T> *p_in,
                    C2<T> *q_out, C2<T> *p_out, const double *__restrict__ wS, const double *__restrict__ wM, double a,
-                   double b, double half_eps, double eps, double c_za, double *guard_slot, StepCtl ctl, bool pair = false) {
+                   double b, double half_eps, double eps, double c_za, double *guard_slot, StepCtl ctl, bool pair = false,
+                   bool vpair = false) {
   constexpr int KB = 128 / (int)sizeof(C2<T>);
   extern __shared__ __attribute__((aligned(16))) unsigned char s_raw_x2[];
   __shared__ double red[NT / 64];
@@ -469,17 +479,14 @@
     for (int m = 0; m < PER; m++) {
       vx[m] = bx_load(at_c(Ck, boff[m]));
       vy[m] = bx_load(at_c(Ck1, boff[m]));
-      vz[m] = bx_load(at_c(Ck2, boff[m]));
+      if (!vpair) vz[m] = bx_load(at_c(Ck2, boff[m]));
     }
 #pragma unroll
     for (int m = 0; m < PER; m++) {
       const int i = irow + rows * m;
       const int r = (int)(__brev((unsigned)i) >> shift) * KB + c;
       sa[r] = vx[m];
-      C2<T> w;
-      w.x = (T)(ky * (double)vy[m].x + kz * (double)vz[m].x);
-      w.y = (T)(ky * (double)vy[m].y + kz * (double)vz[m].y);
-      sb[r] = w;
+      sb[r] = vpair ? vy[m] : bx_w_of<T>(ky, kz, vy[m], vz[m]);
     }
   }
   C2<T> qv[PER], pv[PER];
diff --git a/barcode_amd/csrc/tiles.hpp b/barcode_amd/csrc/tiles.hpp
--- a/barcode_amd/csrc/tiles.hpp
+++ b/barcode_amd/csrc/tiles.hpp
@@ -48,6 +48,25 @@
 }
 template <typename T> constexpr int rec_quads() { return sizeof(T) == 8 ? 2 : 1; }
 
+template <typename T> __device__ __forceinline__ void vrec_store(T *rec, long long p, T vx, T vy, T vz);
+template <> __device__ __forceinline__ void vrec_store<double>(double *rec, long long p, double vx, double vy, double vz) {
+  double2 *b = reinterpret_cast<double2 *>(rec) + 2 * p;
+  b[0] = make_double2(vx, vy);
+  b[1] = make_double2(vz, 0.);
+}
+template <> __device__ __forceinline__ void vrec_store<float>(float *rec, long long p, float vx, float vy, float vz) {
+  reinterpret_cast<float4 *>(rec)[p] = make_float4(vx, vy, vz, 0.f);
+}
+template <typename T> __device__ __forceinline__ void v_zero(T *V, T *vrec, long long p, long long N) {
+  if (vrec) {
+    vrec_store<T>(vrec, p, T(0), T(0), T(0));
+  } else {
+    V[p] = T(0);
+    V[p + N] = T(0);
+    V[p + 2 * N] = T(0);
+  }
+}
+
 __device__ __forceinline__ int tile_of(const TilePar &tp, int n, long long ix, long long iy, long long iz) {
   const int cx = (int)(ix % n), cy = (int)(iy % n), cz = (int)(iz % n);
   return (cz / tp.tz) + tp.ntz * ((cy / tp.ty) + tp.nty * (cx / tp.tx));
@@ -133,7 +152,7 @@
 __global__ void __launch_bounds__(BCHMC_BIN_THREADS) __attribute__((amdgpu_waves_per_eu(BCHMC_BIN_WAVES, BCHMC_BIN_WAVES)))
 k_bin_direct(Geo g, PosPar pp, SphPar sp, TilePar tp, int nsuper, const T *__restrict__ psi, int *__restrict__ cnt,
              int *__restrict__ ovf, RecQuad *__restrict__ srec, T *__restrict__ V, double *__restrict__ zero_part,
-             T *__restrict__ rho_zero, long long *__restrict__ fix_zero) {
+             T *__restrict__ rho_zero, long long *__restrict__ fix_zero, T *__restrict__ vrec = nullptr) {
   constexpr int kSlots = 2048;
   __shared__ int hkey[kSlots], hcnt[kSlots], hbase[kSlots];
   if (zero_part && blockIdx.x == 0)
@@ -198,9 +217,7 @@
         slot[m] = sl;
         local[m] = atomicAdd(&hcnt[sl], 1);
       } else {
-        V[p[m]] = T(0);
-        V[p[m] + g.N] = T(0);
-        V[p[m] + 2 * g.N] = T(0);
+        v_zero<T>(V, vrec, p[m], g.N);
       }
     }
     __syncthreads();
@@ -240,7 +257,7 @@
 template <typename T>
 __global__ void __launch_bounds__(256)
 k_bin(Geo g, PosPar pp, SphPar sp, TilePar tp, int nbricks, const T *__restrict__ psi, int *__restrict__ cnt,
-      const int *__restrict__ ovf, int2 *__restrict__ tile_rank, T *__restrict__ V) {
+      const int *__restrict__ ovf, int2 *__restrict__ tile_rank, T *__restrict__ V, T *__restrict__ vrec = nullptr) {
   constexpr int kSlots = 512;
   __shared__ int hkey[kSlots], hcnt[kSlots], hbase[kSlots];
   if (!*ovf) return;
@@ -270,9 +287,7 @@
         }
         local = atomicAdd(&hcnt[slot], 1);
       } else {
-        V[p] = T(0);
-        V[p + g.N] = T(0);
-        V[p + 2 * g.N] = T(0);
+        v_zero<T>(V, vrec, p, g.N);
       }
     }
     __syncthreads();
@@ -786,7 +801,7 @@
   }
 }
 
-template <typename T, int LY, int LZ>
+template <typename T, int LY, int LZ, bool REC = false>
 __global__ void __launch_bounds__(kTile81Threads, BCHMC_GATHER_WAVES)
 k_gather_tile81(Geo g, HullPar hp, TilePar tp, int rsd, const RecQuad *__restrict__ srec,
                 const long long *__restrict__ off,
@@ -875,10 +890,20 @@
     vz *= normalize;
     if (rsd) vz += (T)hp.f1 * vz;
     const long long p = rid & ~kSortFlagNoScatter;
-    V[p] = vx;
-    V[p + g.N] = vy;
-    V[p + 2 * g.N] = vz;
-  }
-}
-
-}
+    if (REC) {
+      vrec_store<T>(V, p, vx, vy, vz);
+    } else {
+      V[p] = vx;
+      V[p + g.N] = vy;
+      V[p + 2 * g.N] = vz;
+    }
+  }
+}
+
+template <typename T>
+__global__ void k_vrec_unpack(long long n, const T *__restrict__ vrec, int c, T *__restrict__ out) {
+  for (long long i = blockIdx.x * (long long)blockDim.x + threadIdx.x; i < n; i += (long long)gridDim.x * blockDim.x)
+    out[i] = vrec[4 * i + c];
+}
+
+}
diff --git a/barcode_amd/csrc/zpass.hpp b/barcode_amd/csrc/zpass.hpp
--- a/barcode_amd/csrc/zpass.hpp
+++ b/barcode_amd/csrc/zpass.hpp
@@ -90,6 +90,77 @@
   }
 }
 
+template <typename T, int NT, int PER>
+__global__ void __launch_bounds__(NT)
+k_ypass_fwd_pair(Geo g, int log2n, const C2<T> *__restrict__ twiddle, C2<T> *c) {
+  constexpr int KB = 128 / (int)sizeof(C2<T>);
+  extern __shared__ __attribute__((aligned(16))) unsigned char s_raw_yf[];
+  const int n = g.n;
+  C2<T> *s = reinterpret_cast<C2<T> *>(s_raw_yf);
+  C2<T> *tw = s + (size_t)n * KB;
+  for (int t = threadIdx.x; t < n / 2; t += blockDim.x) tw[t] = twiddle[t];
+  const int ntk = g.nhp / KB;
+  const int per_comp = n * ntk;
+  const bool to_w = (int)blockIdx.x < per_comp;
+  const int b = (int)blockIdx.x % per_comp;
+  const int i = b / ntk, k0 = (b % ntk) * KB;
+  const int col = threadIdx.x % KB, jrow = threadIdx.x / KB;
+  constexpr int rows = NT / KB;
+  C2<T> *base = c + (to_w ? g.Nhp : 0ll) + (long long)g.nhp * g.n * i + k0 + col;
+  const int shift = 32 - log2n;
+  if (!to_w) {
+    C2<T> v[PER];
+#pragma unroll
+    for (int m = 0; m < PER; m++) v[m] = base[(long long)g.nhp * (jrow + rows * m)];
+#pragma unroll
+    for (int m = 0; m < PER; m++) s[(int)(__brev((unsigned)(jrow + rows * m)) >> shift) * KB + col] = v[m];
+    __syncthreads();
+    xfft_inplace<T>(s, tw, n, log2n, KB, false);
+#pragma unroll
+    for (int m = 0; m < PER; m++) {
+      const int j = jrow + rows * m;
+      base[(long long)g.nhp * j] = s[j * KB + col];
+    }
+    return;
+  }
+  T yx[PER], yy[PER], zx[PER], zy[PER];
+#pragma unroll
+  for (int m = 0; m < PER; m++) {
+    const C2<T> a = base[(long long)g.nhp * (jrow + rows * m)], b2 = base[g.Nhp + (long long)g.nhp * (jrow + rows * m)];
+    yx[m] = a.x, yy[m] = a.y, zx[m] = b2.x, zy[m] = b2.y;
+  }
+#pragma unroll
+  for (int m = 0; m < PER; m++) {
+    C2<T> a;
+    a.x = yx[m], a.y = yy[m];
+    s[(int)(__brev((unsigned)(jrow + rows * m)) >> shift) * KB + col] = a;
+  }
+  __syncthreads();
+  xfft_inplace<T>(s, tw, n, log2n, KB, false);
+#pragma unroll
+  for (int m = 0; m < PER; m++) {
+    const C2<T> a = s[(jrow + rows * m) * KB + col];
+    yx[m] = a.x, yy[m] = a.y;
+  }
+  __syncthreads();
+#pragma unroll
+  for (int m = 0; m < PER; m++) {
+    C2<T> a;
+    a.x = zx[m], a.y = zy[m];
+    s[(int)(__brev((unsigned)(jrow + rows * m)) >> shift) * KB + col] = a;
+  }
+  __syncthreads();
+  xfft_inplace<T>(s, tw, n, log2n, KB, false);
+  const double kz = kval(k0 + col, g.n, g.kfac);
+#pragma unroll
+  for (int m = 0; m < PER; m++) {
+    const int j = jrow + rows * m;
+    C2<T> a;
+    a.x = yx[m], a.y = yy[m];
+    const C2<T> w = bx_w_of<T>(kval(j, g.n, g.kfac), kz, a, s[j * KB + col]);
+    base[(long long)g.nhp * j] = w;
+  }
+}
 
 #ifndef BCHMC_ZBIN_WAVES
 #define BCHMC_ZBIN_WAVES ((sizeof(T) == 8 && NZ < 512) ? 3 : 4)
@@ -99,7 +170,7 @@
 k_zbin_direct(Geo g, PosPar pp, SphPar sp, TilePar tp, int log2n, const C2<T> *__restrict__ twiddle,
               const C2<T> *__restrict__ ck, int *__restrict__ cnt, int *__restrict__ ovf, RecQuad *__restrict__ srec,
               T *__restrict__ V, double *__restrict__ zero_part, T *__restrict__ rho_zero,
-              long long *__restrict__ fix_zero, T *__restrict__ psi_out) {
+              long long *__restrict__ fix_zero, T *__restrict__ psi_out, T *__restrict__ vrec = nullptr) {
   constexpr int kSlots = 4 * NZ;
   constexpr int kHashShift = 32 - (NZ == 128 ? 9 : (NZ == 256 ? 10 : 11));
   static_assert(NZ == 128 || NZ == 256 || NZ == 512, "k_zbin_direct: one thread per lattice site along z");
@@ -203,9 +274,7 @@
       const int sh = (key[m] & 1) << 5;
       local[m] = (int)((atomicAdd(&hcnt[sl], 1ull << sh) >> sh) & 0xffffffffull);
     } else {
-      V[p[m]] = T(0);
-      V[p[m] + g.N] = T(0);
-      V[p[m] + 2 * g.N] = T(0);
+      v_zero<T>(V, vrec, p[m], g.N);
     }
   }
   if (PSI_ONLY) return;
@@ -244,7 +313,20 @@
   }
 }
 
-template <typename T, int NZ>
+template <typename T> struct VRec4 { T x, y, z, w; };
+template <typename T> __device__ __forceinline__ VRec4<T> vrec_load(const T *rec, long long p);
+template <> __device__ __forceinline__ VRec4<double> vrec_load<double>(const double *rec, long long p) {
+  const double2 *b = reinterpret_cast<const double2 *>(rec) + 2 * p;
+  const double2 lo = b[0], hi = b[1];
+  return {lo.x, lo.y, hi.x, hi.y};
+}
+template <> __device__ __forceinline__ VRec4<float> vrec_load<float>(const float *rec, long long p) {
+  const float4 v = reinterpret_cast<const float4 *>(rec)[p];
+  return {v.x, v.y, v.z, v.w};
+}
+
+
+template <typename T, int NZ, bool REC = false>
 __global__ void __launch_bounds__(NZ)
 k_zr2c(Geo g, int log2n, const C2<T> *__restrict__ twiddle, const T *__restrict__ V, C2<T> *__restrict__ ck) {
   constexpr int KF = 6;
@@ -256,7 +338,26 @@
   const int nb = n >> 1;
   const int j0 = 2 * ((int)blockIdx.x % nb), i0 = 2 * ((int)blockIdx.x / nb);
   const int shift = 32 - log2n;
-  {
+  if (REC) {
+    const int r = (int)(__brev((unsigned)tid) >> shift) * KF;
+    VRec4<T> a[2], b[2];
+#pragma unroll
+    for (int f = 0; f < 2; f++) {
+      const long long p = tid + (long long)n * (j0 + (long long)n * (i0 + f));
+      a[f] = vrec_load<T>(V, p);
+      b[f] = vrec_load<T>(V, p + n);
+    }
+#pragma unroll
+    for (int f = 0; f < 2; f++) {
+      C2<T> v;
+      v.x = a[f].x, v.y = b[f].x;
+      s[r + f] = v;
+      v.x = a[f].y, v.y = b[f].y;
+      s[r + 2 + f] = v;
+      v.x = a[f].z, v.y = b[f].z;
+      s[r + 4 + f] = v;
+    }
+  } else {
     const int r = (int)(__brev((unsigned)tid) >> shift) * KF;
 #pragma unroll
     for (int c = 0; c < 3; c++)
```

Result: faster. 389.1 steps/s (median of 6 runs) (+3.6%).
